# langfod/Zonos

Measured on AMD Instinct MI355X. Metric: audio-sec/sec (RTF), Zonos-v0.1-transformer AR decode loop + DAC decode, higher is better.
Workload: dtype bf16; 1 GPU; Zonos-v0.1-transformer bf16, batch=1 per GPU, 10 s target audio (861 frames, 868 decode steps + prefill of 25 positions, EOS suppressed), greedy, cfg_scale 2; weights=seeded synthetic (zonos_amd/synth.py), parallelism=dp1 (utterance sharding, no data-path collective)

## Files before the change

### include/zonos_hip.h

```cpp
#ifndef ZONOS_HIP_H
#define ZONOS_HIP_H
#include <stddef.h>
#include <stdint.h>

#ifdef __cplusplus
extern "C" {
#endif

#define ZN_ABI_VERSION 9

enum zn_status {
  ZN_OK = 0,
  ZN_ERR_ARG = -1,
  ZN_ERR_HIP = -2,
  ZN_ERR_STATE = -3,
  ZN_ERR_UNSUPPORTED = -4,
  ZN_ERR_NOMEM = -5
};

typedef struct zn_handle_s* zn_handle;
typedef struct zn_dac_s* zn_dac;
typedef struct zn_spk_s* zn_spk;
typedef void* zn_stream;

// ... 9 lines not shown
  int32_t arch;
  int32_t m_d_inner;
  int32_t m_headdim;
  int32_t m_d_state;
  int32_t m_ngroups;
  int32_t m_d_conv;
  int32_t rms_norm;
  int32_t residual_in_fp32;
  int32_t rope_mode;
} zn_config;

typedef struct zn_layer_weights {
  const void *norm_w, *norm_b;
  const void *in_proj;
  const void *out_proj;
  const void *norm2_w, *norm2_b;
  const void *fc1;
  const void *fc2;
  int32_t kind;
  const void *m_in_proj;
  const void *m_conv_w, *m_conv_b;
  const void *m_dt_bias, *m_A_log, *m_D;
  const void *m_norm_w;
  const void *m_out_proj;
  const void *in_proj_bias;
  const void *out_proj_bias;
} zn_layer_weights;

typedef struct zn_weights {
  const void* const* embeddings;
  const void* heads;
  const void *norm_f_w, *norm_f_b;
  const zn_layer_weights* layers;
  const float* rope_table;
} zn_weights;

typedef struct zn_sampling {
  float temperature;
  float top_p; int32_t top_k; float min_p;
  float linear, conf, quad;
  float repetition_penalty; int32_t repetition_penalty_window;
  uint64_t seed;
} zn_sampling;

#define ZN_ROW_PARAMS_BYTES 64
typedef struct zn_row_params {
  zn_sampling sp;
  float cfg_scale;
  int32_t max_new_tokens;
  int32_t reserved[2];
} zn_row_params;

typedef struct zn_admit {
  int32_t slot;
  int32_t row_len;
  int32_t prefix_len;
  int32_t reserved;
  zn_row_params params;
} zn_admit;

int zn_abi_version(void);
int zn_create(const zn_config* cfg, const zn_weights* w, int32_t max_rows, zn_handle* out);
int zn_destroy(zn_handle h);
const char* zn_last_error(zn_handle h);
size_t zn_kv_bytes_per_layer(const zn_config* cfg, int32_t rows, int32_t max_len);
size_t zn_mamba_state_bytes_per_layer(const zn_config* cfg, int32_t rows, size_t* conv_bytes);

int zn_gen_begin(zn_handle h, int32_t batch, const void* const* kv_layers_dev, int32_t max_len,
                 int32_t* lengths_dev, int32_t* delayed_codes_dev, int32_t t_total, int32_t offset0,
                 int32_t max_new_tokens, float cfg_scale, const zn_sampling* sp, zn_stream stream);
int zn_prefill(zn_handle h, const void* hidden_dev, int32_t S, zn_stream stream);
int zn_gen_set_rows(zn_handle h, const zn_row_params* rows_host, int32_t n);
int zn_gen_set_prefix_rows(zn_handle h, const int32_t* prefix_len_host, int32_t n);
int zn_gen_open_slots(zn_handle h, int32_t slack);
int zn_gen_admit(zn_handle h, const zn_admit* a, int32_t n, const void* hidden_dev, int32_t S, zn_stream stream);
int zn_gen_retire(zn_handle h, int32_t slot);
int zn_gen_row_state(zn_handle h, int32_t* remaining_host, int32_t* steps_host, zn_stream stream);
int zn_prefill_rows(zn_handle h, const void* hidden_dev, int32_t S, const int32_t* row_len, zn_stream stream);
int zn_sample_first(zn_handle h, zn_stream stream);
int zn_decode_steps(zn_handle h, int32_t n, zn_stream stream);
int zn_graph_active(zn_handle h);
int zn_decode_path(zn_handle h);
int zn_decode_path_detail(zn_handle h);
int zn_get_counters(zn_handle h, int64_t* out, int32_t n);
int zn_gen_end(zn_handle h);
int zn_tenant_try_claim(int32_t device, const void* owner);
int zn_tenant_release(int32_t device, const void* owner);
int zn_all_stopped(zn_handle h, int32_t* out, zn_stream stream);
int zn_all_stopped_begin(zn_handle h, zn_stream stream);
int zn_all_stopped_end(zn_handle h, int32_t* all_stopped_out);
int zn_get_step_outputs(zn_handle h, float* logits_dev, int32_t* tokens_dev, zn_stream stream);
int zn_codes_changed(zn_handle h);
int zn_debug_force_eos(zn_handle h, int32_t step);
int zn_debug_token_override(zn_handle h, const int32_t* tokens_dev, int32_t calls);
int zn_debug_prefill_mode(zn_handle h, int32_t mode);
enum zn_tune_key {
  ZN_TUNE_WG_IN_PROJ = 0,
  ZN_TUNE_WG_OUT_PROJ = 1,
  ZN_TUNE_WG_FC1 = 2,
  ZN_TUNE_WG_FC2 = 3,
  ZN_TUNE_WG_HEADS = 4,
  ZN_TUNE_ATTN_FUSED_MAX_KEYS = 5,
  ZN_TUNE_GRAPH_RUNS = 6,
  ZN_TUNE_SMALL_M_LDS = 7,
  ZN_TUNE_PERSISTENT = 8,
  ZN_TUNE_FC1_LN_LAUNCH = 9,
  ZN_TUNE_PREFILL_ATTN_VALU = 10,
  ZN_TUNE_NO_SPLIT_SMALL_M = 11,
  ZN_TUNE_NO_PREFILL_GEMM16K = 12,
  ZN_TUNE_GEMM16K_MAX_TILES = 13,
  ZN_TUNE_HOOK = 14,
  ZN_TUNE_WHOLE_STEP = 15,
  ZN_TUNE_SAMPLER = 16,
  ZN_TUNE_RESERVED_17 = 17,
  ZN_TUNE_STACK_PRE = 18,
  ZN_TUNE_ATTN_SPLIT_COLS = 19,
  ZN_TUNE_NKEYS = 20
};
enum zn_tune_hook {
  ZN_HOOK_TAG_WRAP = 7,
  ZN_HOOK_TIMEOUT_WORD = 9,
  ZN_HOOK_PAUSE = 11,
  ZN_HOOK_RESET_WAIT_STATS = 13
};
int zn_debug_tune(zn_handle h, int32_t key, int32_t value);
int zn_debug_chain_stamps(zn_handle h, uint64_t* stamps_dev);
int zn_debug_trace(zn_handle h, void* trace_dev);
int zn_debug_eos_bias(zn_handle h, float bias);

int zn_op_backbone_forward(zn_handle h, const void* hidden_dev, void* out_dev, const void* const* caches_dev, int32_t max_len,
                           int32_t base, int32_t S, int32_t rows, zn_stream stream);

int zn_bench_kernel(zn_handle h, int32_t which, int32_t rows, int32_t iters, float* ms_per_launch,
                    double* bytes_per_launch, zn_stream stream);

int zn_op_linear(zn_handle h, const void* x_dev, const void* ln_w, const void* ln_b, const void* W_dev,
                 void* out_dev, int32_t rows, int32_t N, int32_t K, zn_stream stream);
int zn_op_linear_bias(zn_handle h, const void* x_dev, const void* W_dev, const void* bias_dev, void* out_dev, int32_t rows,
                      int32_t N, int32_t K, zn_stream stream);
int zn_op_gather_rows(zn_handle h, const void* table_dev, const int32_t* ids_dev, void* out_dev, int32_t n, int32_t d,
                      int32_t table_rows, int32_t id_offset, zn_stream stream);
int zn_op_fourier(zn_handle h, const float* x_dev, const void* weight_dev, void* out_dev, int32_t n, int32_t in_dim,
                  int32_t half, float min_val, float max_val, zn_stream stream);
int zn_op_silu(zn_handle h, const void* x_dev, void* out_dev, int64_t n, zn_stream stream);
int zn_op_layernorm(zn_handle h, const void* x_dev, const void* w_dev, const void* b_dev, void* out_dev, int32_t rows,
                    int32_t d, zn_stream stream);
int zn_op_layer_decode(zn_handle h, int32_t layer, void* x_dev, void* kv_dev, int32_t max_len,
                       const int32_t* lengths_dev, const int32_t* ext_dev, int32_t rows, zn_stream stream);
int zn_op_attn_decode(zn_handle h, const void* q_dev, const void* kv_dev, int32_t max_len, const int32_t* lengths_dev,
                      const int32_t* ext_dev, void* out_dev, int32_t rows, zn_stream stream);
int zn_op_attn_prefill(zn_handle h, const void* q_dev, const void* kv_dev, int32_t max_len, void* out_dev, int32_t positions,
                       int32_t rows, zn_stream stream);
int zn_op_add_layernorm(zn_handle h, const void* hidden, void* res, const void* w, const void* b, void* out, int32_t rows,
                        int32_t d, float eps, int32_t flags, zn_stream stream);
int zn_op_mamba_step(zn_handle h, int32_t layer, const void* x, void* state, void* out, int32_t rows, zn_stream stream);
int zn_op_embed(zn_handle h, const int32_t* codes_dev, void* out_dev, int32_t batch, zn_stream stream);
int zn_op_sample(zn_handle h, const float* logits_dev, const int32_t* recent_dev, int32_t window,
                 const zn_sampling* sp, uint64_t draw_index, int32_t* tokens_dev, float* probs_out_dev,
                 int32_t batch, zn_stream stream);
int zn_op_assemble_prefill(zn_handle h, const void* cond_dev, int32_t L_c, const int32_t* cond_len_dev, const int32_t* delayed_codes_dev,
                           int32_t t_total, const int32_t* prefix_len_dev, int32_t batch, int32_t rows, void* hidden_dev, int32_t S,
                           int32_t* row_len_dev, zn_stream stream);
int zn_op_sample_rows(zn_handle h, const float* logits_dev, const int32_t* recent_dev, int32_t window, const zn_row_params* rows_dev,
                      uint64_t draw_index, int32_t* tokens_dev, float* probs_out_dev, int32_t batch, zn_stream stream);

typedef struct zn_dac_config {
  int32_t n_codebooks, codebook_size, codebook_dim, hidden_size, decoder_hidden_size;
  int32_t n_ratios; int32_t ratios[8];
  int32_t encoder_hidden_size;
} zn_dac_config;
typedef struct zn_dac_tensor { const char* name; const float* data_dev; int64_t numel; } zn_dac_tensor;
int zn_dac_create(const zn_dac_config* cfg, const zn_dac_tensor* tensors, int32_t n_tensors, zn_dac* out);
int zn_dac_destroy(zn_dac d);
const char* zn_dac_last_error(zn_dac d);
int zn_dac_decode(zn_dac d, const int32_t* codes_dev, int32_t batch, int32_t T, float* wav_dev, zn_stream stream);
int zn_dac_span(const zn_dac_config* cfg, int32_t c0, int32_t n, int32_t at_end, int64_t* s0, int64_t* s1);
int zn_dac_decode_span(zn_dac d, const int32_t* codes_dev, int32_t batch, int32_t c0, int32_t n, int32_t at_end, float* wav_dev,
                       zn_stream stream);
typedef struct zn_dac_span_row { int32_t c0, n, at_end; } zn_dac_span_row;
int zn_dac_decode_spans(zn_dac d, const int32_t* codes_dev, int32_t n_max, const zn_dac_span_row* rows_host, int32_t rows,
                        float* wav_dev, int64_t t_max, zn_stream stream);
int zn_dac_encode(zn_dac d, const float* wav_dev, int32_t batch, int32_t T, int32_t* codes_dev, zn_stream stream);

int zn_spk_create(const zn_dac_tensor* tensors, int32_t n_tensors, zn_spk* out);
int zn_spk_destroy(zn_spk d);
const char* zn_spk_last_error(zn_spk d);
int zn_spk_embed(zn_spk d, const float* feat_dev, int32_t batch, int32_t T, float* emb_dev, float* lda_out_dev, zn_stream stream);

#ifdef __cplusplus
}
#endif
#endif
```

### zonos_amd/_lib.py

```python
from __future__ import annotations

import ctypes as C
import os
import sys

_HERE = os.path.dirname(os.path.abspath(__file__))
LIB_PATH = os.environ.get("ZONOS_HIP_LIB") or os.path.join(_HERE, "libzonos_hip.so")

ZN_ABI_VERSION = 9

ZN_TUNE_WG_IN_PROJ, ZN_TUNE_WG_OUT_PROJ, ZN_TUNE_WG_FC1, ZN_TUNE_WG_FC2, ZN_TUNE_WG_HEADS = 0, 1, 2, 3, 4
ZN_TUNE_ATTN_FUSED_MAX_KEYS = 5
ZN_TUNE_GRAPH_RUNS = 6
ZN_TUNE_SMALL_M_LDS = 7
ZN_TUNE_PERSISTENT = 8
ZN_TUNE_FC1_LN_LAUNCH = 9
ZN_TUNE_PREFILL_ATTN_VALU = 10
ZN_TUNE_NO_SPLIT_SMALL_M = 11
ZN_TUNE_NO_PREFILL_GEMM16K = 12
ZN_TUNE_GEMM16K_MAX_TILES = 13
ZN_TUNE_HOOK = 14
ZN_TUNE_WHOLE_STEP = 15
ZN_TUNE_SAMPLER = 16
ZN_TUNE_RESERVED_17 = 17
ZN_TUNE_STACK_PRE = 18
ZN_TUNE_ATTN_SPLIT_COLS = 19
ZN_TUNE_NKEYS = 20
ZN_HOOK_TAG_WRAP, ZN_HOOK_TIMEOUT_WORD, ZN_HOOK_PAUSE, ZN_HOOK_RESET_WAIT_STATS = 7, 9, 11, 13


class ZonosHipError(RuntimeError):
    pass


class zn_config(C.Structure):
    _fields_ = [(n, C.c_int32) for n in ("d_model", "n_layer", "n_heads", "n_heads_kv", "d_ff", "n_codebooks", "vocab_head",
                                          "vocab_embed", "eos_id", "mask_id", "rope_positions", "double_out_proj")] + [("norm_eps", C.c_float)] + \
               [(n, C.c_int32) for n in ("arch", "m_d_inner", "m_headdim", "m_d_state", "m_ngroups", "m_d_conv", "rms_norm", "residual_in_fp32", "rope_mode")]


class zn_layer_weights(C.Structure):
    _fields_ = [(n, C.c_void_p) for n in ("norm_w", "norm_b", "in_proj", "out_proj", "norm2_w", "norm2_b", "fc1", "fc2")] + [("kind", C.c_int32)] + \
               [(n, C.c_void_p) for n in ("m_in_proj", "m_conv_w", "m_conv_b", "m_dt_bias", "m_A_log", "m_D", "m_norm_w", "m_out_proj", "in_proj_bias", "out_proj_bias")]


class zn_weights(C.Structure):
    _fields_ = [("embeddings", C.POINTER(C.c_void_p)), ("heads", C.c_void_p), ("norm_f_w", C.c_void_p), ("norm_f_b", C.c_void_p),
                ("layers", C.POINTER(zn_layer_weights)), ("rope_table", C.c_void_p)]


class zn_sampling(C.Structure):
    _fields_ = [("temperature", C.c_float), ("top_p", C.c_float), ("top_k", C.c_int32), ("min_p", C.c_float),
                ("linear", C.c_float), ("conf", C.c_float), ("quad", C.c_float), ("repetition_penalty", C.c_float),
                ("repetition_penalty_window", C.c_int32), ("seed", C.c_uint64)]


class zn_row_params(C.Structure):
    _fields_ = [("sp", zn_sampling), ("cfg_scale", C.c_float), ("max_new_tokens", C.c_int32), ("reserved", C.c_int32 * 2)]


ZN_ROW_PARAMS_BYTES = 64


class zn_admit(C.Structure):
    _fields_ = [("slot", C.c_int32), ("row_len", C.c_int32), ("prefix_len", C.c_int32), ("reserved", C.c_int32), ("params", zn_row_params)]


class zn_dac_config(C.Structure):
    _fields_ = [(n, C.c_int32) for n in ("n_codebooks", "codebook_size", "codebook_dim", "hidden_size", "decoder_hidden_size", "n_ratios")] + \
               [("ratios", C.c_int32 * 8), ("encoder_hidden_size", C.c_int32)]


class zn_dac_tensor(C.Structure):
    _fields_ = [("name", C.c_char_p), ("data_dev", C.c_void_p), ("numel", C.c_int64)]


class zn_dac_span_row(C.Structure):
    _fields_ = [("c0", C.c_int32), ("n", C.c_int32), ("at_end", C.c_int32)]


SIGNATURES = {
    "zn_abi_version": (C.c_int, []),
    "zn_create": (C.c_int, [C.POINTER(zn_config), C.POINTER(zn_weights), C.c_int32, C.POINTER(C.c_void_p)]),
    "zn_destroy": (C.c_int, [C.c_void_p]),
    "zn_last_error": (C.c_char_p, [C.c_void_p]),
    "zn_kv_bytes_per_layer": (C.c_size_t, [C.POINTER(zn_config), C.c_int32, C.c_int32]),
    "zn_mamba_state_bytes_per_layer": (C.c_size_t, [C.POINTER(zn_config), C.c_int32, C.POINTER(C.c_size_t)]),
    "zn_gen_begin": (C.c_int, [C.c_void_p, C.c_int32, C.POINTER(C.c_void_p), C.c_int32, C.c_void_p, C.c_void_p, C.c_int32, C.c_int32,
                               C.c_int32, C.c_float, C.POINTER(zn_sampling), C.c_void_p]),
    "zn_prefill": (C.c_int, [C.c_void_p, C.c_void_p, C.c_int32, C.c_void_p]),
    "zn_prefill_rows": (C.c_int, [C.c_void_p, C.c_void_p, C.c_int32, C.POINTER(C.c_int32), C.c_void_p]),
    "zn_gen_set_rows": (C.c_int, [C.c_void_p, C.POINTER(zn_row_params), C.c_int32]),
    "zn_gen_set_prefix_rows": (C.c_int, [C.c_void_p, C.POINTER(C.c_int32), C.c_int32]),
    "zn_gen_open_slots": (C.c_int, [C.c_void_p, C.c_int32]),
    "zn_gen_admit": (C.c_int, [C.c_void_p, C.POINTER(zn_admit), C.c_int32, C.c_void_p, C.c_int32, C.c_void_p]),
    "zn_gen_retire": (C.c_int, [C.c_void_p, C.c_int32]),
    "zn_gen_row_state": (C.c_int, [C.c_void_p, C.POINTER(C.c_int32), C.POINTER(C.c_int32), C.c_void_p]),
    "zn_sample_first": (C.c_int, [C.c_void_p, C.c_void_p]),
    "zn_decode_steps": (C.c_int, [C.c_void_p, C.c_int32, C.c_void_p]),
    "zn_graph_active": (C.c_int, [C.c_void_p]),
    "zn_gen_end": (C.c_int, [C.c_void_p]),
    "zn_tenant_try_claim": (C.c_int, [C.c_int32, C.c_void_p]),
    "zn_tenant_release": (C.c_int, [C.c_int32, C.c_void_p]),
    "zn_decode_path": (C.c_int, [C.c_void_p]),
    "zn_decode_path_detail": (C.c_int, [C.c_void_p]),
    "zn_get_counters": (C.c_int, [C.c_void_p, C.POINTER(C.c_int64), C.c_int32]),
    "zn_all_stopped": (C.c_int, [C.c_void_p, C.POINTER(C.c_int32), C.c_void_p]),
    "zn_all_stopped_begin": (C.c_int, [C.c_void_p, C.c_void_p]),
    "zn_all_stopped_end": (C.c_int, [C.c_void_p, C.POINTER(C.c_int32)]),
    "zn_get_step_outputs": (C.c_int, [C.c_void_p, C.c_void_p, C.c_void_p, C.c_void_p]),
    "zn_debug_force_eos": (C.c_int, [C.c_void_p, C.c_int32]),
    "zn_debug_token_override": (C.c_int, [C.c_void_p, C.c_void_p, C.c_int32]),
    "zn_codes_changed": (C.c_int, [C.c_void_p]),
    "zn_debug_prefill_mode": (C.c_int, [C.c_void_p, C.c_int32]),
    "zn_debug_tune": (C.c_int, [C.c_void_p, C.c_int32, C.c_int32]),
    "zn_debug_eos_bias": (C.c_int, [C.c_void_p, C.c_float]),
    "zn_debug_chain_stamps": (C.c_int, [C.c_void_p, C.c_void_p]),
    "zn_debug_trace": (C.c_int, [C.c_void_p, C.c_void_p]),
    "zn_bench_kernel": (C.c_int, [C.c_void_p, C.c_int32, C.c_int32, C.c_int32, C.POINTER(C.c_float), C.POINTER(C.c_double), C.c_void_p]),
    "zn_op_linear": (C.c_int, [C.c_void_p] + [C.c_void_p] * 5 + [C.c_int32] * 3 + [C.c_void_p]),
    "zn_op_linear_bias": (C.c_int, [C.c_void_p] * 5 + [C.c_int32] * 3 + [C.c_void_p]),
    "zn_op_gather_rows": (C.c_int, [C.c_void_p] * 4 + [C.c_int32] * 4 + [C.c_void_p]),
    "zn_op_fourier": (C.c_int, [C.c_void_p] * 4 + [C.c_int32] * 3 + [C.c_float, C.c_float, C.c_void_p]),
    "zn_op_silu": (C.c_int, [C.c_void_p] * 3 + [C.c_int64, C.c_void_p]),
    "zn_op_layernorm": (C.c_int, [C.c_void_p] * 5 + [C.c_int32, C.c_int32, C.c_void_p]),
    "zn_op_layer_decode": (C.c_int, [C.c_void_p, C.c_int32, C.c_void_p, C.c_void_p, C.c_int32, C.c_void_p, C.c_void_p, C.c_int32, C.c_void_p]),
    "zn_op_backbone_forward": (C.c_int, [C.c_void_p, C.c_void_p, C.c_void_p, C.POINTER(C.c_void_p), C.c_int32, C.c_int32, C.c_int32, C.c_int32, C.c_void_p]),
    "zn_op_attn_prefill": (C.c_int, [C.c_void_p, C.c_void_p, C.c_void_p, C.c_int32, C.c_void_p, C.c_int32, C.c_int32, C.c_void_p]),
    "zn_op_attn_decode": (C.c_int, [C.c_void_p, C.c_void_p, C.c_void_p, C.c_int32, C.c_void_p, C.c_void_p, C.c_void_p, C.c_int32, C.c_void_p]),
    "zn_op_embed": (C.c_int, [C.c_void_p, C.c_void_p, C.c_void_p, C.c_int32, C.c_void_p]),
    "zn_op_add_layernorm": (C.c_int, [C.c_void_p, C.c_void_p, C.c_void_p, C.c_void_p, C.c_void_p, C.c_void_p, C.c_int32, C.c_int32, C.c_float, C.c_int32, C.c_void_p]),
    "zn_op_mamba_step": (C.c_int, [C.c_void_p, C.c_int32, C.c_void_p, C.c_void_p, C.c_void_p, C.c_int32, C.c_void_p]),
    "zn_op_sample": (C.c_int, [C.c_void_p, C.c_void_p, C.c_void_p, C.c_int32, C.POINTER(zn_sampling), C.c_uint64, C.c_void_p, C.c_void_p,
                               C.c_int32, C.c_void_p]),
    "zn_op_assemble_prefill": (C.c_int, [C.c_void_p, C.c_void_p, C.c_int32, C.c_void_p, C.c_void_p, C.c_int32, C.c_void_p, C.c_int32, C.c_int32,
                                         C.c_void_p, C.c_int32, C.c_void_p, C.c_void_p]),
    "zn_op_sample_rows": (C.c_int, [C.c_void_p, C.c_void_p, C.c_void_p, C.c_int32, C.c_void_p, C.c_uint64, C.c_void_p, C.c_void_p,
                                    C.c_int32, C.c_void_p]),
    "zn_dac_create": (C.c_int, [C.POINTER(zn_dac_config), C.POINTER(zn_dac_tensor), C.c_int32, C.POINTER(C.c_void_p)]),
    "zn_dac_destroy": (C.c_int, [C.c_void_p]),
    "zn_dac_last_error": (C.c_char_p, [C.c_void_p]),
    "zn_dac_decode": (C.c_int, [C.c_void_p, C.c_void_p, C.c_int32, C.c_int32, C.c_void_p, C.c_void_p]),
    "zn_dac_encode": (C.c_int, [C.c_void_p, C.c_void_p, C.c_int32, C.c_int32, C.c_void_p, C.c_void_p]),
    "zn_dac_span": (C.c_int, [C.POINTER(zn_dac_config), C.c_int32, C.c_int32, C.c_int32, C.POINTER(C.c_int64), C.POINTER(C.c_int64)]),
    "zn_dac_decode_span": (C.c_int, [C.c_void_p, C.c_void_p, C.c_int32, C.c_int32, C.c_int32, C.c_int32, C.c_void_p, C.c_void_p]),
    "zn_dac_decode_spans": (C.c_int, [C.c_void_p, C.c_void_p, C.c_int32, C.POINTER(zn_dac_span_row), C.c_int32, C.c_void_p, C.c_int64, C.c_void_p]),
    "zn_spk_create": (C.c_int, [C.POINTER(zn_dac_tensor), C.c_int32, C.POINTER(C.c_void_p)]),
    "zn_spk_destroy": (C.c_int, [C.c_void_p]),
    "zn_spk_last_error": (C.c_char_p, [C.c_void_p]),
    "zn_spk_embed": (C.c_int, [C.c_void_p, C.c_void_p, C.c_int32, C.c_int32, C.c_void_p, C.c_void_p, C.c_void_p]),
}

_lib = None


def load() -> C.CDLL:
    global _lib
    if _lib is not None:
        return _lib
    path = os.environ.get("ZONOS_HIP_LIB_VARIANT")
    if path:
        path = os.path.join(os.path.dirname(_HERE), "build", "variants", f"libzonos_hip_{path}.so")
        if not os.path.exists(path):
            raise ZonosHipError(f"{path} not found (ZONOS_HIP_LIB_VARIANT)")
        print(f"[zonos_amd] loading variant library {path}", file=sys.stderr, flush=True)
    else:
        path = LIB_PATH
    if not os.path.exists(path):
        raise ZonosHipError(f"{path} not found: build it with `python -m zonos_amd.build` "
                            "(the HIP library is the only execution path; there is no CPU fallback)")
    import torch
    lib = C.CDLL(path)
    for name, (res, args) in SIGNATURES.items():
        fn = getattr(lib, name)
        fn.restype, fn.argtypes = res, args
    if lib.zn_abi_version() != ZN_ABI_VERSION:
        raise ZonosHipError(f"ABI mismatch: library {lib.zn_abi_version()} vs binding {ZN_ABI_VERSION}")
    _lib = lib
    return lib


def check(rc: int, handle=None, what: str = "") -> None:
    if rc != 0:
        msg = load().zn_last_error(handle)
        raise ZonosHipError(f"{what} failed (status {rc}): {msg.decode() if msg else ''}")


def check_dac(rc: int, handle=None, what: str = "") -> None:
# ... 13 lines not shown
```

### zonos_amd/csrc/zn_api.hip

```cpp
#include "../../include/zonos_hip.h"
#include "zn_decode_kernels.h"
#include "zn_chain_kernel.h"
#include "zn_step_kernel.h"
#include "zn_prefill_kernels.h"
#include "zn_cond_kernels.h"
#include "zn_mamba_kernels.h"

#include <cmath>
#include <cstdio>
#include <cstdlib>
#include <cstring>
#include <mutex>
#include <string>
#include <vector>

static thread_local std::string g_create_err;
#define ZN_GRAPH_STEPS 8
#define ZN_G16_PART_BYTES ((size_t)8 << 20)
#define ZN_REARM_AFTER 4

struct StepPlan {
  enum Path { LAUNCHES, CHAIN, STACK } path = LAUNCHES;
  int nbk = 0;
  int attn_fused = 0;
  int run = 1;
  bool fused_tail = false;
  int graph_slot = 0;
};

struct zn_handle_s {
  zn_config cfg;
  int max_rows = 0, hd = 0, G = 0;
  std::vector<zn_layer_weights> layers;
  const void* heads = nullptr;
  const void *norm_f_w = nullptr, *norm_f_b = nullptr;
  const float* rope = nullptr;
  const bf16_t** emb_tables_dev = nullptr;
  bool has_io = false;
  bf16_t *x = nullptr, *q = nullptr, *o1 = nullptr, *mbuf = nullptr, *nbuf = nullptr;
  bf16_t *res = nullptr, *hn = nullptr, *m_zx = nullptr, *m_xbc = nullptr, *m_y = nullptr, *m_g = nullptr;
  float* m_vg = nullptr;
  int m_nheads = 0, m_conv_dim = 0, m_d_in_proj = 0;
  unsigned long long *ch_gy1 = nullptr, *ch_gx1 = nullptr, *ch_gx2 = nullptr, *ch_gm = nullptr;
  unsigned long long *ch_gqkv = nullptr, *ch_ga = nullptr;
  unsigned long long *ch_gbmax = nullptr, *ch_gpart = nullptr;
  bool stackv_ok[4] = {};
  bool stackv1_ok[4] = {};
  StackLayer* stack_layers = nullptr;
  bool stack_ok = false, stack1_ok = false, stack_checked = false;
  unsigned* ch_epoch = nullptr;
  unsigned long long epoch_bound = 1;
  unsigned* ch_diag = nullptr;
  unsigned diag_host[8] = {};
  bf16_t* ch_x2 = nullptr;
  bf16_t* dbg_trace = nullptr;
  bf16_t* x_emb = nullptr;
  int* tail_ticket = nullptr;
  bool emb_valid = false;
  unsigned long long* ch_stamps = nullptr;
  int device = 0;
  bool demoted = false;
  int clean_since_demotion = 0;
  long long n_timeouts = 0, n_generations = 0, n_fallback_generations = 0, n_rearms = 0;
  bool gen_timed_out = false;
  hipStream_t gen_stream = nullptr;
  bool persist_ok = true;
  int ch_variant = 0;
  float* g16_part = nullptr;
  int* g16_tickets = nullptr;
  size_t g16_part_bytes = 0;
  float* ln_part = nullptr;
  float *logits_raw = nullptr, *last_logits = nullptr;
  int* tok_raw = nullptr;
  float *scores = nullptr, *cmax = nullptr;
  float* pv_part = nullptr;
  int* pv_tickets = nullptr;
  bf16_t *pf_x = nullptr, *pf_n = nullptr, *pf_qkv = nullptr, *pf_a = nullptr, *pf_u = nullptr, *pf_m = nullptr;
  bf16_t *pf_res = nullptr, *pf_zx = nullptr, *pf_xbc = nullptr, *pf_y = nullptr, *pf_g = nullptr;
  size_t pf_rows = 0;
  int* fw_lengths = nullptr;
  int* row_len = nullptr;
  std::vector<int> row_len_host;
  bool rows_unequal2 = false;
  bf16_t* qkv_tmp = nullptr;
  int prefill_mode = 1;
  int lcap = 0;
  GenState* st = nullptr;
  int *remaining = nullptr, *stopping = nullptr;
  zn_row_params* row_tab = nullptr;
  bool rows_set = false;
  bool pairs_set = false;
  int* prefix_shift = nullptr;
  bool prefix_set = false;
  bool gen_prefilled = false;
  bool slots_open = false;
  int slot_slack = 0;
  int* step0 = nullptr;
  std::vector<int> slot_len;
  std::vector<char> slot_busy;
  void* adm_cache = nullptr;
  size_t adm_layer_bytes = 0;
  int adm_cap_S = 0;
  AdmitLayer* adm_layers = nullptr;
  std::vector<const void*> adm_caches;
  char* adm_stage = nullptr;
  char* adm_dev = nullptr;
  hipEvent_t adm_event = nullptr;
  bool adm_pending = false;
  int* done_host = nullptr;
  hipEvent_t stop_event = nullptr;
  bool stop_pending = false;
  bool gen_active = false;
  bool gen_ended = false;
  int batch = 0, rows = 0, max_len = 0, t_total = 0, offset0 = 0, max_new = 0;
  float cfg_scale = 2.f;
  zn_sampling sp{};
  std::vector<const void*> kv_layers;
  int *lengths = nullptr, *codes = nullptr;
  int force_eos_step = -1;
  float eos_bias = 0.f;
  unsigned dbg_pause = 0;
  int tune[ZN_TUNE_NKEYS] = {};
  int pending_hook = 0;
  const int* tok_override = nullptr;
  int tok_override_calls = 0;
  hipStream_t cap_stream = nullptr;
#define ZN_NGRAPHS (8 + 2 * (ZN_SK_KB_MAXNB + 1))
  hipGraphExec_t graph_exec[ZN_NGRAPHS] = {};
  hipGraph_t graph[ZN_NGRAPHS] = {};
  bool graph_tried[ZN_NGRAPHS] = {};
  int len_hi = 0;
  StepPlan last_plan;
  std::string err;
};

#define ZN_FAIL(h, code, ...)                                   \
  do {                                                          \
    char _b[1024]; snprintf(_b, sizeof _b, __VA_ARGS__);         \
    if (h) (h)->err = _b; else g_create_err = _b;               \
    return (code);                                              \
  } while (0)
#define HIPCHK(h, call)                                                                       \
  do {                                                                                        \
    hipError_t _e = (call);                                                                   \
    if (_e != hipSuccess) ZN_FAIL(h, ZN_ERR_HIP, "%s failed: %s", #call, hipGetErrorString(_e)); \
  } while (0)

extern "C" int zn_abi_version(void) { return ZN_ABI_VERSION; }

extern "C" const char* zn_last_error(zn_handle h) { return h ? h->err.c_str() : g_create_err.c_str(); }

extern "C" size_t zn_kv_bytes_per_layer(const zn_config* c, int32_t rows, int32_t max_len) {
  if (!c || c->n_heads <= 0) return 0;
  const size_t hd = (size_t)c->d_model / c->n_heads;
  return (size_t)rows * max_len * 2 * c->n_heads_kv * hd * 2;
}

extern "C" size_t zn_mamba_state_bytes_per_layer(const zn_config* c, int32_t rows, size_t* conv_bytes) {
  if (conv_bytes) *conv_bytes = 0;
  if (!c || c->arch != 1 || c->m_headdim <= 0 || rows < 0) return 0;
  const size_t conv_dim = (size_t)c->m_d_inner + 2 * (size_t)c->m_ngroups * c->m_d_state;
  const size_t cb = (size_t)rows * conv_dim * c->m_d_conv * 2;
  if (conv_bytes) *conv_bytes = cb;
  return cb + (size_t)rows * c->m_d_inner * c->m_d_state * 2;
}

static void free_graph(zn_handle h) {
  for (int k = 0; k < ZN_NGRAPHS; ++k) {
    if (h->graph_exec[k]) { (void)hipGraphExecDestroy(h->graph_exec[k]); h->graph_exec[k] = nullptr; }
    if (h->graph[k]) { (void)hipGraphDestroy(h->graph[k]); h->graph[k] = nullptr; }
    h->graph_tried[k] = false;
  }
}

static std::mutex g_tenant_mu;
static const void* g_tenant[64] = {};
extern "C" int zn_tenant_try_claim(int32_t device, const void* owner) {
  if (device < 0 || device >= 64 || !owner) return 0;
  std::lock_guard<std::mutex> lk(g_tenant_mu);
  if (g_tenant[device] && g_tenant[device] != owner) return 0;
  g_tenant[device] = owner;
  return 1;
}
extern "C" int zn_tenant_release(int32_t device, const void* owner) {
  if (device < 0 || device >= 64) return 0;
  std::lock_guard<std::mutex> lk(g_tenant_mu);
  if (g_tenant[device] != owner) return 0;
  g_tenant[device] = nullptr;
  return 1;
}
static std::mutex g_capture_mu;
#define ZN_NOT_IN_CAPTURE(call) [&] { std::lock_guard<std::mutex> lk(g_capture_mu); return (call); }()

extern "C" int zn_destroy(zn_handle h) {
  if (!h) return ZN_OK;
  (void)zn_tenant_release(h->device, h);
  free_graph(h);
  void* ptrs[] = {h->emb_tables_dev, h->x, h->q, h->o1, h->mbuf, h->nbuf, h->logits_raw, h->last_logits, h->tok_raw, h->scores, h->cmax, h->pv_part, h->pv_tickets, h->pf_x, h->pf_n, h->pf_qkv, h->pf_a, h->pf_u, h->pf_m, h->pf_res, h->pf_zx, h->pf_xbc, h->pf_y, h->pf_g, h->qkv_tmp, h->fw_lengths, h->row_len, h->st, h->remaining, h->stopping, h->row_tab, h->prefix_shift, h->step0, h->adm_cache, h->adm_layers, h->adm_dev, h->res, h->hn, h->m_zx, h->m_xbc, h->m_y, h->m_g, h->m_vg, h->g16_part, h->g16_tickets, h->ln_part, h->ch_gy1, h->ch_gx1, h->ch_gx2, h->ch_gm, h->ch_epoch, h->ch_x2, h->x_emb, h->tail_ticket, h->ch_gqkv, h->ch_ga, h->ch_gbmax, h->ch_gpart, h->stack_layers, h->ch_diag};
  for (void* p : ptrs) if (p) (void)hipFree(p);
  if (h->done_host) (void)hipHostFree(h->done_host);
  if (h->adm_stage) (void)hipHostFree(h->adm_stage);
  if (h->adm_event) (void)hipEventDestroy(h->adm_event);
  if (h->stop_event) (void)hipEventDestroy(h->stop_event);
  if (h->cap_stream) (void)hipStreamDestroy(h->cap_stream);
  delete h;
  return ZN_OK;
}

#define ZN_CH_GRID 256
#define ZN_CH_DYN_LDS (64 * 1024)
template <int NCH, int T_OUT, int T_FC1, int T_FC2, int T_IN>
static bool chain_resident(int n_cus) {
  int per_cu = 0;
  if (hipOccupancyMaxActiveBlocksPerMultiprocessor(&per_cu, chain_kernel<NCH, T_OUT, T_FC1, T_FC2, T_IN>, ZN_CH_THREADS, ZN_CH_DYN_LDS) != hipSuccess) {
    (void)hipGetLastError();
    return false;
  }
  return per_cu >= 1 && n_cus >= ZN_CH_GRID;
}
static int chain_variant_for(const zn_config& c) {
  if (c.arch != 0 || !c.double_out_proj || c.d_ff != 4 * c.d_model) return 0;
  int dev = 0, n_cus = 0;
  if (hipGetDevice(&dev) != hipSuccess || hipDeviceGetAttribute(&n_cus, hipDeviceAttributeMultiprocessorCount, dev) != hipSuccess) { (void)hipGetLastError(); return 0; }
  const int G = ZN_CH_GRID, hd = c.d_model / c.n_heads, nqkv = (c.n_heads + 2 * c.n_heads_kv) * hd;
  if ((c.d_model / 2) % G || c.d_ff % G || (nqkv / 2) % G || nqkv % 2) return 0;
  const int p_out = c.d_model / 2 / G, p_fc1 = c.d_ff / G, p_in = nqkv / 2 / G;
  if (p_fc1 * 2 > 64 || p_out * 2 > 64 || p_in * 2 > 64) return 0;
  auto fits = [&](int t_out, int t_fc1, int t_fc2, int t_in) {
    return p_out <= ZN_CH_CWAVES * t_out && p_fc1 <= ZN_CH_CWAVES * t_fc1 && p_out <= (ZN_CH_CWAVES / 4) * t_fc2 && p_in <= ZN_CH_CWAVES * t_in;
  };
  if (c.d_model == 2048 && fits(1, 8, 4, 2) && chain_resident<4, 1, 8, 4, 2>(n_cus) && chain_resident<4, 1, 8, 4, 0>(n_cus) && chain_resident<4, 1, 8, 4, 5>(n_cus)) return 1;
  if (c.d_model == 512 && fits(1, 2, 1, 1) && chain_resident<1, 1, 2, 1, 1>(n_cus) && chain_resident<1, 1, 2, 1, 0>(n_cus) && chain_resident<1, 1, 2, 1, 5>(n_cus)) return 2;
  return 0;
}

extern "C" int zn_create(const zn_config* cfg, const zn_weights* w, int32_t max_rows, zn_handle* out) {
  if (!cfg || !w || !out) ZN_FAIL((zn_handle) nullptr, ZN_ERR_ARG, "zn_create: null argument");
  *out = nullptr;
  const zn_config& c = *cfg;
  if (c.d_model <= 0 || c.n_layer <= 0 || c.n_heads <= 0 || c.n_heads_kv <= 0 || c.d_ff <= 0 || c.n_codebooks <= 0)
    ZN_FAIL((zn_handle) nullptr, ZN_ERR_ARG, "zn_create: non-positive dimension");
  if (c.d_model % c.n_heads || c.n_heads % c.n_heads_kv) ZN_FAIL((zn_handle) nullptr, ZN_ERR_ARG, "zn_create: heads do not divide");
  const int hd = c.d_model / c.n_heads, G = c.n_heads / c.n_heads_kv;
  if (hd != 32 && hd != 64 && hd != 128) ZN_FAIL((zn_handle) nullptr, ZN_ERR_UNSUPPORTED, "head_dim %d not in {32,64,128}", hd);
  if (G != 1 && G != 2 && G != 4 && G != 8) ZN_FAIL((zn_handle) nullptr, ZN_ERR_UNSUPPORTED, "GQA group %d not in {1,2,4,8}", G);
  if (c.d_model % 8 || c.d_ff % 8 || c.d_model > 4096) ZN_FAIL((zn_handle) nullptr, ZN_ERR_UNSUPPORTED, "d_model/d_ff must be multiples of 8, d_model <= 4096");
  if (c.n_codebooks > ZN_FRAME_MAXQ) ZN_FAIL((zn_handle) nullptr, ZN_ERR_UNSUPPORTED, "n_codebooks > %d", ZN_FRAME_MAXQ);
  if (c.vocab_head > ZN_SAMPLE_MAXV) ZN_FAIL((zn_handle) nullptr, ZN_ERR_UNSUPPORTED, "vocab_head > %d", ZN_SAMPLE_MAXV);
  if (max_rows < 2 || max_rows % 2) ZN_FAIL((zn_handle) nullptr, ZN_ERR_ARG, "max_rows must be even and >= 2");
  if (c.arch != 0 && c.arch != 1) ZN_FAIL((zn_handle) nullptr, ZN_ERR_ARG, "zn_create: arch must be 0 (transformer) or 1 (hybrid)");
  if (c.arch == 1) {
    if (c.m_headdim != 64 || (c.m_d_state != 64 && c.m_d_state != 128) || c.m_d_conv != 4)
      ZN_FAIL((zn_handle) nullptr, ZN_ERR_UNSUPPORTED, "Mamba2: headdim %d / d_state %d / d_conv %d not in {64} x {64,128} x {4}", c.m_headdim, c.m_d_state, c.m_d_conv);
    if (c.m_d_inner <= 0 || c.m_d_inner % 64 || c.m_ngroups < 1 || (c.m_d_inner / 64) % c.m_ngroups || (c.m_d_inner / c.m_ngroups) % 8 ||
        c.m_d_inner / c.m_ngroups > 8192)
      ZN_FAIL((zn_handle) nullptr, ZN_ERR_UNSUPPORTED, "Mamba2: d_inner %d / ngroups %d not supported", c.m_d_inner, c.m_ngroups);
  }
  if (c.rope_mode < 0 || c.rope_mode > 2) ZN_FAIL((zn_handle) nullptr, ZN_ERR_ARG, "zn_create: rope_mode must be 0, 1 or 2");
  zn_handle h = new zn_handle_s();
  h->cfg = c; h->max_rows = max_rows; h->hd = hd; h->G = G;
  h->tune[ZN_TUNE_WG_IN_PROJ] = 256; h->tune[ZN_TUNE_WG_OUT_PROJ] = 512; h->tune[ZN_TUNE_WG_FC1] = 512; h->tune[ZN_TUNE_WG_FC2] = 1024; h->tune[ZN_TUNE_WG_HEADS] = 512;
  h->tune[ZN_TUNE_ATTN_FUSED_MAX_KEYS] = 512; h->tune[ZN_TUNE_GRAPH_RUNS] = 2; h->tune[ZN_TUNE_SMALL_M_LDS] = 2;
  if (hipGetDevice(&h->device) != hipSuccess) { (void)hipGetLastError(); h->device = 0; }
  if (c.arch == 1) {
    h->m_nheads = c.m_d_inner / c.m_headdim;
    h->m_conv_dim = c.m_d_inner + 2 * c.m_ngroups * c.m_d_state;
    h->m_d_in_proj = 2 * c.m_d_inner + 2 * c.m_ngroups * c.m_d_state + h->m_nheads;
  }
  if (const char* e = getenv("ZN_PREFILL_MODE")) h->prefill_mode = atoi(e);
  h->layers.assign(w->layers, w->layers + c.n_layer);
  h->heads = w->heads; h->norm_f_w = w->norm_f_w; h->norm_f_b = w->norm_f_b; h->rope = w->rope_table;
#define ZC(call) do { hipError_t _e = ZN_NOT_IN_CAPTURE(call); if (_e != hipSuccess) { g_create_err = std::string(#call) + ": " + hipGetErrorString(_e); zn_destroy(h); return ZN_ERR_HIP; } } while (0)
  ZC(hipMalloc(&h->emb_tables_dev, sizeof(void*) * c.n_codebooks));
  if (w->embeddings) ZC(hipMemcpy(h->emb_tables_dev, w->embeddings, sizeof(void*) * c.n_codebooks, hipMemcpyHostToDevice));
  h->has_io = (w->embeddings != nullptr && w->heads != nullptr);
  const size_t R = max_rows;
  ZC(hipMalloc(&h->x, R * c.d_model * 2));
  ZC(hipMalloc(&h->q, R * c.d_model * 2));
  ZC(hipMalloc(&h->o1, R * c.d_model * 2));
  ZC(hipMalloc(&h->mbuf, R * c.d_ff * 2));
  ZC(hipMalloc(&h->nbuf, R * c.d_model * 2));
  ZC(hipMalloc(&h->logits_raw, R * c.n_codebooks * c.vocab_head * sizeof(float)));
  ZC(hipMalloc(&h->last_logits, R * c.n_codebooks * c.vocab_head * sizeof(float)));
  ZC(hipMalloc(&h->tok_raw, R * c.n_codebooks * sizeof(int)));
  ZC(hipMalloc(&h->fw_lengths, R * sizeof(int)));
  ZC(hipMalloc(&h->row_len, R * sizeof(int)));
  ZC(hipMalloc(&h->st, sizeof(GenState)));
  ZC(hipMemset(h->st, 0, sizeof(GenState)));
  ZC(hipMalloc(&h->remaining, R * sizeof(int)));
  ZC(hipMalloc(&h->stopping, R * sizeof(int)));
  ZC(hipMalloc(&h->row_tab, R * sizeof(zn_row_params)));
  ZC(hipMalloc(&h->prefix_shift, R * sizeof(int)));
  ZC(hipHostMalloc(&h->done_host, sizeof(int) * 8));
  ZC(hipEventCreateWithFlags(&h->stop_event, hipEventDisableTiming));
  for (unsigned long long** g : {&h->ch_gy1, &h->ch_gx1, &h->ch_gx2}) {
    ZC(hipMalloc(g, R * (c.d_model / 2) * 8));
    ZC(hipMemset(*g, 0, R * (c.d_model / 2) * 8));
  }
  { const size_t nqkv = (size_t)(c.n_heads + 2 * c.n_heads_kv) * hd;
    ZC(hipMalloc(&h->ch_gqkv, R * (nqkv / 2 + 1) * 8)); ZC(hipMemset(h->ch_gqkv, 0, R * (nqkv / 2 + 1) * 8));
    ZC(hipMalloc(&h->ch_ga, R * (c.d_model / 2) * 8)); ZC(hipMemset(h->ch_ga, 0, R * (c.d_model / 2) * 8));
    { const size_t nbm = (size_t)2 * c.n_heads_kv * ZN_SK_KB_MAXNB * 4 * 8, npt = (size_t)2 * c.n_heads_kv * ZN_SK_KB_MAXNB * ZN_SK_KB_PSZ * 8;
      ZC(hipMalloc(&h->ch_gbmax, nbm)); ZC(hipMemset(h->ch_gbmax, 0, nbm));
      ZC(hipMalloc(&h->ch_gpart, npt)); ZC(hipMemset(h->ch_gpart, 0, npt)); }
    ZC(hipMalloc(&h->stack_layers, (size_t)c.n_layer * sizeof(StackLayer))); }
  ZC(hipMalloc(&h->ch_gm, R * (c.d_ff / 2 + 1) * 8));
  ZC(hipMemset(h->ch_gm, 0, R * (c.d_ff / 2 + 1) * 8));
  ZC(hipMalloc(&h->ch_epoch, 64));
  ZC(hipMalloc(&h->ch_diag, 64));
  ZC(hipMemset(h->ch_diag, 0, 64));
  { const unsigned one = 1; ZC(hipMemcpy(h->ch_epoch, &one, sizeof one, hipMemcpyHostToDevice)); }
  ZC(hipMalloc(&h->ch_x2, R * c.d_model * 2));
  h->ch_variant = chain_variant_for(c);
  if (const char* e = getenv("ZN_CHAIN")) if (atoi(e) == 0) h->tune[ZN_TUNE_PERSISTENT] = 2;
  if (const char* e = getenv("ZN_STACK")) if (atoi(e) == 0) h->tune[ZN_TUNE_WHOLE_STEP] = 2;
  {
    ZC(hipMalloc(&h->x_emb, R * c.d_model * 2));
    ZC(hipMalloc(&h->tail_ticket, sizeof(int)));
    ZC(hipMemset(h->tail_ticket, 0, sizeof(int)));
    ZC(hipMalloc(&h->g16_part, ZN_G16_PART_BYTES));
    ZC(hipMalloc(&h->g16_tickets, ZN_G16_MAX_GROUPS * sizeof(int)));
    ZC(hipMemset(h->g16_tickets, 0, ZN_G16_MAX_GROUPS * sizeof(int)));
    h->g16_part_bytes = ZN_G16_PART_BYTES;
    ZC(hipMalloc(&h->ln_part, R * ZN_G16_LNT * 2 * sizeof(float)));
  }
  if (c.arch == 1) {
    ZC(hipMalloc(&h->res, R * c.d_model * 4));
    ZC(hipMalloc(&h->qkv_tmp, R * (size_t)(c.n_heads + 2 * c.n_heads_kv) * hd * 2));
    ZC(hipMalloc(&h->hn, R * c.d_model * 2));
    ZC(hipMalloc(&h->m_zx, R * h->m_d_in_proj * 2));
    ZC(hipMalloc(&h->m_xbc, R * h->m_conv_dim * 2));
    ZC(hipMalloc(&h->m_y, R * c.m_d_inner * 2));
    ZC(hipMalloc(&h->m_vg, R * c.m_d_inner * sizeof(float)));
    ZC(hipMalloc(&h->m_g, R * c.m_d_inner * 2));
  }
#undef ZC
  *out = h;
  return ZN_OK;
}

template <int R, int NCH, int KS, int PRO, int EPI>
static void launch_gemv_t(const GemvArgs& a, int blocks, bool full, hipStream_t s) {
  if (full) hipLaunchKernelGGL((gemv_kernel<R, NCH, KS, PRO, EPI, true>), dim3(blocks), dim3(256), 0, s, a);
  else hipLaunchKernelGGL((gemv_kernel<R, NCH, KS, PRO, EPI, false>), dim3(blocks), dim3(256), 0, s, a);
}
template <int R, int KS, int PRO, int EPI>
static int launch_gemv_nch(const GemvArgs& a, int nch, int blocks, bool full, hipStream_t s) {
  switch (nch) {
    case 1: launch_gemv_t<R, 1, KS, PRO, EPI>(a, blocks, full, s); return 0;
    case 2: launch_gemv_t<R, 2, KS, PRO, EPI>(a, blocks, full, s); return 0;
    case 4: launch_gemv_t<R, 4, KS, PRO, EPI>(a, blocks, full, s); return 0;
    case 8: launch_gemv_t<R, 8, KS, PRO, EPI>(a, blocks, full, s); return 0;
  }
  return -1;
}
template <int PRO, int EPI>
static int launch_gemv_rows(const GemvArgs& a, int rgroup, int ks, int nch, int blocks, bool full, hipStream_t s) {
  if (ks == 1) {
    if (rgroup <= 2) return launch_gemv_nch<2, 1, PRO, EPI>(a, nch, blocks, full && rgroup == 2, s);
    return launch_gemv_nch<4, 1, PRO, EPI>(a, nch, blocks, full && rgroup == 4, s);
  }
  if constexpr (PRO == PRO_NONE || PRO == PRO_GATED) {
    if (rgroup <= 2) return launch_gemv_nch<2, 4, PRO, EPI>(a, nch, blocks, full && rgroup == 2, s);
    return launch_gemv_nch<4, 4, PRO, EPI>(a, nch, blocks, full && rgroup == 4, s);
  }
  return -1;
}

static void launch_gemm(const bf16_t* A, int lda, const bf16_t* W, bf16_t* out, int ldo, const bf16_t* resid, int M, int N, int K, hipStream_t s,
                        const bf16_t* bias = nullptr) {
  GemmArgs g{A, W, out, resid, M, N, K, lda, ldo, bias};
  dim3 grid((N + 127) / 128, (M + 127) / 128);
  if (M >= 256 && K % ZN_PG_KC == 0 && lda % 8 == 0) {
    if (resid) hipLaunchKernelGGL((gemm_bf16s_kernel<1>), grid, dim3(256), 0, s, g);
    else hipLaunchKernelGGL((gemm_bf16s_kernel<0>), grid, dim3(256), 0, s, g);
    return;
  }
  if (resid) hipLaunchKernelGGL((gemm_bf16_kernel<1>), grid, dim3(256), 0, s, g);
  else hipLaunchKernelGGL((gemm_bf16_kernel<0>), grid, dim3(256), 0, s, g);
}
template <int NW, int EPI>
static void launch_gemm16_t(const GemvArgs& g, int blocks, bool tile8, hipStream_t s) {
  if constexpr (lin_has_tile8(EPI)) if (tile8) { hipLaunchKernelGGL((gemm16_kernel<NW, EPI, 8>), dim3(blocks), dim3(NW * 64), 0, s, g); return; }
  hipLaunchKernelGGL((gemm16_kernel<NW, EPI>), dim3(blocks), dim3(NW * 64), 0, s, g);
}
template <int EPI, bool LNP>
static void launch_gemm16s_t(const GemvArgs& g, const LinearPlan& p, hipStream_t s) {
// ... 242 lines not shown
  a.ln2_w = (const bf16_t*)lw.norm2_w; a.ln2_b = (const bf16_t*)lw.norm2_b; a.eps = c.norm_eps; a.F = c.d_ff;
  a.a = h->o1; a.xin = xin ? xin : chain_x(h, li); a.xout = chain_x(h, li + 1);
  a.g_y1 = h->ch_gy1; a.g_x1 = h->ch_gx1; a.g_x2 = h->ch_gx2; a.g_m = h->ch_gm;
  a.epoch = h->ch_epoch; a.tmo = &h->st->pad[0]; a.diag = h->ch_diag;
  a.dbg_pause = h->dbg_pause; a.stamp_layer = li;
  a.stamps = h->ch_stamps ? h->ch_stamps + (size_t)li * 32 : nullptr;
  if (!last) {
    const zn_layer_weights& nx = h->layers[li + 1];
    a.W_in = (const bf16_t*)nx.in_proj; a.lnn_w = (const bf16_t*)nx.norm_w; a.lnn_b = (const bf16_t*)nx.norm_b;
    a.nqkv = (c.n_heads + 2 * c.n_heads_kv) * h->hd;
    a.q_out = h->q; a.kv = (bf16_t*)kv_layers[li + 1]; a.rope = h->rope; a.lengths = lengths;
    a.max_len = max_len; a.hd = h->hd; a.n_heads = c.n_heads; a.n_heads_kv = c.n_heads_kv; a.rope_positions = c.rope_positions;
  }
  const bool heads = last && with_heads;
  if (heads) {
    a.W_in = (const bf16_t*)h->heads; a.lnn_w = (const bf16_t*)h->norm_f_w; a.lnn_b = (const bf16_t*)h->norm_f_b;
    a.nqkv = c.n_codebooks * c.vocab_head; a.heads_out = h->logits_raw;
  }
  const dim3 grid(ZN_CH_GRID), block(ZN_CH_THREADS);
  if (h->ch_variant == 1) {
    if (heads) hipLaunchKernelGGL((chain_kernel<4, 1, 8, 4, 5>), grid, block, ZN_CH_DYN_LDS, s, a);
    else if (last) hipLaunchKernelGGL((chain_kernel<4, 1, 8, 4, 0>), grid, block, ZN_CH_DYN_LDS, s, a);
    else hipLaunchKernelGGL((chain_kernel<4, 1, 8, 4, 2>), grid, block, ZN_CH_DYN_LDS, s, a);
  } else {
    if (heads) hipLaunchKernelGGL((chain_kernel<1, 1, 2, 1, 5>), grid, block, ZN_CH_DYN_LDS, s, a);
    else if (last) hipLaunchKernelGGL((chain_kernel<1, 1, 2, 1, 0>), grid, block, ZN_CH_DYN_LDS, s, a);
    else hipLaunchKernelGGL((chain_kernel<1, 1, 2, 1, 1>), grid, block, ZN_CH_DYN_LDS, s, a);
  }
  return ZN_OK;
}

#if ZN_SK_CW == 6
#define ZN_SK_T1 4, 1, 7, 4, 4, 6
#define ZN_SK_T2 4, 1, 8, 4, 5, 8
#define ZN_SK_T3 4, 2, 9, 5, 5, 12
#else
#define ZN_SK_T1 4, 2, 10, 5, 6, 6
#define ZN_SK_T2 4, 2, 11, 6, 7, 8
#define ZN_SK_T3 4, 2, 13, 7, 8, 12
#endif
static int stack_variant_of(int mode) { return mode <= 6 ? 1 : mode <= 8 ? 2 : 3; }
template <int R, int NCH, int T_OUT, int T_FC1, int T_FC2, int T_IN, int NBV>
static bool stack_variant_ok(zn_handle h, int natt) {
  const zn_config& c = h->cfg;
  const int nsw = ZN_CH_GRID - natt;
  if (nsw < 64) return false;
  auto most = [&](int units) { return (units + nsw - 1) / nsw; };
  const int nqkv = (c.n_heads + 2 * c.n_heads_kv) * h->hd;
  const int p_out = most(c.d_model / 2), p_fc1 = 2 * most(c.d_ff / 2), p_qkv = most((nqkv + 1) / 2), p_hd = most((c.n_codebooks * c.vocab_head + 1) / 2);
  if (p_out > ZN_SK_CW * T_OUT || 4 * p_out > ZN_SK_CW * T_FC2 || p_fc1 > ZN_SK_CW * T_FC1 || p_qkv > ZN_SK_CW * T_IN || p_hd > ZN_SK_CW * T_IN) return false;
  if (p_qkv > 10) return false;
  if (p_out * 2 > 64 || p_out * 4 > 64 || p_fc1 > 64 || p_qkv * 2 > 64 || p_hd * 2 > 64 || nqkv % 2) return false;
  const void* fn = R == 1 ? (const void*)step_r1_kernel<NCH, T_OUT, T_FC1, T_FC2, T_IN, NBV> : (const void*)step_kernel<NCH, T_OUT, T_FC1, T_FC2, T_IN, NBV>;
  int dev = 0, n_cus = 0, per_cu = 0;
  if (hipGetDevice(&dev) != hipSuccess || hipDeviceGetAttribute(&n_cus, hipDeviceAttributeMultiprocessorCount, dev) != hipSuccess) { (void)hipGetLastError(); return false; }
  if (hipFuncSetAttribute(fn, hipFuncAttributeMaxDynamicSharedMemorySize, ZN_SK_DYN_LDS) != hipSuccess) { (void)hipGetLastError(); return false; }
  if (hipOccupancyMaxActiveBlocksPerMultiprocessor(&per_cu, fn, ZN_SK_THREADS, ZN_SK_DYN_LDS) != hipSuccess) { (void)hipGetLastError(); return false; }
  hipFuncAttributes fa{};
  if (hipFuncGetAttributes(&fa, fn) != hipSuccess) { (void)hipGetLastError(); return false; }
  return per_cu >= 1 && n_cus >= ZN_CH_GRID && fa.localSizeBytes == 0;
}
static bool stack_shapes_ok(zn_handle h) {
  const zn_config& c = h->cfg;
  if (h->ch_variant != 1 || h->hd != 128 || c.n_heads_kv < 1 || c.n_heads != 4 * c.n_heads_kv) return false;
  const int npairs = 2 * c.n_heads_kv, nkvh = c.n_heads_kv;
  h->stackv_ok[1] = stack_variant_ok<2, ZN_SK_T1>(h, npairs * 6);
  h->stackv_ok[2] = stack_variant_ok<2, ZN_SK_T2>(h, npairs * 8);
  h->stackv_ok[3] = stack_variant_ok<2, ZN_SK_T3>(h, npairs * ZN_SK_KB_MAXNB);
  h->stackv1_ok[1] = stack_variant_ok<1, ZN_SK_T1>(h, nkvh * 6);
  h->stackv1_ok[2] = stack_variant_ok<1, ZN_SK_T2>(h, nkvh * 8);
  h->stackv1_ok[3] = stack_variant_ok<1, ZN_SK_T3>(h, nkvh * ZN_SK_KB_MAXNB);
  h->stack1_ok = h->stackv1_ok[1];
  return h->stackv_ok[1];
}
static bool persist_allowed(zn_handle h) { return h->tune[ZN_TUNE_PERSISTENT] != 2 && !h->demoted && h->persist_ok && !h->rows_unequal2 && !h->prefix_set && !h->slots_open && !h->pairs_set; }
static bool persist_shape(zn_handle h, int rows) { return h->ch_variant != 0 && (rows == 2 || (rows == 1 && h->ch_variant == 1)); }
static bool persist_active(zn_handle h, int rows) { return persist_shape(h, rows) && persist_allowed(h); }
static int stack_blocks_for(zn_handle h, int rows, int keys_upper_bound) {
  if (h->tune[ZN_TUNE_WHOLE_STEP] == 2 || !(rows == 1 ? h->stack1_ok : h->stack_ok)) return -1;
  const int nb = keys_upper_bound <= 512 ? 1 : (keys_upper_bound + 511) / 512;
  return nb <= ZN_SK_KB_MAXNB && (rows == 1 ? h->stackv1_ok : h->stackv_ok)[stack_variant_of(nb)] ? nb : -1;
}
static int graph_slot_for(const StepPlan& p) { return p.path == StepPlan::STACK ? 8 + (p.run > 1 ? ZN_SK_KB_MAXNB + 1 : 0) + p.nbk : p.attn_fused + (p.run > 1 ? 4 : 0); }
static bool chain_allowed(zn_handle h, int rows) { return h->ch_variant != 0 && rows == 2 && persist_allowed(h); }
static StepPlan plan_blocks(zn_handle h, int rows, int keys) {
  StepPlan p;
  p.path = chain_allowed(h, rows) ? StepPlan::CHAIN : StepPlan::LAUNCHES; p.attn_fused = attn_fused_for(h, keys);
  return p;
}
static StepPlan plan_steps(zn_handle h, int steps_left) {
  const int rows = h->rows, keys = h->len_hi + 1, keys_run = h->len_hi + ZN_GRAPH_STEPS;
  const bool want_run = steps_left >= ZN_GRAPH_STEPS && h->tune[ZN_TUNE_GRAPH_RUNS] > 1;
  const bool tail_ok = h->cfg.arch == 0 && persist_active(h, rows) && h->batch <= 2;
  const int nb_run = tail_ok && want_run ? stack_blocks_for(h, rows, keys_run) : -1;
  const int nb_one = tail_ok ? stack_blocks_for(h, rows, keys) : -1;
  StepPlan p = plan_blocks(h, rows, keys);
  if (nb_run >= 0 || nb_one >= 0) {
    p.path = StepPlan::STACK; p.nbk = nb_run >= 0 ? nb_run : nb_one; p.run = nb_run >= 0 ? ZN_GRAPH_STEPS : 1;
  } else if (want_run && attn_fused_for(h, keys_run) == p.attn_fused) p.run = ZN_GRAPH_STEPS;
  p.fused_tail = tail_ok && p.path != StepPlan::LAUNCHES;
  p.graph_slot = graph_slot_for(p);
  return p;
}
static bool stack_pre(zn_handle h) { return h->tune[ZN_TUNE_STACK_PRE] != 2; }
static int launch_stack(zn_handle h, hipStream_t s, int rows, int nbk) {
  const zn_config& c = h->cfg;
  ChainArgs a{};
  a.eps = c.norm_eps; a.F = c.d_ff; a.nqkv = (c.n_heads + 2 * c.n_heads_kv) * h->hd;
  a.xin = h->x_emb; a.xout = h->x;
  a.g_y1 = h->ch_gy1; a.g_x1 = h->ch_gx1; a.g_x2 = h->ch_gx2; a.g_m = h->ch_gm; a.g_qkv = h->ch_gqkv; a.g_a = h->ch_ga;
  a.g_bmax = h->ch_gbmax; a.g_part = h->ch_gpart;
  a.epoch = h->ch_epoch; a.tmo = &h->st->pad[0]; a.diag = h->ch_diag;
  a.dbg_pause = h->dbg_pause;
  a.stamps = h->ch_stamps; a.stamp_layer = c.n_layer / 2;
  a.rope = h->rope; a.lengths = h->lengths; a.max_len = h->max_len; a.hd = h->hd; a.n_heads = c.n_heads; a.n_heads_kv = c.n_heads_kv;
  a.rope_positions = c.rope_positions;
  a.layers = h->stack_layers; a.n_layer = c.n_layer; a.q0 = h->q; a.scale = (float)(1.0 / std::sqrt((double)h->hd));
  a.heads_rows = c.n_codebooks * c.vocab_head; a.heads_out = h->logits_raw; a.trace = h->dbg_trace;
  const int mode = nbk, npairs = rows * c.n_heads_kv;
  a.natt = npairs * (mode < 1 ? 1 : mode);
  if (stack_pre(h)) {
    a.pre_W = (const bf16_t*)h->layers[0].in_proj; a.pre_ln_w = (const bf16_t*)h->layers[0].norm_w; a.pre_ln_b = (const bf16_t*)h->layers[0].norm_b;
    a.pre_kv = (bf16_t*)h->kv_layers[0];
  }
  const dim3 grid(ZN_CH_GRID), block(ZN_SK_THREADS);
  if (rows == 1) {
    switch (stack_variant_of(mode)) {
      case 1: hipLaunchKernelGGL((step_r1_kernel<ZN_SK_T1>), grid, block, ZN_SK_DYN_LDS, s, a); break;
      case 2: hipLaunchKernelGGL((step_r1_kernel<ZN_SK_T2>), grid, block, ZN_SK_DYN_LDS, s, a); break;
      default: hipLaunchKernelGGL((step_r1_kernel<ZN_SK_T3>), grid, block, ZN_SK_DYN_LDS, s, a); break;
    }
    return ZN_OK;
  }
  if (rows != 2) ZN_FAIL(h, ZN_ERR_STATE, "launch_stack: %d rows (the whole-step kernel serves one or two)", rows);
  switch (stack_variant_of(mode)) {
    case 1: hipLaunchKernelGGL((step_kernel<ZN_SK_T1>), grid, block, ZN_SK_DYN_LDS, s, a); break;
    case 2: hipLaunchKernelGGL((step_kernel<ZN_SK_T2>), grid, block, ZN_SK_DYN_LDS, s, a); break;
    default: hipLaunchKernelGGL((step_kernel<ZN_SK_T3>), grid, block, ZN_SK_DYN_LDS, s, a); break;
  }
  return ZN_OK;
}
static int build_stack_table(zn_handle h) {
  const zn_config& c = h->cfg;
  std::vector<StackLayer> t(c.n_layer);
  for (int li = 0; li < c.n_layer; ++li) {
    const zn_layer_weights& lw = h->layers[li];
    const bool last = li + 1 == c.n_layer;
    StackLayer& L = t[li];
    L.W_out = (const bf16_t*)lw.out_proj; L.W_fc1 = (const bf16_t*)lw.fc1; L.W_fc2 = (const bf16_t*)lw.fc2;
    L.ln2_w = (const bf16_t*)lw.norm2_w; L.ln2_b = (const bf16_t*)lw.norm2_b;
    L.kv = (const bf16_t*)h->kv_layers[li];
    if (last) { L.W_in = (const bf16_t*)h->heads; L.lnn_w = (const bf16_t*)h->norm_f_w; L.lnn_b = (const bf16_t*)h->norm_f_b; L.kv_next = nullptr; }
    else {
      const zn_layer_weights& nx = h->layers[li + 1];
      L.W_in = (const bf16_t*)nx.in_proj; L.lnn_w = (const bf16_t*)nx.norm_w; L.lnn_b = (const bf16_t*)nx.norm_b; L.kv_next = (bf16_t*)h->kv_layers[li + 1];
    }
  }
  HIPCHK(h, ZN_NOT_IN_CAPTURE(hipMemcpy(h->stack_layers, t.data(), t.size() * sizeof(StackLayer), hipMemcpyHostToDevice)));
  return ZN_OK;
}

static int decode_blocks(zn_handle h, const StepPlan& p, const int* ext, int ext_scalar, hipStream_t s, const bf16_t* x0 = nullptr, bool* heads_done = nullptr) {
  const zn_config& c = h->cfg;
  int rc;
  const size_t tb = (size_t)h->rows * c.d_model * 2;
  const bool chain = p.path == StepPlan::CHAIN;
  if (x0 && !chain) ZN_FAIL(h, ZN_ERR_STATE, "decode_blocks: a separate input buffer is the chain path's");
  auto trace = [&](int li) {
    if (!h->dbg_trace) return;
    (void)hipMemcpyAsync((char*)h->dbg_trace + (size_t)(8 * li) * tb, chain ? chain_x(h, li + 1) : h->x, tb, hipMemcpyDeviceToDevice, s);
    (void)hipMemcpyAsync((char*)h->dbg_trace + (size_t)(8 * li + 1) * tb, h->o1, tb, hipMemcpyDeviceToDevice, s);
    if (!chain) (void)hipMemcpyAsync((char*)h->dbg_trace + (size_t)(8 * li + 3) * tb, h->mbuf, (size_t)h->rows * c.d_ff * 2 <= 4 * tb ? (size_t)h->rows * c.d_ff * 2 : 4 * tb, hipMemcpyDeviceToDevice, s);
  };
  auto trace_q = [&](int li) {
    if (h->dbg_trace) (void)hipMemcpyAsync((char*)h->dbg_trace + (size_t)(8 * li + 2) * tb, h->q, tb, hipMemcpyDeviceToDevice, s);
  };
  if (!chain) {
    for (int li = 0; li < c.n_layer; ++li) {
      if ((rc = layer_in_proj(h, li, h->x, (bf16_t*)h->kv_layers[li], h->max_len, h->lengths, h->rows, s))) return rc;
      trace_q(li);
      if ((rc = run_attention(h, h->q, (bf16_t*)h->kv_layers[li], h->max_len, h->lengths, ext, ext_scalar, h->o1, h->rows, p.attn_fused, s))) return rc;
      if ((rc = layer_post_attention(h, li, h->x, h->rows, s, h->dbg_trace ? (bf16_t*)((char*)h->dbg_trace + (size_t)(8 * li + 7) * tb) : nullptr))) return rc;
      trace(li);
    }
    return ZN_OK;
  }
  if ((rc = layer_in_proj(h, 0, x0 ? const_cast<bf16_t*>(x0) : h->x, (bf16_t*)h->kv_layers[0], h->max_len, h->lengths, h->rows, s))) return rc;
  h->epoch_bound += c.n_layer;
  for (int li = 0; li < c.n_layer; ++li) {
    trace_q(li);
    if ((rc = run_attention(h, h->q, (bf16_t*)h->kv_layers[li], h->max_len, h->lengths, ext, ext_scalar, h->o1, h->rows, p.attn_fused, s,
                            h->ch_stamps ? h->ch_stamps + (size_t)(c.n_layer + li) * 32 : nullptr))) return rc;
    const bool wh = heads_done && li + 1 == c.n_layer && chain_heads_fit(h);
    if ((rc = launch_chain(h, li, h->kv_layers, h->max_len, h->lengths, s, li == 0 ? x0 : nullptr, wh))) return rc;
// ... 63 lines not shown
    GemvArgs a{};
    a.W = (const bf16_t*)lw.in_proj; a.N = nq + 2 * nkv; a.K = d; a.x = h->hn;
    a.lengths = lengths; a.hd = hd; a.n_heads = c.n_heads; a.n_heads_kv = c.n_heads_kv;
    a.q_out = h->q; a.kv = (bf16_t*)cache; a.rope = h->rope; a.max_len = max_len; a.rope_positions = c.rope_positions;
    if ((rc = run_gemv<PRO_NONE, EPI_ROPE_KV>(h, a, rows, h->tune[ZN_TUNE_WG_IN_PROJ], s))) return rc;
  } else {
    GemvArgs a{};
    a.W = (const bf16_t*)lw.in_proj; a.N = nq + 2 * nkv; a.K = d; a.x = h->hn; a.out = h->qkv_tmp; a.bias = (const bf16_t*)lw.in_proj_bias;
    if ((rc = run_gemv<PRO_NONE, EPI_STORE>(h, a, rows, h->tune[ZN_TUNE_WG_IN_PROJ], s))) return rc;
    hipLaunchKernelGGL(rope_kv_any_kernel, dim3(1, rows), dim3(256), 0, s, h->qkv_tmp, h->q, nq, (bf16_t*)cache, h->rope, 1, 0, lengths, max_len,
                       c.n_heads, c.n_heads_kv, hd, c.rope_positions, c.rope_mode);
  }
  if ((rc = run_attention(h, h->q, (const bf16_t*)cache, max_len, lengths, nullptr, 0, h->o1, rows, attn_fused, s))) return rc;
  {
    GemvArgs a{};
    a.W = (const bf16_t*)lw.out_proj; a.N = d; a.K = nq; a.x = h->o1; a.out = h->x; a.bias = (const bf16_t*)lw.out_proj_bias;
    if ((rc = run_gemv<PRO_NONE, EPI_STORE>(h, a, rows, h->tune[ZN_TUNE_WG_OUT_PROJ], s))) return rc;
  }
  launch_add_ln(h, h->x, h->res, 1, 1, lw.norm2_w, lw.norm2_b, h->hn, rows, s);
  {
    GemvArgs a{};
    a.W = (const bf16_t*)lw.fc1; a.N = 2 * c.d_ff; a.K = d; a.x = h->hn; a.out = h->mbuf;
    if ((rc = run_gemv<PRO_NONE, EPI_SILU>(h, a, rows, h->tune[ZN_TUNE_WG_FC1], s))) return rc;
  }
  {
    GemvArgs a{};
    a.W = (const bf16_t*)lw.fc2; a.N = d; a.K = c.d_ff; a.x = h->mbuf; a.out = h->x;
    if ((rc = run_gemv<PRO_NONE, EPI_STORE>(h, a, rows, h->tune[ZN_TUNE_WG_FC2], s))) return rc;
  }
  return ZN_OK;
}

static int hybrid_heads(zn_handle h, hipStream_t s) {
  const zn_config& c = h->cfg;
  launch_add_ln(h, h->x, h->res, 1, 0, h->norm_f_w, h->norm_f_b, h->hn, h->rows, s);
  GemvArgs a{};
  a.W = (const bf16_t*)h->heads; a.N = c.n_codebooks * c.vocab_head; a.K = c.d_model; a.x = h->hn; a.out_f32 = h->logits_raw;
  return run_gemv<PRO_NONE, EPI_F32>(h, a, h->rows, h->tune[ZN_TUNE_WG_HEADS], s);
}

static int hybrid_token(zn_handle h, bool want_logits, int attn_fused, hipStream_t s) {
  const zn_config& c = h->cfg;
  int rc;
  for (int li = 0; li < c.n_layer; ++li)
    if ((rc = hybrid_layer(h, li, (void*)h->kv_layers[li], h->max_len, h->lengths, h->rows, attn_fused, s))) return rc;
  if (!want_logits) return ZN_OK;
  return hybrid_heads(h, s);
}

static SampleArgs make_sample_args(zn_handle h, const zn_sampling& sp) {
  SampleArgs a{};
  const zn_config& c = h->cfg;
  a.n_q = c.n_codebooks; a.V = c.vocab_head; a.eos_id = c.eos_id;
  a.temperature = sp.temperature; a.top_p = sp.top_p; a.top_k = sp.top_k; a.min_p = sp.min_p;
  a.linear = sp.linear; a.conf = sp.conf; a.quad = sp.quad;
  a.penalty = sp.repetition_penalty; a.pen_window = sp.repetition_penalty_window;
  a.seed = sp.seed;
  return a;
}
static_assert(sizeof(zn_row_params) == ZN_ROW_PARAMS_BYTES, "zn_row_params is one 64-byte entry per utterance");

static bool guided(zn_handle h) { return h->rows == 2 * h->batch; }

static EmbedArgs make_embed_args(zn_handle h) {
  const zn_config& c = h->cfg;
  EmbedArgs e{};
  e.tables = h->emb_tables_dev; e.codes = h->codes; e.col_dev = &h->st->offset; e.sb = c.n_codebooks * h->t_total; e.si = h->t_total;
  e.col = 0; e.n_q = c.n_codebooks; e.d = c.d_model; e.batch = h->batch; e.vocab_embed = c.vocab_embed; e.out = h->x_emb; e.dup = guided(h) ? 1 : 0;
  e.shift = h->prefix_set ? h->prefix_shift : nullptr;
  e.step0 = h->slots_open ? h->step0 : nullptr;
  return e;
}

static SampleArgs gen_sample_args(zn_handle h) {
  SampleArgs a = make_sample_args(h, h->sp);
  a.cfg_scale = h->cfg_scale; a.ctx = h->max_new < 100 ? h->max_new : 100;
  a.rows = h->rows_set ? h->row_tab : nullptr;
  a.pairs = h->pairs_set ? 1 : 0;
  a.shift = h->prefix_set ? h->prefix_shift : nullptr;
  a.step0 = h->slots_open ? h->step0 : nullptr;
  return a;
}

static int enqueue_step(zn_handle h, const StepPlan& p, hipStream_t s) {
  const zn_config& c = h->cfg;
  int rc;
  const bool fused = p.fused_tail;
  if (!fused) {
    EmbedArgs e = make_embed_args(h);
    e.out = h->x;
    hipLaunchKernelGGL(embed_kernel, dim3(h->batch), dim3(256), 0, s, e);
  }
  if (c.arch == 1) {
    if ((rc = hybrid_token(h, true, p.attn_fused, s))) return rc;
  } else {
    bool heads_done = false;
    if (p.path == StepPlan::STACK) {
      if (!stack_pre(h) && (rc = layer_in_proj(h, 0, h->x_emb, (bf16_t*)h->kv_layers[0], h->max_len, h->lengths, h->rows, s))) return rc;
      if ((rc = launch_stack(h, s, h->rows, p.nbk))) return rc;
      heads_done = true;
    } else if ((rc = decode_blocks(h, p, nullptr, 0, s, fused ? h->x_emb : nullptr, &heads_done))) return rc;
    if (!heads_done && (rc = heads_logits(h, h->x, h->rows, s))) return rc;
  }
  SampleArgs a = gen_sample_args(h);
  a.raw = h->logits_raw; a.mix = guided(h) ? 1 : 0; a.apply_bias = 1; a.batch = h->batch;
  a.codes = h->codes; a.t_total = h->t_total;
  a.use_penalty = h->rows_set || (h->sp.repetition_penalty != 1.0f); a.st = h->st; a.logits_out = h->last_logits; a.tokens = h->tok_raw;
  a.draw = 1;
  FrameArgs& f = a.fr;
  f.st = h->st; f.codes = h->codes; f.t_total = h->t_total; f.batch = h->batch; f.n_q = c.n_codebooks; f.eos_id = c.eos_id;
  f.mask_id = c.mask_id; f.tokens = h->tok_raw; f.remaining = h->remaining; f.stopping = h->stopping; f.lengths = h->lengths;
  f.rows = h->rows; f.first = 0; f.override = h->tok_override; f.override_calls = h->tok_override_calls; f.shift = a.shift; f.step0 = a.step0;
  if (fused) { a.ticket = h->tail_ticket; a.em = make_embed_args(h); }
  const bool one_wg = fused && h->batch == 1 && !h->rows_set && h->tune[ZN_TUNE_SAMPLER] != 2 && (h->tune[ZN_TUNE_SAMPLER] == 3 || !(h->sp.temperature > 0.f)) && c.vocab_head <= 64 * ZN_S1_IT &&
                      c.n_codebooks <= 16 && !(h->sp.top_p > 0.f) && h->sp.top_k <= 0 && !(h->sp.linear > 0.f) &&
                      (!a.use_penalty || h->sp.repetition_penalty_window <= 16) && h->rows <= 1024;
  if (one_wg) { hipLaunchKernelGGL(sample1_kernel, dim3(1), dim3(1024), 0, s, a); return ZN_OK; }
  hipLaunchKernelGGL(sample_kernel, dim3(c.n_codebooks, h->batch), dim3(256), 0, s, a);
  if (!fused) hipLaunchKernelGGL(frame_update_kernel, dim3(1), dim3(256), 0, s, f);
  return ZN_OK;
}

extern "C" int zn_gen_begin(zn_handle h, int32_t batch, const void* const* kv_layers_dev, int32_t max_len, int32_t* lengths_dev,
                            int32_t* delayed_codes_dev, int32_t t_total, int32_t offset0, int32_t max_new_tokens, float cfg_scale,
                            const zn_sampling* sp, zn_stream stream) {
  if (!h) return ZN_ERR_ARG;
  if (!kv_layers_dev || !lengths_dev || !delayed_codes_dev || !sp) ZN_FAIL(h, ZN_ERR_ARG, "zn_gen_begin: null argument");
  if (!h->has_io) ZN_FAIL(h, ZN_ERR_STATE, "zn_gen_begin: handle was created without embeddings/heads");
  const int rows = cfg_scale == 1.0f ? batch : 2 * batch;
  if (batch < 1 || rows > h->max_rows) ZN_FAIL(h, ZN_ERR_ARG, "zn_gen_begin: batch %d needs %d rows, max_rows is %d", batch, rows, h->max_rows);
  if (max_len < 1 || t_total < 1 || offset0 < 1 || offset0 >= t_total) ZN_FAIL(h, ZN_ERR_ARG, "zn_gen_begin: bad lengths");
  if (max_len > h->cfg.rope_positions)
    ZN_FAIL(h, ZN_ERR_ARG, "sequence length %d exceeds the %d-position RoPE table (zonos/backbone/_torch.py:206)", max_len, h->cfg.rope_positions);
  if (sp->repetition_penalty_window < 0 || sp->repetition_penalty_window > 64) ZN_FAIL(h, ZN_ERR_ARG, "repetition_penalty_window out of range");
  hipStream_t s = (hipStream_t)stream;
  int rc = ensure_attn_ws(h, max_len);
  if (rc) return rc;
  free_graph(h);
  h->batch = batch; h->rows = rows; h->max_len = max_len; h->t_total = t_total; h->offset0 = offset0; h->max_new = max_new_tokens;
  h->cfg_scale = cfg_scale; h->sp = *sp;
  h->kv_layers.assign(kv_layers_dev, kv_layers_dev + h->cfg.n_layer);
  h->lengths = lengths_dev; h->codes = delayed_codes_dev;
  if (h->pending_hook == ZN_HOOK_TAG_WRAP) { h->epoch_bound = 0x70000001ull; h->pending_hook = 0; }
  if (h->epoch_bound > 0x70000000ull) {
    const size_t R = h->max_rows, nqkv = (size_t)(h->cfg.n_heads + 2 * h->cfg.n_heads_kv) * h->hd;
    for (unsigned long long* g : {h->ch_gy1, h->ch_gx1, h->ch_gx2, h->ch_ga}) HIPCHK(h, hipMemsetAsync(g, 0, R * (h->cfg.d_model / 2) * 8, s));
    HIPCHK(h, hipMemsetAsync(h->ch_gqkv, 0, R * (nqkv / 2 + 1) * 8, s));
    HIPCHK(h, hipMemsetAsync(h->ch_gm, 0, R * (h->cfg.d_ff / 2 + 1) * 8, s));
    HIPCHK(h, hipMemsetAsync(h->ch_gbmax, 0, (size_t)2 * h->cfg.n_heads_kv * ZN_SK_KB_MAXNB * 4 * 8, s));
    HIPCHK(h, hipMemsetAsync(h->ch_gpart, 0, (size_t)2 * h->cfg.n_heads_kv * ZN_SK_KB_MAXNB * ZN_SK_KB_PSZ * 8, s));
    const unsigned one = 1;
    HIPCHK(h, hipMemcpyAsync(h->ch_epoch, &one, sizeof one, hipMemcpyHostToDevice, s));
    HIPCHK(h, hipStreamSynchronize(s));
    h->epoch_bound = 1;
  }
  h->n_generations++;
  if (h->demoted && h->clean_since_demotion >= ZN_REARM_AFTER) { h->demoted = false; h->clean_since_demotion = 0; h->n_rearms++; }
  const bool persist_rows = h->cfg.arch == 0 && persist_shape(h, rows);
  if (h->demoted && persist_rows && h->tune[ZN_TUNE_PERSISTENT] != 2) h->n_fallback_generations++;
  h->persist_ok = !persist_rows || zn_tenant_try_claim(h->device, h) != 0;
  if (h->cfg.arch == 0 && h->ch_variant == 1) {
    if (!h->stack_checked) { h->stack_ok = stack_shapes_ok(h); h->stack_checked = true; }
    if (h->stack_ok) { int rc = build_stack_table(h); if (rc) return rc; }
  }
  GenState st{};
  st.offset = offset0; st.step = 0; st.all_done = 0; st.force_eos_step = h->force_eos_step; st.eos_bias = h->eos_bias;
  h->dbg_pause = 0;
  if (h->pending_hook == ZN_HOOK_PAUSE) { h->dbg_pause = 3000000u; h->pending_hook = 0; }
  if (h->pending_hook == ZN_HOOK_TIMEOUT_WORD) { st.pad[0] = 1; h->pending_hook = 0; }
  HIPCHK(h, hipMemcpyAsync(h->st, &st, sizeof st, hipMemcpyHostToDevice, s));
  std::vector<int> rem(batch, t_total - offset0), stop(batch, 0);
  HIPCHK(h, hipMemcpyAsync(h->remaining, rem.data(), batch * sizeof(int), hipMemcpyHostToDevice, s));
  HIPCHK(h, hipMemcpyAsync(h->stopping, stop.data(), batch * sizeof(int), hipMemcpyHostToDevice, s));
  std::vector<int> len0(rows, 0);
  HIPCHK(h, hipMemcpyAsync(len0.data(), lengths_dev, rows * sizeof(int), hipMemcpyDeviceToHost, s));
  HIPCHK(h, hipStreamSynchronize(s));
  h->len_hi = 0;
  for (int v : len0) if (v > h->len_hi) h->len_hi = v;
  h->gen_active = true;
  h->rows_set = false;
  h->pairs_set = false;
  h->prefix_set = false;
  h->slots_open = false;
  h->gen_prefilled = false;
  h->rows_unequal2 = false;
  h->gen_ended = false;
  h->gen_timed_out = false;
  h->gen_stream = s;
  h->stop_pending = false;
  h->emb_valid = false;
  return ZN_OK;
}

static int ensure_prefill_ws(zn_handle h, size_t M) {
  if (M <= h->pf_rows) return ZN_OK;
  const zn_config& c = h->cfg;
  for (bf16_t** p : {&h->pf_x, &h->pf_n, &h->pf_qkv, &h->pf_a, &h->pf_u, &h->pf_m, &h->pf_res, &h->pf_zx, &h->pf_xbc, &h->pf_y, &h->pf_g})
    if (*p) { (void)hipFree(*p); *p = nullptr; }
  h->pf_rows = 0;
  const size_t nqkv = (size_t)(c.n_heads + 2 * c.n_heads_kv) * h->hd;
  HIPCHK(h, hipMalloc(&h->pf_x, M * c.d_model * 2));
  HIPCHK(h, hipMalloc(&h->pf_n, M * c.d_model * 2));
  HIPCHK(h, hipMalloc(&h->pf_qkv, M * nqkv * 2));
  HIPCHK(h, hipMalloc(&h->pf_a, M * (size_t)c.n_heads * h->hd * 2));
  HIPCHK(h, hipMalloc(&h->pf_u, M * 2 * (size_t)c.d_ff * 2));
  HIPCHK(h, hipMalloc(&h->pf_m, M * (size_t)c.d_ff * 2));
  if (c.arch == 1) {
    HIPCHK(h, hipMalloc(&h->pf_res, M * c.d_model * 4));
    HIPCHK(h, hipMalloc(&h->pf_zx, M * (size_t)h->m_d_in_proj * 2));
    HIPCHK(h, hipMalloc(&h->pf_xbc, M * (size_t)h->m_conv_dim * 2));
    HIPCHK(h, hipMalloc(&h->pf_y, M * (size_t)c.m_d_inner * 2));
    HIPCHK(h, hipMalloc(&h->pf_g, M * (size_t)c.m_d_inner * 2));
  }
  h->pf_rows = M;
  return ZN_OK;
}

template <int HD>
static int launch_prefill_attn(const PrefillAttnArgs& a, int G, int R, bool mfma, hipStream_t s) {
  if constexpr (HD == 128) {
    if (mfma) {
      dim3 grid((a.S + 64 / G - 1) / (64 / G), a.n_heads_kv, R);
      switch (G) {
        case 1: hipLaunchKernelGGL((attn_prefill_mfma_kernel<1>), grid, dim3(256), 0, s, a); return 0;
        case 2: hipLaunchKernelGGL((attn_prefill_mfma_kernel<2>), grid, dim3(256), 0, s, a); return 0;
        case 4: hipLaunchKernelGGL((attn_prefill_mfma_kernel<4>), grid, dim3(256), 0, s, a); return 0;
        case 8: hipLaunchKernelGGL((attn_prefill_mfma_kernel<8>), grid, dim3(256), 0, s, a); return 0;
      }
    }
  }
  switch (G) {
#define ZN_PA(GG) case GG: hipLaunchKernelGGL((attn_prefill_kernel<HD, GG>), dim3((a.S + 64 / GG - 1) / (64 / GG), a.n_heads_kv, R), dim3(256), 0, s, a); return 0;
    ZN_PA(1) ZN_PA(2) ZN_PA(4) ZN_PA(8)
// ... 429 lines not shown
    hipLaunchKernelGGL(sample_kernel, dim3(nq, 1), dim3(256), 0, s, sa);
    FrameArgs f{};
    f.st = h->st; f.codes = h->codes; f.t_total = h->t_total; f.batch = B; f.n_q = nq; f.eos_id = c.eos_id;
    f.mask_id = c.mask_id; f.tokens = h->tok_raw; f.remaining = h->remaining; f.stopping = h->stopping; f.lengths = h->lengths;
    f.rows = h->rows; f.first = 1; f.shift = sa.shift; f.step0 = sa.step0; f.slot_base = a[j].slot; f.slot_count = 1;
    hipLaunchKernelGGL(frame_update_kernel, dim3(1), dim3(256), 0, s, f);
  }
  for (int j = 0; j < n; ++j) { h->slot_busy[a[j].slot] = 1; h->slot_len[a[j].slot] = a[j].row_len; }
  slots_len_hi(h);
  h->emb_valid = false;
  HIPCHK(h, hipGetLastError());
  return ZN_OK;
}

extern "C" int zn_gen_retire(zn_handle h, int32_t slot) {
  if (!h) return ZN_ERR_ARG;
  ZN_SESSION_CHECK(h, "zn_gen_retire");
  if (slot < 0 || slot >= h->batch) ZN_FAIL(h, ZN_ERR_ARG, "zn_gen_retire: slot %d out of range 0..%d", slot, h->batch - 1);
  if (!h->slot_busy[slot]) ZN_FAIL(h, ZN_ERR_STATE, "zn_gen_retire: slot %d is idle already", slot);
  hipStream_t s = h->gen_stream;
  HIPCHK(h, hipMemsetAsync(h->lengths + slot, 0, sizeof(int), s));
  if (guided(h)) HIPCHK(h, hipMemsetAsync(h->lengths + h->batch + slot, 0, sizeof(int), s));
  HIPCHK(h, hipMemsetAsync(h->remaining + slot, 0, sizeof(int), s));
  HIPCHK(h, hipMemsetAsync(h->step0 + slot, 0xFF, sizeof(int), s));
  h->slot_busy[slot] = 0; h->slot_len[slot] = 0;
  slots_len_hi(h);
  return ZN_OK;
}

extern "C" int zn_gen_row_state(zn_handle h, int32_t* remaining_host, int32_t* steps_host, zn_stream stream) {
  if (!h) return ZN_ERR_ARG;
  ZN_SESSION_CHECK(h, "zn_gen_row_state");
  hipStream_t s = (hipStream_t)stream;
  const int B = h->batch;
  std::vector<int> rem(B), s0(B);
  GenState st{};
  HIPCHK(h, hipMemcpyAsync(rem.data(), h->remaining, B * sizeof(int), hipMemcpyDeviceToHost, s));
  HIPCHK(h, hipMemcpyAsync(s0.data(), h->step0, B * sizeof(int), hipMemcpyDeviceToHost, s));
  HIPCHK(h, hipMemcpyAsync(&st, h->st, sizeof st, hipMemcpyDeviceToHost, s));
  HIPCHK(h, hipStreamSynchronize(s));
  for (int b = 0; b < B; ++b) {
    if (remaining_host) remaining_host[b] = rem[b];
    if (steps_host) steps_host[b] = s0[b] < 0 ? -1 : st.step - s0[b];
  }
  if (st.pad[0] != 0) return handoff_timeout(h, st.pad[0]);
  return ZN_OK;
}

extern "C" int zn_sample_first(zn_handle h, zn_stream stream) {
  if (!h) return ZN_ERR_ARG;
  if (!h->gen_active) ZN_FAIL(h, ZN_ERR_STATE, "zn_sample_first before zn_gen_begin");
  if (h->slots_open) ZN_FAIL(h, ZN_ERR_STATE, "zn_sample_first in a slotted session: zn_gen_admit samples each slot's first frame");
  hipStream_t s = (hipStream_t)stream;
  const zn_config& c = h->cfg;
  SampleArgs a = gen_sample_args(h);
  a.raw = h->logits_raw; a.mix = guided(h) ? 1 : 0; a.apply_bias = 0; a.batch = h->batch;
  a.use_penalty = 0; a.st = h->st; a.logits_out = h->last_logits; a.tokens = h->tok_raw; a.draw = 0;
  hipLaunchKernelGGL(sample_kernel, dim3(c.n_codebooks, h->batch), dim3(256), 0, s, a);
  FrameArgs f{};
  f.st = h->st; f.codes = h->codes; f.t_total = h->t_total; f.batch = h->batch; f.n_q = c.n_codebooks; f.eos_id = c.eos_id;
  f.mask_id = c.mask_id; f.tokens = h->tok_raw; f.remaining = h->remaining; f.stopping = h->stopping; f.lengths = h->lengths;
  f.rows = h->rows; f.first = 1; f.override = h->tok_override; f.override_calls = h->tok_override_calls; f.shift = a.shift;
  hipLaunchKernelGGL(frame_update_kernel, dim3(1), dim3(256), 0, s, f);
  h->emb_valid = false;
  HIPCHK(h, hipGetLastError());
  return ZN_OK;
}

extern "C" int zn_decode_steps(zn_handle h, int32_t n, zn_stream stream) {
  if (!h) return ZN_ERR_ARG;
  if (!h->gen_active || h->gen_ended) ZN_FAIL(h, ZN_ERR_STATE, "zn_decode_steps before zn_gen_begin");
  if (n < 0) ZN_FAIL(h, ZN_ERR_ARG, "n < 0");
  hipStream_t s = (hipStream_t)stream;
  h->gen_stream = s;
  if (h->slots_open)
    for (int b = 0; b < h->batch; ++b)
      if (h->slot_busy[b] && h->slot_len[b] + n > h->max_len)
        ZN_FAIL(h, ZN_ERR_STATE, "zn_decode_steps: %d steps would take slot %d (%d positions) past max_len %d: retire it first", n, b, h->slot_len[b], h->max_len);
  for (int i = 0; i < n;) {
    const StepPlan p = h->last_plan = plan_steps(h, n - i);
    const int k = p.graph_slot, run = p.run;
    if (p.fused_tail && !h->emb_valid) hipLaunchKernelGGL(embed_kernel, dim3(h->batch), dim3(256), 0, s, make_embed_args(h));
    h->emb_valid = p.fused_tail;
    if (!h->graph_exec[k] && !h->graph_tried[k] && n > 1) {
      h->graph_tried[k] = true;
      if (!h->cap_stream) (void)hipStreamCreateWithFlags(&h->cap_stream, hipStreamNonBlocking);
      hipStream_t cs = h->cap_stream; std::unique_lock<std::mutex> capturing(g_capture_mu);
      if (cs && hipStreamBeginCapture(cs, hipStreamCaptureModeThreadLocal) == hipSuccess) {
        int rc = ZN_OK;
        for (int j = 0; j < run && rc == ZN_OK; ++j) rc = enqueue_step(h, p, cs);
        hipGraph_t g = nullptr;
        hipError_t e = hipStreamEndCapture(cs, &g); capturing.unlock();
        if (rc == ZN_OK && e == hipSuccess && g && hipGraphInstantiate(&h->graph_exec[k], g, nullptr, nullptr, 0) == hipSuccess) h->graph[k] = g;
        else { if (g) (void)hipGraphDestroy(g); h->graph_exec[k] = nullptr; (void)hipGetLastError(); }
      } else (void)hipGetLastError();
    }
    if (h->graph_exec[k]) HIPCHK(h, hipGraphLaunch(h->graph_exec[k], s));
    else for (int j = 0; j < run; ++j) { int rc = enqueue_step(h, p, s); if (rc) return rc; }
    i += run; h->len_hi += run; h->epoch_bound += (unsigned long long)run * (h->cfg.n_layer + 1);
  }
  if (h->slots_open) {
    for (int b = 0; b < h->batch; ++b) if (h->slot_busy[b]) h->slot_len[b] += n;
    slots_len_hi(h);
  }
  HIPCHK(h, hipGetLastError());
  return ZN_OK;
}

extern "C" int zn_gen_end(zn_handle h) {
  if (!h) return ZN_ERR_ARG;
  (void)zn_tenant_release(h->device, h);
  if (h->gen_active && !h->gen_ended && h->demoted && !h->gen_timed_out) h->clean_since_demotion++;
  h->gen_ended = true;
  return ZN_OK;
}

extern "C" int zn_get_counters(zn_handle h, int64_t* out, int32_t n) {
  if (!h || !out || n < 0) return ZN_ERR_ARG;
  unsigned w[2] = {0, 0};
  if (n > 6 && h->ch_diag) HIPCHK(h, ZN_NOT_IN_CAPTURE(hipMemcpy(w, h->ch_diag + 8, sizeof w, hipMemcpyDeviceToHost)));
  const long long v[8] = {h->n_timeouts, h->n_generations, h->n_fallback_generations, h->demoted ? 1 : 0, h->n_rearms, h->clean_since_demotion, (long long)(w[0] / 100u), (long long)w[1]};
  for (int i = 0; i < n && i < 8; ++i) out[i] = v[i];
  return ZN_OK;
}

extern "C" int zn_decode_path_detail(zn_handle h) {
  if (!h || !h->gen_active || h->cfg.arch != 0 || !persist_active(h, h->rows)) return 0;
  return h->last_plan.path == StepPlan::STACK ? 2 : chain_allowed(h, h->rows) ? 1 : 0;
}
extern "C" int zn_decode_path(zn_handle h) { return zn_decode_path_detail(h) != 0 ? 1 : 0; }
extern "C" int zn_graph_active(zn_handle h) {
  if (!h) return 0;
  for (int k = 0; k < ZN_NGRAPHS; ++k) if (h->graph_exec[k]) return 1;
  return 0;
}

static int handoff_timeout(zn_handle h, int count) {
  if (h->gen_stream) (void)hipStreamSynchronize(h->gen_stream);
  (void)ZN_NOT_IN_CAPTURE(hipMemcpy(h->diag_host, h->ch_diag, sizeof h->diag_host, hipMemcpyDeviceToHost));
  (void)ZN_NOT_IN_CAPTURE(hipMemset(h->ch_diag, 0, 32));
  (void)ZN_NOT_IN_CAPTURE(hipMemset(&h->st->pad[0], 0, sizeof(int)));
  h->demoted = true; h->clean_since_demotion = 0; h->n_timeouts++; h->gen_timed_out = true;
  free_graph(h);
  const unsigned* d = h->diag_host;
  ZN_FAIL(h, ZN_ERR_HIP, "decode chain: %d hand-off wait(s) timed out - the results of this generation are invalid. First: stage %u of block %u, workgroup %u wave %u lane %u "
          "waited for tag %u, granule at byte %u carried tag %u after %u passes. This handle runs the launches path for its next %d generations (zn_debug_tune(8, 1) re-arms the persistent kernels at once; zn_get_counters)",
          count, d[0] >> 8, d[0] & 255u, d[1], d[2], d[6], d[3], d[4], d[5], d[7], ZN_REARM_AFTER);
}

extern "C" int zn_all_stopped(zn_handle h, int32_t* out, zn_stream stream) {
  if (!h || !out) return ZN_ERR_ARG;
  hipStream_t s = (hipStream_t)stream;
  HIPCHK(h, hipMemcpyAsync(h->done_host, &h->st->all_done, 4 * sizeof(int), hipMemcpyDeviceToHost, s));
  HIPCHK(h, hipStreamSynchronize(s));
  *out = h->done_host[0];
  if (h->done_host[3] != 0) return handoff_timeout(h, h->done_host[3]);
  return ZN_OK;
}

extern "C" int zn_all_stopped_begin(zn_handle h, zn_stream stream) {
  if (!h) return ZN_ERR_ARG;
  hipStream_t s = (hipStream_t)stream;
  HIPCHK(h, hipMemcpyAsync(h->done_host + 4, &h->st->all_done, 4 * sizeof(int), hipMemcpyDeviceToHost, s));
  HIPCHK(h, hipEventRecord(h->stop_event, s));
  h->stop_pending = true;
  return ZN_OK;
}
extern "C" int zn_all_stopped_end(zn_handle h, int32_t* out) {
  if (!h || !out) return ZN_ERR_ARG;
  if (!h->stop_pending) ZN_FAIL(h, ZN_ERR_STATE, "zn_all_stopped_end without zn_all_stopped_begin");
  HIPCHK(h, hipEventSynchronize(h->stop_event));
  h->stop_pending = false;
  *out = h->done_host[4];
  if (h->done_host[7] != 0) return handoff_timeout(h, h->done_host[7]);
  return ZN_OK;
}

extern "C" int zn_get_step_outputs(zn_handle h, float* logits_dev, int32_t* tokens_dev, zn_stream stream) {
  if (!h) return ZN_ERR_ARG;
  hipStream_t s = (hipStream_t)stream;
  const zn_config& c = h->cfg;
  if (logits_dev) HIPCHK(h, hipMemcpyAsync(logits_dev, h->last_logits, (size_t)h->batch * c.n_codebooks * c.vocab_head * sizeof(float), hipMemcpyDeviceToDevice, s));
  if (tokens_dev) HIPCHK(h, hipMemcpyAsync(tokens_dev, h->tok_raw, (size_t)h->batch * c.n_codebooks * sizeof(int), hipMemcpyDeviceToDevice, s));
  return ZN_OK;
}

extern "C" int zn_codes_changed(zn_handle h) { if (!h) return ZN_ERR_ARG; h->emb_valid = false; return ZN_OK; }
extern "C" int zn_debug_force_eos(zn_handle h, int32_t step) { if (!h) return ZN_ERR_ARG; h->force_eos_step = step; return ZN_OK; }
extern "C" int zn_debug_token_override(zn_handle h, const int32_t* tokens_dev, int32_t calls) {
  if (!h) return ZN_ERR_ARG;
  h->tok_override = tokens_dev; h->tok_override_calls = tokens_dev ? calls : 0;
  free_graph(h);
  return ZN_OK;
}
extern "C" int zn_debug_tune(zn_handle h, int32_t key, int32_t value) {
  if (!h || key < 0 || key >= ZN_TUNE_NKEYS || value < 1) return ZN_ERR_ARG;
  if (key == ZN_TUNE_HOOK && value == ZN_HOOK_RESET_WAIT_STATS) {
    if (h->ch_diag) { (void)hipDeviceSynchronize(); (void)ZN_NOT_IN_CAPTURE(hipMemset(h->ch_diag + 8, 0, 2 * sizeof(unsigned))); }
    return ZN_OK;
  }
  (key == ZN_TUNE_HOOK ? h->pending_hook : h->tune[key]) = value; free_graph(h); h->emb_valid = false;
  if (key == ZN_TUNE_PERSISTENT && value == 1 && h->demoted) { h->demoted = false; h->clean_since_demotion = 0; h->n_rearms++; }
  return ZN_OK;
}
extern "C" int zn_debug_trace(zn_handle h, void* trace_dev) {
  if (!h) return ZN_ERR_ARG;
  h->dbg_trace = (bf16_t*)trace_dev; free_graph(h);
  return ZN_OK;
}
extern "C" int zn_debug_chain_stamps(zn_handle h, uint64_t* stamps_dev) {
  if (!h) return ZN_ERR_ARG;
  h->ch_stamps = (unsigned long long*)stamps_dev; free_graph(h);
// ... 338 lines not shown
```

### zonos_amd/csrc/zn_chain_kernel.h

```cpp
#pragma once
#include <utility>
#include "zn_decode_kernels.h"

#ifndef ZN_CH_DEFER_MASK
#define ZN_CH_DEFER_MASK 0xF
#endif
#define ZN_CH_CWAVES 4
#ifndef ZN_CH_NBUF
#define ZN_CH_NBUF 3
#endif
#define ZN_CH_THREADS ((ZN_CH_CWAVES + 2) * 64)
#ifndef ZN_CH_SWEEP_DELAY
#define ZN_CH_SWEEP_DELAY 40
#endif
#ifndef ZN_SWEEP_BACKOFF
#define ZN_SWEEP_BACKOFF 0
#endif
#ifdef ZN_TIMING_STREAM_ONLY
#define ZN_TIMING_PASS(bad) (bad) = 0ull
#else
#define ZN_TIMING_PASS(bad) (void)0
#endif
#define ZN_CH_TIMEOUT_TICKS 2000000ull
#define ZN_CH_TIMEOUT_PASSES 4096u

struct ChainArgs {
  const bf16_t *W_out, *W_fc1, *W_fc2, *W_in;
  const bf16_t *ln2_w, *ln2_b, *lnn_w, *lnn_b;
  float eps;
  int F, nqkv;
  float* heads_out;
  const bf16_t* a;
  const bf16_t* xin;
  bf16_t* xout;
  unsigned long long *g_y1, *g_x1, *g_x2;
  unsigned long long* g_m;
  bf16_t* q_out; bf16_t* kv; const float* rope; const int* lengths;
  int max_len, hd, n_heads, n_heads_kv, rope_positions;
  unsigned* epoch;
  int* tmo;
  unsigned long long* stamps;
  const struct StackLayer* layers;
  int n_layer, stamp_layer;
  unsigned long long *g_qkv, *g_a;
  const bf16_t* q0;
  float scale;
  int heads_rows;
  bf16_t* trace;
  unsigned* diag;
  unsigned dbg_pause;
  int natt;
  unsigned long long* g_bmax;
  unsigned long long* g_part;
  const bf16_t *pre_W, *pre_ln_w, *pre_ln_b;
  bf16_t* pre_kv;
};
struct StackLayer {
  const bf16_t *W_out, *W_fc1, *W_fc2, *W_in;
  const bf16_t *ln2_w, *ln2_b, *lnn_w, *lnn_b;
  const bf16_t* kv;
  bf16_t* kv_next;
};

template <int I, int N, class Fn> ZN_DEVINL void zn_static_for(Fn&& f) {
  if constexpr (I < N) { f(std::integral_constant<int, I>{}); zn_static_for<I + 1, N>(f); }
}
ZN_DEVINL u32x4 ld_sc1_16(__amdgpu_buffer_rsrc_t rs, int byte_off) { return __builtin_amdgcn_raw_buffer_load_b128(rs, byte_off, 0, 16); }
ZN_DEVINL u32x2 ld_sc1_8(__amdgpu_buffer_rsrc_t rs, int byte_off) { return __builtin_amdgcn_raw_buffer_load_b64(rs, byte_off, 0, 16); }
ZN_DEVINL __amdgpu_buffer_rsrc_t zn_rsrc(const void* p) { return __builtin_amdgcn_make_buffer_rsrc((void*)p, 0, 0x7fffffff, 0x00020000); }
ZN_DEVINL void st_sc1_u32(void* p, unsigned v) { __hip_atomic_store((unsigned*)p, v, __ATOMIC_RELAXED, __HIP_MEMORY_SCOPE_AGENT); }
ZN_DEVINL unsigned ld_sc1_u32(const void* p) { return __hip_atomic_load((const unsigned*)p, __ATOMIC_RELAXED, __HIP_MEMORY_SCOPE_AGENT); }
ZN_DEVINL unsigned dpp_movu(unsigned v, int) { return v; }
template <int CTRL> ZN_DEVINL unsigned dpp_u(unsigned v) { return (unsigned)__builtin_amdgcn_update_dpp(0, (int)v, CTRL, 0xF, 0xF, true); }

ZN_DEVINL void st_granule(unsigned long long* g, unsigned tag, unsigned value) {
  __hip_atomic_store(g, ((unsigned long long)tag << 32) | value, __ATOMIC_RELAXED, __HIP_MEMORY_SCOPE_AGENT);
}
struct SweepWho { unsigned code; unsigned* diag; };
template <int N, class OffFn>
ZN_DEVINL bool sweep_granules_at(__amdgpu_buffer_rsrc_t rs, OffFn off, unsigned tag, u32x4 (&data)[N], int* tmo, int lane, SweepWho who, unsigned* passes_out = nullptr) {
  const unsigned long long t0 = __builtin_amdgcn_s_memrealtime();
  unsigned np = 0;
  for (;;) {
    ++np;
    bool ok = true;
#pragma unroll
    for (int i = 0; i < N; ++i) {
      const int o = off(i);
      const u32x4 l0 = ld_sc1_16(rs, o), l1 = ld_sc1_16(rs, o + 16);
      ok &= (l0.y == tag) & (l0.w == tag) & (l1.y == tag) & (l1.w == tag);
      data[i] = u32x4{l0.x, l0.z, l1.x, l1.z};
    }
    unsigned long long bad = __builtin_amdgcn_ballot_w64(!ok);
    ZN_TIMING_PASS(bad);
    if (bad == 0ull) { if (passes_out) *passes_out = np; return true; }
    if constexpr (ZN_SWEEP_BACKOFF > 0) __builtin_amdgcn_s_sleep(ZN_SWEEP_BACKOFF);
    if ((np >= ZN_CH_TIMEOUT_PASSES && __builtin_amdgcn_s_memrealtime() - t0 > ZN_CH_TIMEOUT_TICKS) || __hip_atomic_load(tmo, __ATOMIC_RELAXED, __HIP_MEMORY_SCOPE_AGENT) != 0) {
      if (lane == (int)__builtin_ctzll(bad) && atomicAdd(tmo, 1) == 0 && who.diag) {
        unsigned badoff = 0xffffffffu, badtag = 0;
#pragma unroll
        for (int i = N - 1; i >= 0; --i) {
          const int o = off(i);
          const u32x4 l0 = ld_sc1_16(rs, o), l1 = ld_sc1_16(rs, o + 16);
          if (l1.w != tag) { badoff = o + 24; badtag = l1.w; }
          if (l1.y != tag) { badoff = o + 16; badtag = l1.y; }
          if (l0.w != tag) { badoff = o + 8; badtag = l0.w; }
          if (l0.y != tag) { badoff = o; badtag = l0.y; }
        }
        who.diag[0] = who.code; who.diag[1] = blockIdx.x; who.diag[2] = threadIdx.x >> 6; who.diag[3] = tag;
        who.diag[4] = badoff; who.diag[5] = badtag; who.diag[6] = (unsigned)lane; who.diag[7] = np;
      }
      return false;
    }
  }
}
template <int N>
ZN_DEVINL bool sweep_granules(__amdgpu_buffer_rsrc_t rs, const int (&off)[N], unsigned tag, u32x4 (&data)[N], int* tmo, int lane, SweepWho who, unsigned* passes_out = nullptr) {
  return sweep_granules_at<N>(rs, [&](int i) { return off[i]; }, tag, data, tmo, lane, who, passes_out);
}

template <int DEPTH>
ZN_DEVINL bool sweep_granules_piped(__amdgpu_buffer_rsrc_t rs, int off, unsigned tag, u32x4& data, int* tmo, int lane, SweepWho who) {
  const unsigned long long t0 = __builtin_amdgcn_s_memrealtime();
  unsigned np = 0;
  u32x4 l0[DEPTH], l1[DEPTH];
#pragma unroll
  for (int d = 0; d < DEPTH; ++d) { l0[d] = ld_sc1_16(rs, off); l1[d] = ld_sc1_16(rs, off + 16); }
  for (;;) {
#pragma unroll
    for (int d = 0; d < DEPTH; ++d) {
      ++np;
      const u32x4 a0 = l0[d], a1 = l1[d];
      const bool ok = (a0.y == tag) & (a0.w == tag) & (a1.y == tag) & (a1.w == tag);
      unsigned long long bad = __builtin_amdgcn_ballot_w64(!ok);
      ZN_TIMING_PASS(bad);
      if (bad == 0ull) { data = u32x4{a0.x, a0.z, a1.x, a1.z}; return true; }
      if ((np >= ZN_CH_TIMEOUT_PASSES && __builtin_amdgcn_s_memrealtime() - t0 > ZN_CH_TIMEOUT_TICKS) || __hip_atomic_load(tmo, __ATOMIC_RELAXED, __HIP_MEMORY_SCOPE_AGENT) != 0) {
        if (lane == (int)__builtin_ctzll(bad) && atomicAdd(tmo, 1) == 0 && who.diag) {
// ... 282 lines not shown
```

### zonos_amd/csrc/zn_decode_kernels.h

```cpp
#pragma once
#include "zn_common.h"
#include "../../include/zonos_hip.h"
#include "zn_linear_plan.h"


struct GemvArgs {
  const bf16_t* W;
  int N, K, nrows;
  int units;
  int upw;
  const bf16_t* x;
  const bf16_t *ln_w, *ln_b;
  float eps;
  const float* gv;
  const int* lengths;
  int hd, n_heads;
  bf16_t* out;
  const bf16_t* resid;
  const bf16_t* bias;
  float* out_f32;
  bf16_t* q_out;
  bf16_t* kv;
  const float* rope;
  int max_len, n_heads_kv, rope_positions;
// ... 1641 lines not shown
        s3 = block_sum(s3, sv);
        for (int i = tid; i < V; i += 256) sp[i] = sp[i] / s3;
        __syncthreads();
      }
      if (top_k > 0) {
        const int kk = top_k < V ? top_k : V;
        const float pivot = sp[kk - 1];
        __syncthreads();
        float s4 = 0.f;
        for (int i = tid; i < V; i += 256) { if (sp[i] < pivot) sp[i] = 0.f; s4 += sp[i]; }
        s4 = block_sum(s4, sv);
        for (int i = tid; i < V; i += 256) sp[i] = sp[i] / s4;
        __syncthreads();
      }
    } else {
      for (int i = tid; i < V; i += 256) sidx[i] = i;
      __syncthreads();
    }
    if (min_p > 0.f) {
      float m3 = 0.f;
      for (int i = tid; i < V; i += 256) m3 = fmaxf(m3, sp[i]);
      m3 = block_max(m3, sv);
      float s5 = 0.f;
      for (int i = tid; i < V; i += 256) { if (sp[i] < min_p * m3) sp[i] = 0.f; s5 += sp[i]; }
      s5 = block_sum(s5, sv);
      for (int i = tid; i < V; i += 256) sp[i] = sp[i] / s5;
      __syncthreads();
    }
    if (a.probs_out) for (int i = tid; i < V; i += 256) a.probs_out[((size_t)b * a.n_q + cb) * V + sidx[i]] = sp[i];
    float bv = -1.f; int bi = 0x7fffffff;
    for (int i = tid; i < V; i += 256) {
      const int tokid = sidx[i];
      unsigned long long h = zn_mix64(seed ^ zn_mix64(a.draw + (a.st ? (unsigned long long)(a.st->step - step_b0) : 0ull)));
      h = zn_mix64(h + 0x9E3779B97F4A7C15ull * (unsigned long long)((key_b * a.n_q + cb) * V + tokid + 1));
      const float uu = ((float)(h >> 40) + 0.5f) * (1.0f / 16777216.0f);
      const float q = -logf(uu);
      const float v = sp[i] / q;
      if (v > bv || (v == bv && tokid < bi)) { bv = v; bi = tokid; }
    }
    float rv; int ri;
    block_argmax(bv, bi, sv, si, rv, ri);
    tok = ri == 0x7fffffff ? 0 : ri;
  }
  if (!a.ticket) {
    if (tid == 0) a.tokens[b * a.n_q + cb] = tok;
    return;
  }
  __shared__ int s_last;
  __shared__ int s_code[ZN_TAIL_MAXB][ZN_FRAME_MAXQ];
  if (tid == 0) __hip_atomic_store(a.tokens + b * a.n_q + cb, tok, __ATOMIC_RELAXED, __HIP_MEMORY_SCOPE_AGENT);
  __builtin_amdgcn_s_waitcnt(0);
  __syncthreads();
  if (tid == 0) {
    const int n = (int)(gridDim.x * gridDim.y);
    const int t = __hip_atomic_fetch_add(a.ticket, 1, __ATOMIC_RELAXED, __HIP_MEMORY_SCOPE_AGENT);
    s_last = (t == n - 1);
    if (s_last) __hip_atomic_store(a.ticket, 0, __ATOMIC_RELAXED, __HIP_MEMORY_SCOPE_AGENT);
  }
  __syncthreads();
  if (!s_last) return;
  frame_update_body<true>(a.fr, s_code);
  __syncthreads();
  for (int ub = 0; ub < a.fr.batch; ++ub) {
    int code[ZN_EMBED_MAXQ];
#pragma unroll
    for (int i = 0; i < ZN_EMBED_MAXQ; ++i) {
      const int c = s_code[ub][min(i, a.em.n_q - 1)];
      code[i] = c < 0 ? 0 : (c >= a.em.vocab_embed ? a.em.vocab_embed - 1 : c);
    }
    embed_row(a.em, ub, code);
  }
}

#define ZN_S1_IT 17
template <typename F> ZN_DEVINL float s1_sum(const float (&x)[ZN_S1_IT], int lane, int V, F keep) {
  float part[4] = {0.f, 0.f, 0.f, 0.f};
#pragma unroll
  for (int j = 0; j < ZN_S1_IT; ++j) if (lane + 64 * j < V) part[j & 3] += keep(x[j]);
  float t = 0.f;
#pragma unroll
  for (int w = 0; w < 4; ++w) t += wave_sum(part[w]);
  return t;
}
ZN_DEVINL void s1_argmax(float& v, int& i) {
#pragma unroll
  for (int o = 32; o > 0; o >>= 1) {
    const float ov = __shfl_xor(v, o);
    const int oi = __shfl_xor(i, o);
    if (ov > v || (ov == v && oi < i)) { v = ov; i = oi; }
  }
}
__global__ __launch_bounds__(1024) void sample1_kernel(SampleArgs a) {
  const int tid = threadIdx.x, lane = tid & 63, cb = tid >> 6;
  const int V = a.V, nq = a.n_q;
  __shared__ int s_tok[ZN_FRAME_MAXQ];
  __shared__ int s_code[ZN_FRAME_MAXQ];
  const FrameArgs& fr = a.fr;
  const int o = a.st->offset, stp = a.st->step;
  const float st_bias = a.st->eos_bias;
  const bool st_force = a.st->force_eos_step == stp;
  float cc[ZN_S1_IT], uu[ZN_S1_IT];
  const bool on = cb < nq;
  const int cbq = on ? cb : nq - 1;
  const float* rc = a.raw + (size_t)cbq * V;
  const float* ru = a.raw + (size_t)((a.mix ? 1 : 0) * nq + cbq) * V;
#pragma unroll
  for (int j = 0; j < ZN_S1_IT; ++j) {
    const int i = min(lane + 64 * j, V - 1);
    cc[j] = rc[i];
    uu[j] = ru[i];
  }
  int nw = 0, hist_tok = -1;
  if (a.use_penalty && a.codes) {
    const int avail = o + 1 < a.ctx ? o + 1 : a.ctx;
    nw = avail < a.pen_window ? avail : a.pen_window;
    if (lane < nw) hist_tok = a.codes[(size_t)cbq * a.t_total + (o + 1 - nw) + lane];
  }
  const int fcb = tid & (ZN_FRAME_MAXQ - 1), fcbc = min(fcb, nq - 1);
  const int col = o + 1;
  const bool in_range = fcb < nq && col < fr.t_total;
  int* cell = fr.codes + (size_t)fcbc * fr.t_total + min(col, fr.t_total - 1);
  const int call = stp + 1;
  const bool ovr = fr.override && call < fr.override_calls;
  int cur = 0, rem = 0, stop = 0, otok = 0, otok0 = 0;
  if (tid < ZN_FRAME_MAXQ) {
    cur = *cell; rem = fr.remaining[0]; stop = fr.stopping[0];
    if (ovr) { otok = fr.override[(size_t)call * nq + fcbc]; otok0 = fr.override[(size_t)call * nq]; }
  }
  int tok = 0;
  if (on) {
    float l[ZN_S1_IT];
#pragma unroll
    for (int j = 0; j < ZN_S1_IT; ++j) {
      const int i = lane + 64 * j;
      float x = a.mix ? __fadd_rn(uu[j], __fmul_rn(__fsub_rn(cc[j], uu[j]), a.cfg_scale)) : cc[j];
      if (a.apply_bias && i == a.eos_id) {
        if (cb == 0) {
          x = __fadd_rn(x, -0.6931471824645996f);
          x += st_bias;
          if (st_force) x = 1.0e4f;
        } else x = -INFINITY;
      }
      if (a.logits_out && i < V) a.logits_out[(size_t)cb * V + i] = x;
      l[j] = x;
    }
    for (int w = 0; w < nw; ++w) {
      int g = __shfl(hist_tok, w);
      if (g < 0) continue;
      g = g > V - 1 ? V - 1 : g;
      bool seen = false;
      float f = 1.f;
      for (int w2 = 0; w2 < nw; ++w2) {
        int g2 = __shfl(hist_tok, w2);
        g2 = g2 > V - 1 ? V - 1 : g2;
        if (g2 == g) { if (w2 < w) seen = true; else f = __fmul_rn(f, a.penalty); }
      }
      if (seen) continue;
#pragma unroll
      for (int j = 0; j < ZN_S1_IT; ++j)
        if (lane + 64 * j == g) l[j] = (l[j] <= 0.f) ? __fmul_rn(l[j], f) : __fdiv_rn(l[j], f);
    }
    if (!(a.temperature > 0.f)) {
      float bv = -INFINITY; int bi = 0x7fffffff;
#pragma unroll
      for (int j = 0; j < ZN_S1_IT; ++j) { const int i = lane + 64 * j; if (i < V && l[j] > bv) { bv = l[j]; bi = i; } }
      s1_argmax(bv, bi);
      tok = bi == 0x7fffffff ? 0 : bi;
    } else {
      float mx = -INFINITY;
#pragma unroll
      for (int j = 0; j < ZN_S1_IT; ++j) { l[j] = l[j] / a.temperature; if (lane + 64 * j < V) mx = fmaxf(mx, l[j]); }
      mx = wave_max(mx);
#pragma unroll
      for (int j = 0; j < ZN_S1_IT; ++j) l[j] = expf(l[j] - mx);
      const float ssum = s1_sum(l, lane, V, [](float e) { return e; });
#pragma unroll
      for (int j = 0; j < ZN_S1_IT; ++j) l[j] = l[j] / ssum;
      if (a.min_p > 0.f) {
        float m3 = 0.f;
#pragma unroll
        for (int j = 0; j < ZN_S1_IT; ++j) if (lane + 64 * j < V) m3 = fmaxf(m3, l[j]);
        m3 = wave_max(m3);
        const float thr = a.min_p * m3;
#pragma unroll
        for (int j = 0; j < ZN_S1_IT; ++j) if (l[j] < thr) l[j] = 0.f;
        const float s5 = s1_sum(l, lane, V, [](float e) { return e; });
#pragma unroll
        for (int j = 0; j < ZN_S1_IT; ++j) l[j] = l[j] / s5;
      }
      if (a.probs_out) {
#pragma unroll
        for (int j = 0; j < ZN_S1_IT; ++j) { const int i = lane + 64 * j; if (i < V) a.probs_out[(size_t)cb * V + i] = l[j]; }
      }
      const unsigned long long h0 = zn_mix64(a.seed ^ zn_mix64(a.draw + (unsigned long long)stp));
      float bv = -1.f; int bi = 0x7fffffff;
#pragma unroll
      for (int j = 0; j < ZN_S1_IT; ++j) {
        const int i = lane + 64 * j;
        if (i < V) {
          const unsigned long long h = zn_mix64(h0 + 0x9E3779B97F4A7C15ull * (unsigned long long)((size_t)cb * V + i + 1));
          const float u01 = ((float)(h >> 40) + 0.5f) * (1.0f / 16777216.0f);
          const float v = l[j] / (-logf(u01));
          if (v > bv || (v == bv && i < bi)) { bv = v; bi = i; }
        }
      }
      s1_argmax(bv, bi);
      tok = bi == 0x7fffffff ? 0 : bi;
    }
    if (lane == 0) { s_tok[cb] = tok; a.tokens[cb] = tok; }
  }
  __syncthreads();
  if (tid < ZN_FRAME_MAXQ) {
    const int tk = ovr ? otok : s_tok[fcbc], tk0 = ovr ? otok0 : s_tok[0];
    if (tk0 == fr.eos_id) { rem = rem < nq ? rem : nq; stop = 1; }
    int eos_idx = nq - rem; if (eos_idx > nq - 1) eos_idx = nq - 1;
    int t = tk;
    if (stop && fcb < eos_idx) t = fr.mask_id; else if (stop && fcb == eos_idx) t = fr.eos_id;
    if (in_range && cur == -1) *cell = t;
    s_code[fcb] = (in_range && cur == -1) ? t : cur;
    rem -= 1;
    if (fcb == 0) {
      fr.remaining[0] = rem; fr.stopping[0] = stop;
      a.st->offset = o + 1; a.st->step = stp + 1; a.st->all_done = rem > 0 ? 0 : 1;
    }
  }
  if (tid < fr.rows) fr.lengths[tid] += 1;
  __syncthreads();
  if (tid < 256) {
    int code[ZN_EMBED_MAXQ];
#pragma unroll
    for (int i = 0; i < ZN_EMBED_MAXQ; ++i) {
      const int c = s_code[min(i, a.em.n_q - 1)];
      code[i] = c < 0 ? 0 : (c >= a.em.vocab_embed ? a.em.vocab_embed - 1 : c);
    }
    embed_row(a.em, 0, code);
  }
}
```

### zonos_amd/csrc/zn_step_kernel.h

```cpp
#pragma once
#include "zn_chain_kernel.h"
#include "zn_step_sched.h"

#define ZN_SK_THREADS 512
#ifndef ZN_SK_CW
#define ZN_SK_CW 6
#endif
#define ZN_SK_HELPERS (8 - (ZN_SK_CW + 2))
#ifndef ZN_SK_NBUF
#define ZN_SK_NBUF 3
#endif
#ifndef ZN_SK_PARK
#define ZN_SK_PARK (ZN_SK_CW == 4 ? 4 : 2)
#endif
#ifndef ZN_SK_HELP
#define ZN_SK_HELP 0
#endif
#ifndef ZN_SK_HELP_AT
#define ZN_SK_HELP_AT 0
#endif
#ifndef ZN_SK_EARLY
#define ZN_SK_EARLY 0
#endif
#ifndef ZN_SK_MSWEEP_DELAY
#define ZN_SK_MSWEEP_DELAY 0
#endif
#ifndef ZN_SK_SWEEP_DELAY
#define ZN_SK_SWEEP_DELAY 32
#endif
#define ZN_SK_DYN_LDS (ZN_SK_CW * ZN_SK_PARK * 8192)
static_assert(ZN_SK_CW == 4 || ZN_SK_CW == 6, "4 compute waves + 2 helper waves, or 6 compute waves");
static_assert(ZN_SK_DYN_LDS + 26 * 1024 <= 160 * 1024, "parked tiles + the streaming role's static LDS fit a CU");
static_assert(ZN_SK_CW == 4 || ZN_SK_DYN_LDS >= 2 * 4 * 2048 * 2, "fc2's input [2][4 d_model] is staged in the parked tiles' LDS");
#ifndef ZN_SK_APOLL
#define ZN_SK_APOLL 1
#endif
#ifndef ZN_SK_XDELAY
#define ZN_SK_XDELAY 16
#endif
#ifndef ZN_SK_XDELAY_NB
#define ZN_SK_XDELAY_NB 5
#endif
#ifndef ZN_SK_PACE_MARGIN
#define ZN_SK_PACE_MARGIN 0
#endif
#ifndef ZN_SK_PACE_SHIFT
#define ZN_SK_PACE_SHIFT 2
#endif

#ifndef ZN_SK_PACE_CAP
#define ZN_SK_PACE_CAP 8192u
#endif
#define ZN_SK_LONG_WAIT 20000u
struct StepPacer {
  unsigned long long t_ref; unsigned prev;
  unsigned worst = 0, n_long = 0;
  ZN_DEVINL void start() { t_ref = __builtin_amdgcn_s_memrealtime(); }
  ZN_DEVINL void sleep() const {
#ifdef ZN_TIMING_STREAM_ONLY
    return;
#endif
    const unsigned long long until = t_ref + (ZN_SK_PACE_MARGIN > 0 ? (prev > ZN_SK_PACE_MARGIN ? prev - ZN_SK_PACE_MARGIN : 0u) : (prev - (prev >> ZN_SK_PACE_SHIFT)));
    while (__builtin_amdgcn_s_memrealtime() < until) __builtin_amdgcn_s_sleep(8);
  }
  ZN_DEVINL void done() {
    const unsigned long long d = __builtin_amdgcn_s_memrealtime() - t_ref;
    prev = d < ZN_SK_PACE_CAP ? (unsigned)d : ZN_SK_PACE_CAP;
    const unsigned du = d < 0xffffffffull ? (unsigned)d : 0xffffffffu;
    worst = du > worst ? du : worst;
    n_long += du > ZN_SK_LONG_WAIT ? 1u : 0u;
  }
  ZN_DEVINL void report(unsigned* diag, int lane) const {
    if (lane == 0 && diag) { if (worst > ZN_SK_LONG_WAIT / 2) atomicMax(diag + 8, worst); if (n_long) atomicAdd(diag + 9, n_long); }
  }
};
ZN_DEVINL void step_debug_pause(unsigned ticks) {
  const unsigned long long t0 = __builtin_amdgcn_s_memrealtime();
  while (__builtin_amdgcn_s_memrealtime() - t0 < ticks) __builtin_amdgcn_s_sleep(127);
}

#define ZN_SK_KB_MAXNB 12
#define ZN_SK_KB_PSZ 520
struct StepKbLds {
  float sc[4][512];
  float bm[8][4];
  float bmall[ZN_SK_KB_MAXNB][4];
  float accw[8][4][128];
  float l[8][4];
  __attribute__((aligned(16))) bf16_t p[4][512];
  __attribute__((aligned(16))) bf16_t q[4][128];
  __attribute__((aligned(16))) bf16_t knew[128], vnew[128];
  __attribute__((aligned(16))) bf16_t out[4][128];
};
static_assert(sizeof(StepKbLds) <= ZN_SK_DYN_LDS, "the key-block attention role's LDS fits the launch's dynamic LDS");

template <int CH, int DEPTH>
ZN_DEVINL void kb_combine_chunk(__amdgpu_buffer_rsrc_t rs_part, int voff, int loff, int j0, int nb, unsigned tag, const float (*bmall)[4], int g,
                                float& tot0, float& tot1, float& lt, float& mprev, int* tmo, int lane, SweepWho who) {
  constexpr int PSZ8 = ZN_SK_KB_PSZ * 8;
  u32x4 pv[DEPTH][CH];
  u32x2 pl[DEPTH][CH];
  auto issue = [&](auto DC) {
    constexpr int d = decltype(DC)::value;
#pragma unroll
    for (int j = 0; j < CH; ++j) {
      const int jo = min(j0 + j, nb - 1) * PSZ8;
      pv[d][j] = ld_sc1_16(rs_part, voff + jo);
      pl[d][j] = ld_sc1_8(rs_part, loff + jo);
    }
  };
  zn_static_for<0, DEPTH>([&](auto DC) { issue(DC); });
  SpinBound sb; sb.begin();
  int got = -1;
  while (got < 0) {
    zn_static_for<0, DEPTH>([&](auto DC) {
      constexpr int d = decltype(DC)::value;
      if (got >= 0) return;
      ++sb.np;
      bool ok = true;
#pragma unroll
      for (int j = 0; j < CH; ++j) ok &= (pv[d][j].y == tag) & (pv[d][j].w == tag) & (pl[d][j].y == tag);
      unsigned long long bad = __builtin_amdgcn_ballot_w64(!ok);
      ZN_TIMING_PASS(bad);
      if (bad == 0ull) { got = d; return; }
      if (sb.give_up(tmo)) {
        unsigned badoff = 0, badtag = 0;
#pragma unroll
        for (int j = CH - 1; j >= 0; --j) {
          const bool okj = (pv[d][j].y == tag) & (pv[d][j].w == tag) & (pl[d][j].y == tag);
          if (!okj) { badoff = (unsigned)(voff + min(j0 + j, nb - 1) * PSZ8); badtag = pv[d][j].y != tag ? pv[d][j].y : pv[d][j].w != tag ? pv[d][j].w : pl[d][j].y; }
        }
        sb.report(tmo, who, bad, lane, tag, badoff, badtag);
        got = d;
        return;
      }
      issue(DC);
    });
  }
  zn_static_for<0, DEPTH>([&](auto DC) {
    constexpr int d = decltype(DC)::value;
    if (got != d) return;
#pragma unroll
    for (int j = 0; j < CH; ++j) {
      if (j0 + j < nb) {
        const float mj = fmaxf(mprev, bmall[j0 + j][g]);
        const float fj = (j0 + j == 0) ? 0.f : expf(mprev - mj);
        mprev = mj;
        tot0 = __fadd_rn(__fmul_rn(tot0, fj), __uint_as_float(pv[d][j].x));
        tot1 = __fadd_rn(__fmul_rn(tot1, fj), __uint_as_float(pv[d][j].z));
        lt = __fadd_rn(__fmul_rn(lt, fj), __uint_as_float(pl[d][j].x));
      }
    }
  });
}

template <int NBV, int R>
ZN_DEVINL void step_attention_kb_role(const ChainArgs& a, StepKbLds& S, const unsigned tag0, const int c, const int wave, const int lane_in) {
  static_assert(NBV >= 1 && NBV <= ZN_SK_KB_MAXNB, "blocks covered");
  constexpr int HD = 128, G = 4, NW = 8, KST = HD / 32, TPW = 4, MAXNB = ZN_SK_KB_MAXNB, PSZ = ZN_SK_KB_PSZ;
  typedef __attribute__((ext_vector_type(4))) float f32x4_t;
  const int npairs = a.n_heads_kv * R;
  const int pair = c % npairs, jb = c / npairs, kvh = pair % a.n_heads_kv, ar = pair / a.n_heads_kv;
  const int nq = a.n_heads * HD, nk = a.n_heads_kv * HD, D = nq;
  const int L = a.lengths[ar] + 1, nb = (L + 511) >> 9;
  if (jb >= nb) return;
  const int tb = jb * 512, nkeys = min(512, L - tb), tend = tb + nkeys;
  const bool has_newest = jb == nb - 1;
  const int hi = L >= 2 ? L - 2 : 0;
  const size_t kvrow = (size_t)2 * nk;
  const bool stamped = a.stamps && c == 0 && wave == 0 && lane_in == 0;
  u32x4 kk[TPW][KST];
  AttnV<HD> V;
  const int rowbytes = (int)kvrow * 2;
  auto issue_kv = [&](const bf16_t* kv, int opq, int ln) {
    const int kn = ln & 15, kg = ln >> 4;
    const __amdgpu_buffer_rsrc_t rs = zn_rsrc(kv);
    const int kbase = ar * a.max_len * rowbytes + (kvh * HD + 8 * kg) * 2, kr0 = opq + tb + wave * 16 + kn;
#pragma unroll
    for (int tl = 0; tl < TPW; ++tl)
#pragma unroll
      for (int st = 0; st < KST; ++st) kk[tl][st] = __builtin_amdgcn_raw_buffer_load_b128(rs, kbase + min(kr0 + tl * NW * 16, hi) * rowbytes + 64 * st, 0, 0);
    const int vbase = ar * a.max_len * rowbytes + ((a.n_heads_kv + kvh) * HD + kn * 8) * 2, vr0 = opq + tb + wave * 64 + 8 * kg;
#pragma unroll
    for (int ks = 0; ks < 2; ++ks)
#pragma unroll
      for (int j = 0; j < 8; ++j) {
        const u32x4 x = __builtin_amdgcn_raw_buffer_load_b128(rs, vbase + min(vr0 + 32 * ks + j, hi) * rowbytes, 0, 0);
        V.v[ks][j][0] = x.x; V.v[ks][j][1] = x.y; V.v[ks][j][2] = x.z; V.v[ks][j][3] = x.w;
      }
  };
  issue_kv(a.layers[0].kv, 0, lane_in);
  const __amdgpu_buffer_rsrc_t rs_bmax = zn_rsrc(a.g_bmax), rs_part = zn_rsrc(a.g_part);
  StepPacer pace{0ull, 0u};
  pace.start();
#pragma unroll 1
  for (int li = 0; li < a.n_layer; ++li) {
    const unsigned tag = tag0 + 1u + (unsigned)li;
    if (a.dbg_pause && li == 3) step_debug_pause(a.dbg_pause);
    const bool st_on = stamped && li == a.stamp_layer;
    auto stamp = [&](int i) { if (st_on) a.stamps[32 + i] = __builtin_amdgcn_s_memrealtime(); };
    stamp(0);
    int lane = lane_in;
    asm volatile("" : "+v"(lane));
    const int kn = lane & 15, kg = lane >> 4, vsub = lane & 3;
    const int tid = wave * 64 + lane;
    if (wave == ZN_SK_CW || (wave == ZN_SK_CW + 1 && has_newest)) {
      const bool first = wave == ZN_SK_CW;
      if (li == 0 && !a.pre_W) {
        if (first) *(u32x4*)&S.q[lane >> 4][(lane & 15) * 8] = ld16(a.q0 + ((size_t)ar * a.n_heads + kvh * G + (lane >> 4)) * HD + (lane & 15) * 8);
        else if (lane < 32) {
          const bf16_t* rowp = a.layers[0].kv + ((size_t)ar * a.max_len + (L - 1)) * kvrow + (size_t)(lane < 16 ? 0 : nk) + (size_t)kvh * HD + (lane & 15) * 8;
          const u32x4 v = ld16(rowp);
          if (lane < 16) *(u32x4*)&S.knew[lane * 8] = v; else *(u32x4*)&S.vnew[(lane - 16) * 8] = v;
        }
      } else {
        const int qoff = (ar * (a.nqkv / 2) + ((kvh * G) * HD) / 2 + lane * 4) * 8;
        const int kvsel = lane < 16 ? nq + kvh * HD : nq + nk + kvh * HD;
        const int koff = (ar * (a.nqkv / 2) + kvsel / 2 + (lane & 15) * 4) * 8;
        u32x4 d1[1];
        pace.sleep();
        sweep_granules_piped<ZN_SK_APOLL>(zn_rsrc(a.g_qkv), first ? qoff : koff, tag - 1u, d1[0], a.tmo, lane, SweepWho{(5u << 8) | (unsigned)li, a.diag});
        pace.done();
        if (first) *(u32x4*)&S.q[lane >> 4][(lane & 15) * 8] = d1[0];
        else if (lane < 16) *(u32x4*)&S.knew[lane * 8] = d1[0];
        else if (lane < 32) *(u32x4*)&S.vnew[(lane - 16) * 8] = d1[0];
      }
    }
    __syncthreads();
    stamp(1);
    {
      zn_bf16x8 qa[KST];
#pragma unroll
      for (int st = 0; st < KST; ++st) {
        u32x4 v = u32x4{0, 0, 0, 0};
        if (kn < G) v = *(const u32x4*)&S.q[kn][32 * st + 8 * kg];
        qa[st] = __builtin_bit_cast(zn_bf16x8, v);
      }
      u32x4 knew_frag[KST];
// ... 55 lines not shown
            const bool ok = !act || ((v.y == tag) & (v.w == tag));
            unsigned long long bad = __builtin_amdgcn_ballot_w64(!ok);
            ZN_TIMING_PASS(bad);
            if (bad == 0ull) {
              if (act) { S.bmall[lane >> 1][2 * (lane & 1)] = __uint_as_float(v.x); S.bmall[lane >> 1][2 * (lane & 1) + 1] = __uint_as_float(v.z); }
              done = true;
            } else if (sb.give_up(a.tmo)) {
              sb.report(a.tmo, SweepWho{(7u << 8) | (unsigned)li, a.diag}, bad, lane, tag, (unsigned)off + (v.y != tag ? 0u : 8u), v.y != tag ? v.y : v.w);
              done = true;
            } else pv_[d] = ld_sc1_16(rs_bmax, off);
          }
        }
      } else if (lane < G) S.bmall[0][lane] = bmx;
    }
    __syncthreads();
    stamp(3);
    {
      float m_run = -INFINITY;
      for (int j = 0; j < jb; ++j) m_run = fmaxf(m_run, S.bmall[j][vsub]);
      const float mnew[1] = {fmaxf(m_run, S.bmall[jb][vsub])};
      attn_block_probs<G>(S.sc, mnew, nkeys, nkeys & ~15, S.p, S.l, wave, lane);
    }
    __syncthreads();
    if (has_newest && ((L - 1 - tb) >> 6) == wave) {
      const u32x4 vnew_piece = *(const u32x4*)&S.vnew[8 * kn];
#pragma unroll
      for (int ks = 0; ks < 2; ++ks)
#pragma unroll
        for (int j = 0; j < 8; ++j)
          if (tb + wave * 64 + 32 * ks + 8 * kg + j == L - 1) { V.v[ks][j][0] = vnew_piece.x; V.v[ks][j][1] = vnew_piece.y; V.v[ks][j][2] = vnew_piece.z; V.v[ks][j][3] = vnew_piece.w; }
    }
    attn_block_pv<HD, G>(S.p, V, S.accw, wave, lane);
    __syncthreads();
    stamp(4);
    {
      const int g = tid >> 7, d = tid & 127;
      float v = 0.f, l = 0.f;
#pragma unroll
      for (int w = 0; w < NW; ++w) v += S.accw[w][g][d];
#pragma unroll
      for (int w = 0; w < NW; ++w) l += S.l[w][g];
      if (nb == 1) S.out[g][d] = f2bf(__fmul_rn(v, 1.0f / l));
      else {
        unsigned long long* pp = a.g_part + ((size_t)pair * MAXNB + jb) * PSZ;
        st_granule(pp + g * 128 + d, tag, __float_as_uint(v));
        if (d == 0) st_granule(pp + G * 128 + g, tag, __float_as_uint(l));
      }
    }
    if (nb == 1) __syncthreads();
    stamp(5);
    if (wave < 4 && (nb == 1 || jb == 0)) {
      const int p = tid, g = p >> 6, dp = p & 63;
      unsigned o;
      if (nb == 1) o = *(const unsigned*)&S.out[g][2 * dp];
      else {
        const int voff = ((pair * MAXNB) * PSZ + g * 128 + 2 * dp) * 8, loff = ((pair * MAXNB) * PSZ + G * 128 + g) * 8;
        float tot0 = 0.f, tot1 = 0.f, lt = 0.f, mprev = -INFINITY;
        const SweepWho who{(8u << 8) | (unsigned)li, a.diag};
        if (ZN_SK_XDELAY > 0 && nb >= ZN_SK_XDELAY_NB) __builtin_amdgcn_s_sleep(ZN_SK_XDELAY);
        if (nb <= 2) kb_combine_chunk<2, ZN_SK_APOLL>(rs_part, voff, loff, 0, nb, tag, S.bmall, g, tot0, tot1, lt, mprev, a.tmo, lane, who);
        else if (nb <= 4) kb_combine_chunk<4, 2>(rs_part, voff, loff, 0, nb, tag, S.bmall, g, tot0, tot1, lt, mprev, a.tmo, lane, who);
        else {
#pragma unroll
          for (int j0 = 0; j0 < NBV; j0 += 6)
            if (j0 < nb) kb_combine_chunk<6, 1>(rs_part, voff, loff, j0, nb, tag, S.bmall, g, tot0, tot1, lt, mprev, a.tmo, lane, who);
        }
        const float inv = 1.0f / lt;
        o = pack2(__fmul_rn(tot0, inv), __fmul_rn(tot1, inv));
      }
      st_granule(a.g_a + (size_t)ar * (D / 2) + ((kvh * G + g) * HD) / 2 + dp, tag, o);
      if (a.trace) *(unsigned*)(a.trace + ((size_t)(8 * li + 1) * R + ar) * D + (kvh * G + g) * HD + 2 * dp) = o;
    }
    if (a.trace && jb == 0 && wave == ZN_SK_CW)
      *(u32x4*)(a.trace + ((size_t)(8 * li + 2) * R + ar) * D + (kvh * G + (lane >> 4)) * HD + (lane & 15) * 8) = *(const u32x4*)&S.q[lane >> 4][(lane & 15) * 8];
    stamp(6);
    if (li + 1 < a.n_layer) {
      int opq = 0;
      asm volatile("" : "+v"(opq));
      issue_kv(a.layers[li + 1].kv, opq, lane);
    }
    pace.start();
  }
  if (wave == ZN_SK_CW) pace.report(a.diag, lane_in);
}

template <int R, int NCH, int T_OUT, int T_FC1, int T_FC2, int T_IN, int NBV>
ZN_DEVINL void step_body(const ChainArgs& a) {
  static_assert(R == 1 || R == 2, "one or two activation rows");
  constexpr int D = NCH * 512, CW = ZN_SK_CW;
  constexpr int NS = 2 * T_OUT + T_FC1 + T_FC2 + T_IN;
  constexpr int NOPS = 5;
  constexpr int MASK = ZN_CH_DEFER_MASK;
  constexpr int NB = ZN_SK_NBUF, P = ZN_SK_PARK;
  constexpr int NL = NS - T_OUT;
  static_assert(T_IN > 0 && NCH == 4, "step_kernel: d_model 2048, head size 128");
  static_assert(P >= T_OUT && NB >= 2 && P + NB <= NL, "op 0's tiles are parked (op 1 reads them again); the prefetch stays inside the block");
  const int tid = threadIdx.x, lane = tid & 63, wave = __builtin_amdgcn_readfirstlane(tid >> 6);
  const int c = blockIdx.x;
  const int F = a.F;
  const unsigned tag0 = ld_sc1_u32(a.epoch);
  extern __shared__ __attribute__((aligned(16))) unsigned char zn_dyn_lds[];
  const int natt = a.natt;
  if (c < natt) {
    step_attention_kb_role<NBV, R>(a, *reinterpret_cast<StepKbLds*>(zn_dyn_lds), tag0, c, wave, lane);
    return;
  }
  __shared__ __attribute__((aligned(16))) bf16_t s_act[R * D];
  __shared__ float s_res[2][64][2][R];
  __shared__ __attribute__((aligned(16))) bf16_t s_ln[4 * D];
  const int sc = c - natt, NSW = (int)gridDim.x - natt;
  auto split = [&](int U, int& n, int& start) { const int base = U / NSW, extra = U % NSW; n = base + (sc < extra ? 1 : 0); start = sc * base + min(sc, extra); };
  int n_out, s_out, ng1, sg1;
  split(D / 2, n_out, s_out);
  split(F / 2, ng1, sg1);
  const int n_fc1 = 2 * ng1, s_fc1 = 2 * sg1;
  int n_qkv, s_qkv, n_hd, s_hd;
  split((a.nqkv + 1) / 2, n_qkv, s_qkv);
  split((a.heads_rows + 1) / 2, n_hd, s_hd);
  constexpr bool MLDS = CW != 4;
  constexpr int NBAR = 14 + (MLDS ? 1 : 0);
  __shared__ int s_pf[2];
  constexpr int NPW = ZN_SK_HELPERS > 0 ? ZN_SK_HELPERS : CW;
  constexpr int NPT = (10 + NPW - 1) / NPW;
  const bool pre = a.pre_W != nullptr;
  if (tid < 2) s_pf[tid] = 0;
  __syncthreads();

  using SC = StepSched<T_OUT, T_FC1, T_FC2, T_IN, NB, P, ZN_SK_HELP, MASK, ZN_SK_EARLY>;
  auto op_of = [](int s) constexpr { return SC::op_of(s); };
  auto first_of = [](int op) constexpr { return SC::first_of(op); };

  constexpr int L_F2 = SC::L_F2;
  constexpr int NH = ZN_SK_HELP;
  static_assert(NH >= 0 && NH <= T_OUT && NH < T_FC1 - (P - T_OUT), "helper tiles take the slots of op 0's tiles");
  static_assert(NH == 0 || ZN_SK_HELPERS == 2, "helper tiles need the two helper waves");
  constexpr int NREG = SC::NREG;
  auto slot_of_load = [](int l) constexpr { return SC::slot_of_load(l); };
  struct WT { u32x4 a[NCH], b[NCH]; };
  struct LW { const bf16_t *out, *fc1, *fc2, *in; };
  auto tile_of = [&](const LW& Lr, int rows_in, int n_in, int s_in, int s, int w, bool& ok, const bf16_t*& pa, const bf16_t*& pb, int& ridx) {
    const int op = op_of(s), t = s - first_of(op);
    if (op == 3) {
      const int i = w + CW * t, qt = i & 3, j = i >> 2;
      ok = j < n_out;
      const int u = s_out + (ok ? j : 0);
      pa = Lr.fc2 + (size_t)(2 * u) * (4 * D) + qt * D + lane * 8;
      pb = pa + 4 * D;
      ridx = j * 4 + qt;
      return;
    }
    const int j = w + CW * t;
    const int n = op <= 1 ? n_out : op == 2 ? n_fc1 : n_in;
    const int st = op <= 1 ? s_out : op == 2 ? s_fc1 : s_in;
    ok = j < n;
    const int u = st + (ok ? j : 0);
    ridx = j;
    if (op <= 1) { pa = Lr.out + (size_t)(2 * u) * D + lane * 8; pb = pa + D; }
    else if (op == 2) { pa = Lr.fc1 + (size_t)u * D + lane * 8; pb = pa + (size_t)F * D; }
    else { pa = Lr.in + (size_t)(2 * u) * D + lane * 8; pb = (2 * u + 1 < rows_in) ? pa + D : pa; }
  };
  auto park_of = [&](int w) { return reinterpret_cast<u32x4*>(zn_dyn_lds) + (size_t)w * (P * 2 * NCH * 64) + lane; };

  auto pre_contract = [&](int pw) {
    WT pt[NPT];
#pragma unroll
    for (int t = 0; t < NPT; ++t) {
      const int j = pw + NPW * t;
      if (j < n_qkv) {
        const int u = s_qkv + j;
        const bf16_t* pa = a.pre_W + (size_t)(2 * u) * D + lane * 8;
        const bf16_t* pb = (2 * u + 1 < a.nqkv) ? pa + D : pa;
#pragma unroll
        for (int c2 = 0; c2 < NCH; ++c2) { pt[t].a[c2] = ld_nt16(pa + c2 * 512); pt[t].b[c2] = ld_nt16(pb + c2 * 512); }
      }
    }
    while (__hip_atomic_load(&s_pf[0], __ATOMIC_ACQUIRE, __HIP_MEMORY_SCOPE_WORKGROUP) < R) __builtin_amdgcn_s_sleep(1);
    u32x4 xr[NCH][R];
#pragma unroll
    for (int c2 = 0; c2 < NCH; ++c2)
#pragma unroll
      for (int r = 0; r < R; ++r) xr[c2][r] = *(const u32x4*)&s_act[r * D + (c2 * 64 + lane) * 8];
#pragma unroll
    for (int t = 0; t < NPT; ++t) {
      const int j = pw + NPW * t;
      if (j < n_qkv) {
        float accA[R] = {}, accB[R] = {};
#pragma unroll
        for (int c2 = 0; c2 < NCH; ++c2) {
#pragma unroll
          for (int r = 0; r < R; ++r) { accA[r] = dot8(pt[t].a[c2], xr[c2][r], accA[r]); accB[r] = dot8(pt[t].b[c2], xr[c2][r], accB[r]); }
        }
#pragma unroll
        for (int r = 0; r < R; ++r) { accA[r] = wave_sum(accA[r]); accB[r] = wave_sum(accB[r]); }
        if (lane == 0) {
// ... 218 lines not shown
      __syncthreads();
    }
    return;
  }

  const int myr = wave - CW;
  if constexpr (R == 1) {
    if (myr >= R) {
#pragma unroll 1
      for (int li = 0; li < a.n_layer; ++li)
#pragma unroll
        for (int b = 0; b < NBAR; ++b) __syncthreads();
      return;
    }
  }
  const bool epi = myr == 0;
  u32x4 g[NCH];
  const int ij = lane >> 1, ir = lane & 1;
  const bool it_out = epi && ij < n_out && ir < R;
  const int u_out = s_out + (it_out ? ij : 0);
  unsigned resid = 0;
  if (it_out) resid = *(const unsigned*)(a.xin + (size_t)ir * D + 2 * u_out);
  const int nq = a.n_heads * a.hd, nk = a.n_heads_kv * a.hd;
  const bool it_qkv = epi && ij < n_qkv && ir < R;
  const int u_qkv = s_qkv + (it_qkv ? ij : 0);
  int pos = 0; float cs = 1.f, sn = 0.f;
  if (it_qkv) {
    pos = a.lengths[ir];
    const int rowA = 2 * u_qkv;
    if (rowA < nq + nk) {
      const int i = (rowA % a.hd) >> 1;
      const int p = pos < a.rope_positions ? pos : a.rope_positions - 1;
      const float2 c2v = *(const float2*)(a.rope + ((size_t)p * (a.hd >> 1) + i) * 2);
      cs = c2v.x; sn = c2v.y;
    }
  }
  int goff[NCH];
#pragma unroll
  for (int c2 = 0; c2 < NCH; ++c2) goff[c2] = (myr * (D / 2) + (c2 * 64 + lane) * 4) * 8;
  unsigned x1own = 0;
  if (pre) {
    u32x4 lw[NCH], lb[NCH];
#pragma unroll
    for (int c2 = 0; c2 < NCH; ++c2) {
      g[c2] = ld16(a.xin + (size_t)myr * D + (c2 * 64 + lane) * 8);
      lw[c2] = ld16(a.pre_ln_w + (c2 * 64 + lane) * 8);
      lb[c2] = ld16(a.pre_ln_b + (c2 * 64 + lane) * 8);
    }
    chain_layernorm_row<NCH>(g, lw, lb, a.eps);
#pragma unroll
    for (int c2 = 0; c2 < NCH; ++c2) *(u32x4*)&s_act[myr * D + (c2 * 64 + lane) * 8] = g[c2];
    if (lane == 0) __hip_atomic_fetch_add(&s_pf[0], 1, __ATOMIC_RELEASE, __HIP_MEMORY_SCOPE_WORKGROUP);
    while (__hip_atomic_load(&s_pf[1], __ATOMIC_ACQUIRE, __HIP_MEMORY_SCOPE_WORKGROUP) < NPW) __builtin_amdgcn_s_sleep(1);
    if (it_qkv) {
      const int rowA = 2 * u_qkv;
      const float x0 = bfround(s_res[0][ij][0][ir]), x1 = bfround(s_res[0][ij][1][ir]);
      unsigned packed;
      if (rowA < nq + nk) {
        float re, im;
        zn_rope_pair(x0, x1, cs, sn, re, im);
        packed = pack2(re, im);
      } else packed = pack2(x0, x1);
      st_granule(a.g_qkv + (size_t)ir * (a.nqkv / 2) + u_qkv, tag0, packed);
      if (rowA >= nq && pos < a.max_len) {
        const int which = rowA < nq + nk ? 0 : 1, colk = rowA - nq - which * nk;
        *(unsigned*)(a.pre_kv + (((size_t)ir * a.max_len + pos) * 2 + which) * nk + colk) = packed;
      }
    }
  }
  StepPacer pace{0ull, 0u};
  pace.start();
#pragma unroll 1
  for (int li = 0; li < a.n_layer; ++li) {
    const StackLayer& Lr = a.layers[li];
    const bool last = li + 1 == a.n_layer;
    const unsigned tag = tag0 + 1u + (unsigned)li;
    const bool stamped = a.stamps && li == a.stamp_layer && epi && sc == 0 && lane == 0;
    int nst = 0;
    auto stamp = [&]() { if (stamped) a.stamps[nst] = __builtin_amdgcn_s_memrealtime(); ++nst; };
    stamp();
    int opq = 0;
    asm volatile("" : "+v"(opq));
    const int irq = ir + opq, uoq = u_out + opq, uqq = u_qkv + opq;
    pace.sleep();
    stamp();
    sweep_granules<NCH>(zn_rsrc(a.g_a), goff, tag, g, a.tmo, lane, SweepWho{(6u << 8) | (unsigned)li, a.diag});
    pace.done();
#pragma unroll
    for (int c2 = 0; c2 < NCH; ++c2) *(u32x4*)&s_act[myr * D + (c2 * 64 + lane) * 8] = g[c2];
    __syncthreads();
    stamp();
    zn_static_for<0, NOPS>([&](auto OC) {
      constexpr int op = decltype(OC)::value;
      constexpr int par = op & 1;
      __syncthreads();
      stamp();
      if constexpr (op == 0) {
        if (it_out) st_granule(a.g_y1 + (size_t)irq * (D / 2) + uoq, tag, pack2(s_res[par][ij][0][ir], s_res[par][ij][1][ir]));
      } else if constexpr (op == 1) {
        if (it_out) {
          x1own = pack2(lo_f(resid) + bfround(s_res[par][ij][0][ir]), hi_f(resid) + bfround(s_res[par][ij][1][ir]));
          st_granule(a.g_x1 + (size_t)irq * (D / 2) + uoq, tag, x1own);
        }
      } else if constexpr (op == 2) {
        const bool on = lane < n_fc1;
        const int jj = on ? lane : 0;
        const float y = bfround(s_res[par][jj][0][myr]), gt = bfround(s_res[par][jj][1][myr]);
        const float sg = bfround(gt / (1.0f + expf(-gt)));
        const unsigned mine = (unsigned)f2bf(y * sg);
        const unsigned nbv = (unsigned)__shfl_down((int)mine, 1);
        if (on && (lane & 1) == 0) st_granule(a.g_m + (size_t)(myr + opq) * (F / 2) + ((s_fc1 + lane) >> 1), tag, mine | (nbv << 16));
      } else if constexpr (op == 3) {
        if (it_out) {
          const float vA = ((s_res[par][ij * 4 + 0][0][ir] + s_res[par][ij * 4 + 1][0][ir]) + s_res[par][ij * 4 + 2][0][ir]) + s_res[par][ij * 4 + 3][0][ir];
          const float vB = ((s_res[par][ij * 4 + 0][1][ir] + s_res[par][ij * 4 + 1][1][ir]) + s_res[par][ij * 4 + 2][1][ir]) + s_res[par][ij * 4 + 3][1][ir];
          const unsigned o = pack2(lo_f(x1own) + bfround(vA), hi_f(x1own) + bfround(vB));
          st_granule(a.g_x2 + (size_t)irq * (D / 2) + uoq, tag, o);
          if (last) *(unsigned*)(a.xout + (size_t)irq * D + 2 * uoq) = o;
          if (a.trace) *(unsigned*)(a.trace + ((size_t)(8 * li) * R + irq) * D + 2 * uoq) = o;
          resid = o;
        }
      } else {
        if (last) {
          if (epi && ij < n_hd && ir < R) {
            const int u = s_hd + ij;
            a.heads_out[(size_t)irq * a.heads_rows + 2 * u] = bfround(s_res[par][ij][0][ir]);
            if (2 * u + 1 < a.heads_rows) a.heads_out[(size_t)irq * a.heads_rows + 2 * u + 1] = bfround(s_res[par][ij][1][ir]);
          }
        } else if (it_qkv) {
          const int rowA = 2 * u_qkv;
          const float x0 = bfround(s_res[par][ij][0][ir]), x1 = bfround(s_res[par][ij][1][ir]);
          unsigned packed;
          if (rowA < nq + nk) {
            float re, im;
            zn_rope_pair(x0, x1, cs, sn, re, im);
            packed = pack2(re, im);
          } else packed = pack2(x0, x1);
          st_granule(a.g_qkv + (size_t)irq * (a.nqkv / 2) + uqq, tag, packed);
          if (rowA >= nq && pos < a.max_len) {
            const int which = rowA < nq + nk ? 0 : 1, colk = rowA - nq - which * nk;
            *(unsigned*)(Lr.kv_next + (((size_t)irq * a.max_len + pos) * 2 + which) * nk + colk) = packed;
          }
        }
      }
      __syncthreads();
      stamp();
      if constexpr (op + 1 < NOPS) {
        if constexpr (op != 2) {
          if constexpr (ZN_SK_SWEEP_DELAY > 0) __builtin_amdgcn_s_sleep(ZN_SK_SWEEP_DELAY);
          sweep_granules<NCH>(zn_rsrc(op == 0 ? a.g_y1 : op == 1 ? a.g_x1 : a.g_x2), goff, tag, g, a.tmo, lane,
                              SweepWho{((op == 0 ? 1u : op == 1 ? 2u : 4u) << 8) | (unsigned)li, a.diag});
          stamp();
          if constexpr (op == 1 || op == 3) {
            u32x4 lw[NCH], lb[NCH];
#pragma unroll
            for (int c2 = 0; c2 < NCH; ++c2) {
              lw[c2] = *(const u32x4*)&s_ln[(op == 1 ? 0 : 2) * D + (c2 * 64 + lane) * 8];
              lb[c2] = *(const u32x4*)&s_ln[(op == 1 ? 1 : 3) * D + (c2 * 64 + lane) * 8];
            }
            chain_layernorm_row<NCH>(g, lw, lb, a.eps);
          }
#pragma unroll
          for (int c2 = 0; c2 < NCH; ++c2) *(u32x4*)&s_act[myr * D + (c2 * 64 + lane) * 8] = g[c2];
          __syncthreads();
        } else {
          if constexpr (MLDS) __syncthreads();
          stamp();
        }
        stamp();
      }
    });
    if (a.dbg_pause && li == 2) step_debug_pause(a.dbg_pause);
    pace.start();
  }
  pace.report(a.diag, lane);
  if (epi && sc == 0 && lane == 0) st_sc1_u32(a.epoch, tag0 + 1u + (unsigned)a.n_layer);
}

#define ZN_SK_DETACH_ARGS(a, a_in) \
  ChainArgs a = a_in;                \
  asm volatile("" : "+s"(a.max_len), "+s"(a.hd), "+s"(a.n_heads), "+s"(a.n_heads_kv), "+s"(a.rope_positions), "+s"(a.F), "+s"(a.nqkv), "+s"(a.natt), "+s"(a.dbg_pause))

template <int NCH, int T_OUT, int T_FC1, int T_FC2, int T_IN, int NBV>
__global__ __launch_bounds__(ZN_SK_THREADS) void step_kernel(ChainArgs a_in) {
  ZN_SK_DETACH_ARGS(a, a_in);
  step_body<2, NCH, T_OUT, T_FC1, T_FC2, T_IN, NBV>(a);
}

template <int NCH, int T_OUT, int T_FC1, int T_FC2, int T_IN, int NBV>
__global__ __launch_bounds__(ZN_SK_THREADS) void step_r1_kernel(ChainArgs a_in) {
  ZN_SK_DETACH_ARGS(a, a_in);
  step_body<1, NCH, T_OUT, T_FC1, T_FC2, T_IN, NBV>(a);
}
```

Baseline: 13.86 audio-sec/sec.

## Fuse greedy sampling and frame update into the persistent stack kernel tail

Moves the per-step sampling tail into the persistent stack decode kernel for the greedy single-WG case. CFG mixing, EOS bias, repetition penalty and a partial argmax run on each workgroup's head outputs, and the candidates are published via tagged granules. One workgroup then reduces them, updates the frame and codes, and embeds the next token. This removes the separate sample1_kernel launch and the round trip of logits through global memory. The cost is extra cross-workgroup spin synchronisation, a device-side SampleArgs record refreshed from the host when it changes, and more complexity in the kernel epilogue.

```diff
diff --git a/include/zonos_hip.h b/include/zonos_hip.h
--- a/include/zonos_hip.h
+++ b/include/zonos_hip.h
@@ -115,6 +115,7 @@
 int zn_graph_active(zn_handle h);
 int zn_decode_path(zn_handle h);
 int zn_decode_path_detail(zn_handle h);
+int zn_step_tail_in_kernel(zn_handle h);
 int zn_get_counters(zn_handle h, int64_t* out, int32_t n);
 int zn_gen_end(zn_handle h);
 int zn_tenant_try_claim(int32_t device, const void* owner);
@@ -145,7 +146,7 @@
   ZN_TUNE_HOOK = 14,
   ZN_TUNE_WHOLE_STEP = 15,
   ZN_TUNE_SAMPLER = 16,
-  ZN_TUNE_RESERVED_17 = 17,
+  ZN_TUNE_STEP_TAIL = 17,
   ZN_TUNE_STACK_PRE = 18,
   ZN_TUNE_ATTN_SPLIT_COLS = 19,
   ZN_TUNE_NKEYS = 20
diff --git a/zonos_amd/_lib.py b/zonos_amd/_lib.py
--- a/zonos_amd/_lib.py
+++ b/zonos_amd/_lib.py
@@ -22,7 +22,7 @@
 ZN_TUNE_HOOK = 14
 ZN_TUNE_WHOLE_STEP = 15
 ZN_TUNE_SAMPLER = 16
-ZN_TUNE_RESERVED_17 = 17
+ZN_TUNE_STEP_TAIL = 17
 ZN_TUNE_STACK_PRE = 18
 ZN_TUNE_ATTN_SPLIT_COLS = 19
 ZN_TUNE_NKEYS = 20
@@ -104,6 +104,7 @@
     "zn_tenant_release": (C.c_int, [C.c_int32, C.c_void_p]),
     "zn_decode_path": (C.c_int, [C.c_void_p]),
     "zn_decode_path_detail": (C.c_int, [C.c_void_p]),
+    "zn_step_tail_in_kernel": (C.c_int, [C.c_void_p]),
     "zn_get_counters": (C.c_int, [C.c_void_p, C.POINTER(C.c_int64), C.c_int32]),
     "zn_all_stopped": (C.c_int, [C.c_void_p, C.POINTER(C.c_int32), C.c_void_p]),
     "zn_all_stopped_begin": (C.c_int, [C.c_void_p, C.c_void_p]),
diff --git a/zonos_amd/csrc/zn_api.hip b/zonos_amd/csrc/zn_api.hip
--- a/zonos_amd/csrc/zn_api.hip
+++ b/zonos_amd/csrc/zn_api.hip
@@ -25,6 +25,7 @@
   int attn_fused = 0;
   int run = 1;
   bool fused_tail = false;
+  bool tail_in_kernel = false;
   int graph_slot = 0;
 };
 
@@ -44,6 +45,10 @@
   unsigned long long *ch_gy1 = nullptr, *ch_gx1 = nullptr, *ch_gx2 = nullptr, *ch_gm = nullptr;
   unsigned long long *ch_gqkv = nullptr, *ch_ga = nullptr;
   unsigned long long *ch_gbmax = nullptr, *ch_gpart = nullptr;
+  unsigned long long* ch_gcand = nullptr;
+  SampleArgs* tail_rec = nullptr;
+  SampleArgs tail_rec_host{};
+  bool tail_rec_valid = false;
   bool stackv_ok[4] = {};
   bool stackv1_ok[4] = {};
   StackLayer* stack_layers = nullptr;
@@ -196,7 +201,7 @@
   if (!h) return ZN_OK;
   (void)zn_tenant_release(h->device, h);
   free_graph(h);
-  void* ptrs[] = {h->emb_tables_dev, h->x, h->q, h->o1, h->mbuf, h->nbuf, h->logits_raw, h->last_logits, h->tok_raw, h->scores, h->cmax, h->pv_part, h->pv_tickets, h->pf_x, h->pf_n, h->pf_qkv, h->pf_a, h->pf_u, h->pf_m, h->pf_res, h->pf_zx, h->pf_xbc, h->pf_y, h->pf_g, h->qkv_tmp, h->fw_lengths, h->row_len, h->st, h->remaining, h->stopping, h->row_tab, h->prefix_shift, h->step0, h->adm_cache, h->adm_layers, h->adm_dev, h->res, h->hn, h->m_zx, h->m_xbc, h->m_y, h->m_g, h->m_vg, h->g16_part, h->g16_tickets, h->ln_part, h->ch_gy1, h->ch_gx1, h->ch_gx2, h->ch_gm, h->ch_epoch, h->ch_x2, h->x_emb, h->tail_ticket, h->ch_gqkv, h->ch_ga, h->ch_gbmax, h->ch_gpart, h->stack_layers, h->ch_diag};
+  void* ptrs[] = {h->emb_tables_dev, h->x, h->q, h->o1, h->mbuf, h->nbuf, h->logits_raw, h->last_logits, h->tok_raw, h->scores, h->cmax, h->pv_part, h->pv_tickets, h->pf_x, h->pf_n, h->pf_qkv, h->pf_a, h->pf_u, h->pf_m, h->pf_res, h->pf_zx, h->pf_xbc, h->pf_y, h->pf_g, h->qkv_tmp, h->fw_lengths, h->row_len, h->st, h->remaining, h->stopping, h->row_tab, h->prefix_shift, h->step0, h->adm_cache, h->adm_layers, h->adm_dev, h->res, h->hn, h->m_zx, h->m_xbc, h->m_y, h->m_g, h->m_vg, h->g16_part, h->g16_tickets, h->ln_part, h->ch_gy1, h->ch_gx1, h->ch_gx2, h->ch_gm, h->ch_epoch, h->ch_x2, h->x_emb, h->tail_ticket, h->ch_gqkv, h->ch_ga, h->ch_gbmax, h->ch_gpart, h->ch_gcand, h->tail_rec, h->stack_layers, h->ch_diag};
   for (void* p : ptrs) if (p) (void)hipFree(p);
   if (h->done_host) (void)hipHostFree(h->done_host);
   if (h->adm_stage) (void)hipHostFree(h->adm_stage);
@@ -302,7 +307,9 @@
     ZC(hipMalloc(&h->ch_ga, R * (c.d_model / 2) * 8)); ZC(hipMemset(h->ch_ga, 0, R * (c.d_model / 2) * 8));
     { const size_t nbm = (size_t)2 * c.n_heads_kv * ZN_SK_KB_MAXNB * 4 * 8, npt = (size_t)2 * c.n_heads_kv * ZN_SK_KB_MAXNB * ZN_SK_KB_PSZ * 8;
       ZC(hipMalloc(&h->ch_gbmax, nbm)); ZC(hipMemset(h->ch_gbmax, 0, nbm));
-      ZC(hipMalloc(&h->ch_gpart, npt)); ZC(hipMemset(h->ch_gpart, 0, npt)); }
+      ZC(hipMalloc(&h->ch_gpart, npt)); ZC(hipMemset(h->ch_gpart, 0, npt));
+      ZC(hipMalloc(&h->ch_gcand, (size_t)ZN_CH_GRID * 4 * 8)); ZC(hipMemset(h->ch_gcand, 0, (size_t)ZN_CH_GRID * 4 * 8));
+      ZC(hipMalloc(&h->tail_rec, sizeof(SampleArgs))); }
     ZC(hipMalloc(&h->stack_layers, (size_t)c.n_layer * sizeof(StackLayer))); }
   ZC(hipMalloc(&h->ch_gm, R * (c.d_ff / 2 + 1) * 8));
   ZC(hipMemset(h->ch_gm, 0, R * (c.d_ff / 2 + 1) * 8));
@@ -711,6 +718,12 @@
   return nb <= ZN_SK_KB_MAXNB && (rows == 1 ? h->stackv1_ok : h->stackv_ok)[stack_variant_of(nb)] ? nb : -1;
 }
 static int graph_slot_for(const StepPlan& p) { return p.path == StepPlan::STACK ? 8 + (p.run > 1 ? ZN_SK_KB_MAXNB + 1 : 0) + p.nbk : p.attn_fused + (p.run > 1 ? 4 : 0); }
+static bool one_wg_sampler(zn_handle h) {
+  const zn_config& c = h->cfg;
+  const bool use_penalty = h->rows_set || (h->sp.repetition_penalty != 1.0f);
+  return h->batch == 1 && !h->rows_set && h->tune[ZN_TUNE_SAMPLER] != 2 && c.vocab_head <= 64 * ZN_S1_IT && c.n_codebooks <= 16 && !(h->sp.top_p > 0.f) && h->sp.top_k <= 0 &&
+         !(h->sp.linear > 0.f) && (!use_penalty || h->sp.repetition_penalty_window <= 16) && h->rows <= 1024;
+}
 static bool chain_allowed(zn_handle h, int rows) { return h->ch_variant != 0 && rows == 2 && persist_allowed(h); }
 static StepPlan plan_blocks(zn_handle h, int rows, int keys) {
   StepPlan p;
@@ -728,17 +741,20 @@
     p.path = StepPlan::STACK; p.nbk = nb_run >= 0 ? nb_run : nb_one; p.run = nb_run >= 0 ? ZN_GRAPH_STEPS : 1;
   } else if (want_run && attn_fused_for(h, keys_run) == p.attn_fused) p.run = ZN_GRAPH_STEPS;
   p.fused_tail = tail_ok && p.path != StepPlan::LAUNCHES;
+  p.tail_in_kernel = p.path == StepPlan::STACK && p.fused_tail && one_wg_sampler(h) && !(h->sp.temperature > 0.f) && h->tune[ZN_TUNE_SAMPLER] != 3 &&
+                     h->tune[ZN_TUNE_STEP_TAIL] != 2 && h->cfg.vocab_head > 128 && h->cfg.vocab_head < 0xffff;
   p.graph_slot = graph_slot_for(p);
   return p;
 }
 static bool stack_pre(zn_handle h) { return h->tune[ZN_TUNE_STACK_PRE] != 2; }
-static int launch_stack(zn_handle h, hipStream_t s, int rows, int nbk) {
+static int launch_stack(zn_handle h, hipStream_t s, int rows, int nbk, bool tail = false) {
   const zn_config& c = h->cfg;
   ChainArgs a{};
   a.eps = c.norm_eps; a.F = c.d_ff; a.nqkv = (c.n_heads + 2 * c.n_heads_kv) * h->hd;
   a.xin = h->x_emb; a.xout = h->x;
   a.g_y1 = h->ch_gy1; a.g_x1 = h->ch_gx1; a.g_x2 = h->ch_gx2; a.g_m = h->ch_gm; a.g_qkv = h->ch_gqkv; a.g_a = h->ch_ga;
   a.g_bmax = h->ch_gbmax; a.g_part = h->ch_gpart;
+  if (tail) { a.tail = h->tail_rec; a.g_cand = h->ch_gcand; }
   a.epoch = h->ch_epoch; a.tmo = &h->st->pad[0]; a.diag = h->ch_diag;
   a.dbg_pause = h->dbg_pause;
   a.stamps = h->ch_stamps; a.stamp_layer = c.n_layer / 2;
@@ -968,26 +984,8 @@
   return a;
 }
 
-static int enqueue_step(zn_handle h, const StepPlan& p, hipStream_t s) {
-  const zn_config& c = h->cfg;
-  int rc;
-  const bool fused = p.fused_tail;
-  if (!fused) {
-    EmbedArgs e = make_embed_args(h);
-    e.out = h->x;
-    hipLaunchKernelGGL(embed_kernel, dim3(h->batch), dim3(256), 0, s, e);
-  }
-  if (c.arch == 1) {
-    if ((rc = hybrid_token(h, true, p.attn_fused, s))) return rc;
-  } else {
-    bool heads_done = false;
-    if (p.path == StepPlan::STACK) {
-      if (!stack_pre(h) && (rc = layer_in_proj(h, 0, h->x_emb, (bf16_t*)h->kv_layers[0], h->max_len, h->lengths, h->rows, s))) return rc;
-      if ((rc = launch_stack(h, s, h->rows, p.nbk))) return rc;
-      heads_done = true;
-    } else if ((rc = decode_blocks(h, p, nullptr, 0, s, fused ? h->x_emb : nullptr, &heads_done))) return rc;
-    if (!heads_done && (rc = heads_logits(h, h->x, h->rows, s))) return rc;
-  }
+static SampleArgs step_sample_args(zn_handle h, bool fused) {
+  const zn_config& c = h->cfg;
   SampleArgs a = gen_sample_args(h);
   a.raw = h->logits_raw; a.mix = guided(h) ? 1 : 0; a.apply_bias = 1; a.batch = h->batch;
   a.codes = h->codes; a.t_total = h->t_total;
@@ -998,9 +996,33 @@
   f.mask_id = c.mask_id; f.tokens = h->tok_raw; f.remaining = h->remaining; f.stopping = h->stopping; f.lengths = h->lengths;
   f.rows = h->rows; f.first = 0; f.override = h->tok_override; f.override_calls = h->tok_override_calls; f.shift = a.shift; f.step0 = a.step0;
   if (fused) { a.ticket = h->tail_ticket; a.em = make_embed_args(h); }
-  const bool one_wg = fused && h->batch == 1 && !h->rows_set && h->tune[ZN_TUNE_SAMPLER] != 2 && (h->tune[ZN_TUNE_SAMPLER] == 3 || !(h->sp.temperature > 0.f)) && c.vocab_head <= 64 * ZN_S1_IT &&
-                      c.n_codebooks <= 16 && !(h->sp.top_p > 0.f) && h->sp.top_k <= 0 && !(h->sp.linear > 0.f) &&
-                      (!a.use_penalty || h->sp.repetition_penalty_window <= 16) && h->rows <= 1024;
+  return a;
+}
+
+static int enqueue_step(zn_handle h, const StepPlan& p, hipStream_t s) {
+  const zn_config& c = h->cfg;
+  int rc;
+  const bool fused = p.fused_tail;
+  if (!fused) {
+    EmbedArgs e = make_embed_args(h);
+    e.out = h->x;
+    hipLaunchKernelGGL(embed_kernel, dim3(h->batch), dim3(256), 0, s, e);
+  }
+  if (c.arch == 1) {
+    if ((rc = hybrid_token(h, true, p.attn_fused, s))) return rc;
+  } else {
+    bool heads_done = false;
+    if (p.path == StepPlan::STACK) {
+      if (!stack_pre(h) && (rc = layer_in_proj(h, 0, h->x_emb, (bf16_t*)h->kv_layers[0], h->max_len, h->lengths, h->rows, s))) return rc;
+      if ((rc = launch_stack(h, s, h->rows, p.nbk, p.tail_in_kernel))) return rc;
+      if (p.tail_in_kernel) return ZN_OK;
+      heads_done = true;
+    } else if ((rc = decode_blocks(h, p, nullptr, 0, s, fused ? h->x_emb : nullptr, &heads_done))) return rc;
+    if (!heads_done && (rc = heads_logits(h, h->x, h->rows, s))) return rc;
+  }
+  SampleArgs a = step_sample_args(h, fused);
+  FrameArgs& f = a.fr;
+  const bool one_wg = fused && one_wg_sampler(h) && (h->tune[ZN_TUNE_SAMPLER] == 3 || !(h->sp.temperature > 0.f));
   if (one_wg) { hipLaunchKernelGGL(sample1_kernel, dim3(1), dim3(1024), 0, s, a); return ZN_OK; }
   hipLaunchKernelGGL(sample_kernel, dim3(c.n_codebooks, h->batch), dim3(256), 0, s, a);
   if (!fused) hipLaunchKernelGGL(frame_update_kernel, dim3(1), dim3(256), 0, s, f);
@@ -1035,6 +1057,7 @@
     HIPCHK(h, hipMemsetAsync(h->ch_gm, 0, R * (h->cfg.d_ff / 2 + 1) * 8, s));
     HIPCHK(h, hipMemsetAsync(h->ch_gbmax, 0, (size_t)2 * h->cfg.n_heads_kv * ZN_SK_KB_MAXNB * 4 * 8, s));
     HIPCHK(h, hipMemsetAsync(h->ch_gpart, 0, (size_t)2 * h->cfg.n_heads_kv * ZN_SK_KB_MAXNB * ZN_SK_KB_PSZ * 8, s));
+    HIPCHK(h, hipMemsetAsync(h->ch_gcand, 0, (size_t)ZN_CH_GRID * 4 * 8, s));
     const unsigned one = 1;
     HIPCHK(h, hipMemcpyAsync(h->ch_epoch, &one, sizeof one, hipMemcpyHostToDevice, s));
     HIPCHK(h, hipStreamSynchronize(s));
@@ -1630,6 +1653,14 @@
     const int k = p.graph_slot, run = p.run;
     if (p.fused_tail && !h->emb_valid) hipLaunchKernelGGL(embed_kernel, dim3(h->batch), dim3(256), 0, s, make_embed_args(h));
     h->emb_valid = p.fused_tail;
+    if (p.tail_in_kernel) {
+      const SampleArgs rec = step_sample_args(h, true);
+      if (!h->tail_rec_valid || std::memcmp(&rec, &h->tail_rec_host, sizeof rec) != 0) {
+        std::memcpy(&h->tail_rec_host, &rec, sizeof rec);
+        HIPCHK(h, ZN_NOT_IN_CAPTURE(hipMemcpyAsync(h->tail_rec, &h->tail_rec_host, sizeof rec, hipMemcpyHostToDevice, s)));
+        h->tail_rec_valid = true;
+      }
+    }
     if (!h->graph_exec[k] && !h->graph_tried[k] && n > 1) {
       h->graph_tried[k] = true;
       if (!h->cap_stream) (void)hipStreamCreateWithFlags(&h->cap_stream, hipStreamNonBlocking);
@@ -1676,6 +1707,7 @@
   if (!h || !h->gen_active || h->cfg.arch != 0 || !persist_active(h, h->rows)) return 0;
   return h->last_plan.path == StepPlan::STACK ? 2 : chain_allowed(h, h->rows) ? 1 : 0;
 }
+extern "C" int zn_step_tail_in_kernel(zn_handle h) { return h && h->gen_active && h->last_plan.tail_in_kernel ? 1 : 0; }
 extern "C" int zn_decode_path(zn_handle h) { return zn_decode_path_detail(h) != 0 ? 1 : 0; }
 extern "C" int zn_graph_active(zn_handle h) {
   if (!h) return 0;
diff --git a/zonos_amd/csrc/zn_chain_kernel.h b/zonos_amd/csrc/zn_chain_kernel.h
--- a/zonos_amd/csrc/zn_chain_kernel.h
+++ b/zonos_amd/csrc/zn_chain_kernel.h
@@ -54,6 +54,8 @@
   unsigned long long* g_part;
   const bf16_t *pre_W, *pre_ln_w, *pre_ln_b;
   bf16_t* pre_kv;
+  const SampleArgs* tail;
+  unsigned long long* g_cand;
 };
 struct StackLayer {
   const bf16_t *W_out, *W_fc1, *W_fc2, *W_in;
diff --git a/zonos_amd/csrc/zn_decode_kernels.h b/zonos_amd/csrc/zn_decode_kernels.h
--- a/zonos_amd/csrc/zn_decode_kernels.h
+++ b/zonos_amd/csrc/zn_decode_kernels.h
@@ -1747,13 +1747,80 @@
   for (int w = 0; w < 4; ++w) t += wave_sum(part[w]);
   return t;
 }
+#include "zn_step_tail.h"
 ZN_DEVINL void s1_argmax(float& v, int& i) {
 #pragma unroll
   for (int o = 32; o > 0; o >>= 1) {
     const float ov = __shfl_xor(v, o);
     const int oi = __shfl_xor(i, o);
-    if (ov > v || (ov == v && oi < i)) { v = ov; i = oi; }
-  }
+    if (zn_first_max(ov, oi, v, i)) { v = ov; i = oi; }
+  }
+}
+ZN_DEVINL float s1_logit(float cc, float uu, bool mix, float cfg_scale, bool apply_bias, int i, int eos_id, int cb, float st_bias, bool st_force) {
+  float x = mix ? __fadd_rn(uu, __fmul_rn(__fsub_rn(cc, uu), cfg_scale)) : cc;
+  if (apply_bias && i == eos_id) {
+    if (cb == 0) {
+      x = __fadd_rn(x, -0.6931471824645996f);
+      x += st_bias;
+      if (st_force) x = 1.0e4f;
+    } else x = -INFINITY;
+  }
+  return x;
+}
+template <class Tok> ZN_DEVINL bool s1_window_factor(int w, int nw, int V, float penalty, Tok tokat, int& g, float& f) {
+  g = tokat(w);
+  if (g < 0) return false;
+  g = g > V - 1 ? V - 1 : g;
+  bool seen = false;
+  f = 1.f;
+  for (int w2 = 0; w2 < nw; ++w2) {
+    int g2 = tokat(w2);
+    g2 = g2 > V - 1 ? V - 1 : g2;
+    if (g2 == g) { if (w2 < w) seen = true; else f = __fmul_rn(f, penalty); }
+  }
+  return !seen;
+}
+ZN_DEVINL float s1_penalised(float l, float f) { return (l <= 0.f) ? __fmul_rn(l, f) : __fdiv_rn(l, f); }
+struct S1Frame {
+  int o, stp, fcb, fcbc; bool in_range, ovr; int* cell;
+  int cur = 0, rem = 0, stop = 0, otok = 0, otok0 = 0;
+  ZN_DEVINL void request(const FrameArgs& fr, int nq, int o_, int stp_, int t) {
+    o = o_; stp = stp_;
+    fcb = t & (ZN_FRAME_MAXQ - 1); fcbc = min(fcb, nq - 1);
+    const int col = o + 1;
+    in_range = fcb < nq && col < fr.t_total;
+    cell = fr.codes + (size_t)fcbc * fr.t_total + min(col, fr.t_total - 1);
+    const int call = stp + 1;
+    ovr = fr.override && call < fr.override_calls;
+    if (t < ZN_FRAME_MAXQ) {
+      cur = *cell; rem = fr.remaining[0]; stop = fr.stopping[0];
+      if (ovr) { otok = fr.override[(size_t)call * nq + fcbc]; otok0 = fr.override[(size_t)call * nq]; }
+    }
+  }
+  ZN_DEVINL int finish(const FrameArgs& fr, GenState* st, int nq, int tok_own, int tok0) {
+    const int tk = ovr ? otok : tok_own, tk0 = ovr ? otok0 : tok0;
+    if (tk0 == fr.eos_id) { rem = rem < nq ? rem : nq; stop = 1; }
+    int eos_idx = nq - rem; if (eos_idx > nq - 1) eos_idx = nq - 1;
+    int t = tk;
+    if (stop && fcb < eos_idx) t = fr.mask_id; else if (stop && fcb == eos_idx) t = fr.eos_id;
+    if (in_range && cur == -1) *cell = t;
+    const int code = (in_range && cur == -1) ? t : cur;
+    rem -= 1;
+    if (fcb == 0) {
+      fr.remaining[0] = rem; fr.stopping[0] = stop;
+      st->offset = o + 1; st->step = stp + 1; st->all_done = rem > 0 ? 0 : 1;
+    }
+    return code;
+  }
+};
+ZN_DEVINL void s1_embed_next(const EmbedArgs& em, const int* s_code) {
+  int code[ZN_EMBED_MAXQ];
+#pragma unroll
+  for (int i = 0; i < ZN_EMBED_MAXQ; ++i) {
+    const int c = s_code[min(i, em.n_q - 1)];
+    code[i] = c < 0 ? 0 : (c >= em.vocab_embed ? em.vocab_embed - 1 : c);
+  }
+  embed_row(em, 0, code);
 }
 __global__ __launch_bounds__(1024) void sample1_kernel(SampleArgs a) {
   const int tid = threadIdx.x, lane = tid & 63, cb = tid >> 6;
@@ -1781,49 +1848,24 @@
     nw = avail < a.pen_window ? avail : a.pen_window;
     if (lane < nw) hist_tok = a.codes[(size_t)cbq * a.t_total + (o + 1 - nw) + lane];
   }
-  const int fcb = tid & (ZN_FRAME_MAXQ - 1), fcbc = min(fcb, nq - 1);
-  const int col = o + 1;
-  const bool in_range = fcb < nq && col < fr.t_total;
-  int* cell = fr.codes + (size_t)fcbc * fr.t_total + min(col, fr.t_total - 1);
-  const int call = stp + 1;
-  const bool ovr = fr.override && call < fr.override_calls;
-  int cur = 0, rem = 0, stop = 0, otok = 0, otok0 = 0;
-  if (tid < ZN_FRAME_MAXQ) {
-    cur = *cell; rem = fr.remaining[0]; stop = fr.stopping[0];
-    if (ovr) { otok = fr.override[(size_t)call * nq + fcbc]; otok0 = fr.override[(size_t)call * nq]; }
-  }
+  S1Frame fq;
+  fq.request(fr, nq, o, stp, tid);
   int tok = 0;
   if (on) {
     float l[ZN_S1_IT];
 #pragma unroll
     for (int j = 0; j < ZN_S1_IT; ++j) {
       const int i = lane + 64 * j;
-      float x = a.mix ? __fadd_rn(uu[j], __fmul_rn(__fsub_rn(cc[j], uu[j]), a.cfg_scale)) : cc[j];
-      if (a.apply_bias && i == a.eos_id) {
-        if (cb == 0) {
-          x = __fadd_rn(x, -0.6931471824645996f);
-          x += st_bias;
-          if (st_force) x = 1.0e4f;
-        } else x = -INFINITY;
-      }
+      const float x = s1_logit(cc[j], uu[j], a.mix != 0, a.cfg_scale, a.apply_bias != 0, i, a.eos_id, cb, st_bias, st_force);
       if (a.logits_out && i < V) a.logits_out[(size_t)cb * V + i] = x;
       l[j] = x;
     }
     for (int w = 0; w < nw; ++w) {
-      int g = __shfl(hist_tok, w);
-      if (g < 0) continue;
-      g = g > V - 1 ? V - 1 : g;
-      bool seen = false;
-      float f = 1.f;
-      for (int w2 = 0; w2 < nw; ++w2) {
-        int g2 = __shfl(hist_tok, w2);
-        g2 = g2 > V - 1 ? V - 1 : g2;
-        if (g2 == g) { if (w2 < w) seen = true; else f = __fmul_rn(f, a.penalty); }
-      }
-      if (seen) continue;
+      int g; float f;
+      if (!s1_window_factor(w, nw, V, a.penalty, [&](int w2) { return __shfl(hist_tok, w2); }, g, f)) continue;
 #pragma unroll
       for (int j = 0; j < ZN_S1_IT; ++j)
-        if (lane + 64 * j == g) l[j] = (l[j] <= 0.f) ? __fmul_rn(l[j], f) : __fdiv_rn(l[j], f);
+        if (lane + 64 * j == g) l[j] = s1_penalised(l[j], f);
     }
     if (!(a.temperature > 0.f)) {
       float bv = -INFINITY; int bi = 0x7fffffff;
@@ -1875,29 +1917,8 @@
     if (lane == 0) { s_tok[cb] = tok; a.tokens[cb] = tok; }
   }
   __syncthreads();
-  if (tid < ZN_FRAME_MAXQ) {
-    const int tk = ovr ? otok : s_tok[fcbc], tk0 = ovr ? otok0 : s_tok[0];
-    if (tk0 == fr.eos_id) { rem = rem < nq ? rem : nq; stop = 1; }
-    int eos_idx = nq - rem; if (eos_idx > nq - 1) eos_idx = nq - 1;
-    int t = tk;
-    if (stop && fcb < eos_idx) t = fr.mask_id; else if (stop && fcb == eos_idx) t = fr.eos_id;
-    if (in_range && cur == -1) *cell = t;
-    s_code[fcb] = (in_range && cur == -1) ? t : cur;
-    rem -= 1;
-    if (fcb == 0) {
-      fr.remaining[0] = rem; fr.stopping[0] = stop;
-      a.st->offset = o + 1; a.st->step = stp + 1; a.st->all_done = rem > 0 ? 0 : 1;
-    }
-  }
+  if (tid < ZN_FRAME_MAXQ) s_code[fq.fcb] = fq.finish(fr, a.st, nq, s_tok[fq.fcbc], s_tok[0]);
   if (tid < fr.rows) fr.lengths[tid] += 1;
   __syncthreads();
-  if (tid < 256) {
-    int code[ZN_EMBED_MAXQ];
-#pragma unroll
-    for (int i = 0; i < ZN_EMBED_MAXQ; ++i) {
-      const int c = s_code[min(i, a.em.n_q - 1)];
-      code[i] = c < 0 ? 0 : (c >= a.em.vocab_embed ? a.em.vocab_embed - 1 : c);
-    }
-    embed_row(a.em, 0, code);
-  }
-}
+  if (tid < 256) s1_embed_next(a.em, s_code);
+}
diff --git a/zonos_amd/csrc/zn_step_kernel.h b/zonos_amd/csrc/zn_step_kernel.h
--- a/zonos_amd/csrc/zn_step_kernel.h
+++ b/zonos_amd/csrc/zn_step_kernel.h
@@ -1,6 +1,7 @@
 #pragma once
 #include "zn_chain_kernel.h"
 #include "zn_step_sched.h"
+#include "zn_step_tail.h"
 
 #define ZN_SK_THREADS 512
 #ifndef ZN_SK_CW
@@ -154,6 +155,7 @@
   });
 }
 
+ZN_DEVINL void step_tail_role(const ChainArgs& a, unsigned tag, int nsw, int wave, int lane, unsigned wait_prev);
 template <int NBV, int R>
 ZN_DEVINL void step_attention_kb_role(const ChainArgs& a, StepKbLds& S, const unsigned tag0, const int c, const int wave, const int lane_in) {
   static_assert(NBV >= 1 && NBV <= ZN_SK_KB_MAXNB, "blocks covered");
@@ -375,6 +377,96 @@
     pace.start();
   }
   if (wave == ZN_SK_CW) pace.report(a.diag, lane_in);
+  if (c == 0 && a.tail) step_tail_role(a, tag0 + (unsigned)a.n_layer, (int)gridDim.x - a.natt, wave, lane_in, pace.prev);
+}
+
+#ifndef ZN_SK_TAIL_BACKOFF
+#define ZN_SK_TAIL_BACKOFF 8
+#endif
+ZN_DEVINL void step_tail_role(const ChainArgs& a, const unsigned tag, const int nsw, const int wave, const int lane, const unsigned wait_prev) {
+  __shared__ int s_tcode[ZN_FRAME_MAXQ];
+  __shared__ unsigned s_twait;
+  const SampleArgs& t = *a.tail;
+  const unsigned long long t_ref = __builtin_amdgcn_s_memrealtime();
+  if (wave == ZN_SK_CW && lane == 0) s_twait = wait_prev;
+  __syncthreads();
+  if (wave == 0) {
+    const bool stamped = a.stamps && lane == 0;
+    const int nq = t.n_q;
+    const int o = t.st->offset, stp = t.st->step;
+    S1Frame fq;
+    fq.request(t.fr, nq, o, stp, lane);
+    {
+      const unsigned prev = s_twait;
+      const unsigned long long until = t_ref + (prev - (prev >> ZN_SK_PACE_SHIFT));
+      while (__builtin_amdgcn_s_memrealtime() < until) __builtin_amdgcn_s_sleep(8);
+    }
+    if (stamped) a.stamps[58] = __builtin_amdgcn_s_memrealtime();
+    const __amdgpu_buffer_rsrc_t rs = zn_rsrc(a.g_cand);
+    u32x4 c0[4], c1[4];
+    SpinBound sb; sb.begin();
+    for (;;) {
+      ++sb.np;
+      bool ok = true;
+#pragma unroll
+      for (int j = 0; j < 4; ++j) {
+        const int off = min(lane + 64 * j, nsw - 1) * 32;
+        c0[j] = ld_sc1_16(rs, off); c1[j] = ld_sc1_16(rs, off + 16);
+        ok &= (c0[j].y == tag) & (c0[j].w == tag) & (c1[j].y == tag) & (c1[j].w == tag);
+      }
+      unsigned long long bad = __builtin_amdgcn_ballot_w64(!ok);
+      ZN_TIMING_PASS(bad);
+      if (bad == 0ull) break;
+      if (sb.give_up(a.tmo)) {
+        unsigned badoff = 0, badtag = 0;
+#pragma unroll
+        for (int j = 3; j >= 0; --j) {
+          const int off = min(lane + 64 * j, nsw - 1) * 32;
+          if (c1[j].w != tag) { badoff = off + 24; badtag = c1[j].w; }
+          if (c1[j].y != tag) { badoff = off + 16; badtag = c1[j].y; }
+          if (c0[j].w != tag) { badoff = off + 8; badtag = c0[j].w; }
+          if (c0[j].y != tag) { badoff = off; badtag = c0[j].y; }
+        }
+        sb.report(a.tmo, SweepWho{(9u << 8) | (unsigned)(a.n_layer - 1), a.diag}, bad, lane, tag, badoff, badtag);
+        break;
+      }
+      __builtin_amdgcn_s_sleep(ZN_SK_TAIL_BACKOFF);
+    }
+    if (stamped) a.stamps[59] = __builtin_amdgcn_s_memrealtime();
+    int tok_own = 0, tok0 = 0, tok_lane = 0;
+    zn_static_for<0, ZN_FRAME_MAXQ>([&](auto CB) {
+      constexpr int cb = decltype(CB)::value;
+      float bv = -INFINITY; int bi = ZN_TAIL_NONE;
+#pragma unroll
+      for (int j = 0; j < 4; ++j)
+#pragma unroll
+        for (int k = 0; k < 2; ++k) {
+          const float v = __uint_as_float(k == 0 ? c0[j].x : c1[j].x);
+          const unsigned w = k == 0 ? c0[j].z : c1[j].z;
+          const int wi = zn_tail_word_idx(w);
+          const bool take = zn_tail_word_cb(w) == cb && zn_first_max(v, wi, bv, bi);
+          bv = take ? v : bv; bi = take ? wi : bi;
+        }
+#pragma unroll
+      for (int o2 = 32; o2 > 0; o2 >>= 1) {
+        const float ov = __shfl_xor(bv, o2);
+        const int oi = __shfl_xor(bi, o2);
+        const bool take = zn_first_max(ov, oi, bv, bi);
+        bv = take ? ov : bv; bi = take ? oi : bi;
+      }
+      const int tok = zn_first_max_token(bi);
+      tok_own = cb == fq.fcbc ? tok : tok_own;
+      tok0 = cb == 0 ? tok : tok0;
+      tok_lane = cb == lane ? tok : tok_lane;
+    });
+    if (lane < nq) t.tokens[lane] = tok_lane;
+    if (stamped) a.stamps[60] = __builtin_amdgcn_s_memrealtime();
+    if (lane < ZN_FRAME_MAXQ) s_tcode[fq.fcb] = fq.finish(t.fr, t.st, nq, tok_own, tok0);
+    if (lane < t.fr.rows) t.fr.lengths[lane] += 1;
+  }
+  __syncthreads();
+  if (threadIdx.x < 256) s1_embed_next(t.em, s_tcode);
+  if (a.stamps && threadIdx.x == 0) { __builtin_amdgcn_s_waitcnt(0); a.stamps[61] = __builtin_amdgcn_s_memrealtime(); }
 }
 
 template <int R, int NCH, int T_OUT, int T_FC1, int T_FC2, int T_IN, int NBV>
@@ -402,7 +494,7 @@
   __shared__ float s_res[2][64][2][R];
   __shared__ __attribute__((aligned(16))) bf16_t s_ln[4 * D];
   const int sc = c - natt, NSW = (int)gridDim.x - natt;
-  auto split = [&](int U, int& n, int& start) { const int base = U / NSW, extra = U % NSW; n = base + (sc < extra ? 1 : 0); start = sc * base + min(sc, extra); };
+  auto split = [&](int U, int& n, int& start) { zn_tail_split(U, NSW, sc, n, start); };
   int n_out, s_out, ng1, sg1;
   split(D / 2, n_out, s_out);
   split(F / 2, ng1, sg1);
@@ -787,6 +879,23 @@
     int opq = 0;
     asm volatile("" : "+v"(opq));
     const int irq = ir + opq, uoq = u_out + opq, uqq = u_qkv + opq;
+    const SampleArgs* tl = a.tail;
+    const bool tail_on = tl != nullptr && last && epi;
+    int t_nw = 0, t_hist = -1, t_cbA = 0;
+    float t_bias = 0.f;
+    bool t_force = false;
+    if (tail_on) {
+      const int o = tl->st->offset, stp = tl->st->step;
+      t_bias = tl->st->eos_bias;
+      t_force = tl->st->force_eos_step == stp;
+      t_cbA = (2 * s_hd) / tl->V;
+      if (tl->use_penalty && tl->codes) {
+        const int avail = o + 1 < tl->ctx ? o + 1 : tl->ctx;
+        t_nw = avail < tl->pen_window ? avail : tl->pen_window;
+        const int cbw = min(t_cbA + (lane >> 4), tl->n_q - 1);
+        if (lane < 32 && (lane & 15) < t_nw) t_hist = tl->codes[(size_t)cbw * tl->t_total + (o + 1 - t_nw) + (lane & 15)];
+      }
+    }
     pace.sleep();
     stamp();
     sweep_granules<NCH>(zn_rsrc(a.g_a), goff, tag, g, a.tmo, lane, SweepWho{(6u << 8) | (unsigned)li, a.diag});
@@ -832,6 +941,51 @@
             a.heads_out[(size_t)irq * a.heads_rows + 2 * u] = bfround(s_res[par][ij][0][ir]);
             if (2 * u + 1 < a.heads_rows) a.heads_out[(size_t)irq * a.heads_rows + 2 * u + 1] = bfround(s_res[par][ij][1][ir]);
           }
+          if (tail_on) {
+            const bool tstamp = a.stamps && sc == 0 && lane == 0;
+            if (tstamp) a.stamps[56] = __builtin_amdgcn_s_memrealtime();
+            const int V = tl->V;
+            const bool mix = tl->mix != 0;
+            float xh[2]; int cbh[2], ih[2]; bool vh[2];
+#pragma unroll
+            for (int hh = 0; hh < 2; ++hh) {
+              const int r = 2 * (s_hd + ij) + hh;
+              vh[hh] = ij < n_hd && ir == 0 && r < a.heads_rows;
+              const int rr = vh[hh] ? r : 0;
+              cbh[hh] = rr / V; ih[hh] = rr - cbh[hh] * V;
+              const float cc = bfround(s_res[par][ij][hh][0]);
+              const float uu = (R == 2 && mix) ? bfround(s_res[par][ij][hh][R - 1]) : cc;
+              xh[hh] = s1_logit(cc, uu, mix, tl->cfg_scale, tl->apply_bias != 0, ih[hh], tl->eos_id, cbh[hh], t_bias, t_force);
+              if (vh[hh] && tl->logits_out) tl->logits_out[rr] = xh[hh];
+            }
+#pragma unroll
+            for (int k = 0; k < 2; ++k)
+              for (int w = 0; w < t_nw; ++w) {
+                int gt; float f;
+                if (!s1_window_factor(w, t_nw, V, tl->penalty, [&](int w2) { return __shfl(t_hist, 16 * k + w2); }, gt, f)) continue;
+#pragma unroll
+                for (int hh = 0; hh < 2; ++hh)
+                  if (vh[hh] && cbh[hh] == t_cbA + k && ih[hh] == gt) xh[hh] = s1_penalised(xh[hh], f);
+              }
+            float bv[2] = {-INFINITY, -INFINITY}; int bi[2] = {ZN_TAIL_NONE, ZN_TAIL_NONE};
+#pragma unroll
+            for (int k = 0; k < 2; ++k) {
+#pragma unroll
+              for (int hh = 0; hh < 2; ++hh)
+                if (vh[hh] && cbh[hh] == t_cbA + k) zn_first_max_scan(xh[hh], ih[hh], bv[k], bi[k]);
+              s1_argmax(bv[k], bi[k]);
+            }
+            if (lane < 4) {
+              const int k = lane >> 1;
+              const int r_last = min(2 * (s_hd + n_hd), a.heads_rows) - 1;
+              const bool used = n_hd > 0 && (k == 0 || r_last / V != t_cbA);
+              const float v = k == 0 ? bv[0] : bv[1];
+              const int bidx = k == 0 ? bi[0] : bi[1];
+              const unsigned word = (lane & 1) == 0 ? __float_as_uint(used ? v : -INFINITY) : (used ? zn_tail_pack(bidx, t_cbA + k) : (unsigned)ZN_TAIL_NONE);
+              st_granule(a.g_cand + ((size_t)sc * 2 + k) * 2 + (lane & 1), tag, word);
+            }
+            if (tstamp) a.stamps[57] = __builtin_amdgcn_s_memrealtime();
+          }
         } else if (it_qkv) {
           const int rowA = 2 * u_qkv;
           const float x0 = bfround(s_res[par][ij][0][ir]), x1 = bfround(s_res[par][ij][1][ir]);
diff --git a/zonos_amd/csrc/zn_step_tail.h b/zonos_amd/csrc/zn_step_tail.h
--- /dev/null
+++ b/zonos_amd/csrc/zn_step_tail.h
@@ -0,0 +1,23 @@
+#pragma once
+
+#if defined(__HIPCC__)
+#define ZN_TAIL_FN __host__ __device__ __forceinline__
+#else
+#define ZN_TAIL_FN inline
+#endif
+
+#define ZN_TAIL_NONE 0x7fffffff
+
+ZN_TAIL_FN void zn_tail_split(int U, int NSW, int sc, int& n, int& start) {
+  const int base = U / NSW, extra = U % NSW;
+  n = base + (sc < extra ? 1 : 0);
+  start = sc * base + (sc < extra ? sc : extra);
+}
+
+ZN_TAIL_FN void zn_first_max_scan(float x, int i, float& bv, int& bi) { if (x > bv) { bv = x; bi = i; } }
+ZN_TAIL_FN bool zn_first_max(float ov, int oi, float v, int i) { return ov > v || (ov == v && oi < i); }
+ZN_TAIL_FN int zn_first_max_token(int bi) { return bi == ZN_TAIL_NONE ? 0 : bi; }
+
+ZN_TAIL_FN unsigned zn_tail_pack(int idx, int cb) { return (unsigned)(idx == ZN_TAIL_NONE ? 0xffff : idx) | ((unsigned)cb << 16); }
+ZN_TAIL_FN int zn_tail_word_cb(unsigned w) { return (int)(w >> 16); }
+ZN_TAIL_FN int zn_tail_word_idx(unsigned w) { return (w & 0xffffu) == 0xffffu ? ZN_TAIL_NONE : (int)(w & 0xffffu); }
```

After: 13.70 audio-sec/sec. -1.1%, worse.
